# alexkroman/tiny-audio

Measured on AMD Instinct MI355X. Metric: training audio-sec/sec on 10s@16kHz clips, higher is better.
Workload: dtype bf16

## Files before the change

### include/ta355.h

```cpp
#ifndef TA355_H
#define TA355_H

#ifdef __cplusplus
extern "C" {
#endif

#ifndef __HIP_PLATFORM_AMD__
typedef struct ihipStream_t* hipStream_t;
#endif

#define TA_OK 0
#define TA_ERR_ARG 1
#define TA_ERR_LAUNCH 2

int ta_version(void);



long ta_logmel_scratch_floats(int B, int Ls, int n_mels);
int ta_logmel_mel_ranges(const float* melfb, int n_mels, int* mel_ranges, hipStream_t st);
int ta_logmel_f32(const float* wav, const long* lens, int B, int Ls, const float* dft, const float* window,
                  const float* melfb, int n_mels, float* feats, int* mask, float* scratch, const int* mel_ranges, hipStream_t st);

typedef struct {
// ... 83 lines not shown

int ta_moe_pack_images(const float* const* w1, const float* const* b1, const float* const* w2, const float* const* b2, int n, int H, int In,
                       int D, void* W1a, void* W1ta, void* W2a, void* W2ta, float* B1a, float* B2a, hipStream_t st);
long ta_moe_tape_bytes(const ta_moe_weights* w, int B, int S);
long ta_moe_bwd_workspace_bytes(const ta_moe_weights* w, int B, int S);
int ta_moe_projector_forward(const ta_moe_weights* w, const void* x_bf16, int B, int S, const float* noise, int training,
                             float* y, float* aux, void* tape, hipStream_t st);
int ta_moe_projector_backward(const ta_moe_weights* w, const void* x_bf16, int B, int S, const float* dy, float d_aux,
                              const float* noise, int training, const void* tape, float* d_norm_w, float* d_router_w,
                              float* const* dW1, float* const* db1, float* const* dW2, float* const* db2, void* ws,
                              long ws_bytes, hipStream_t st);
int ta_moe_projector_backward_dev(const ta_moe_weights* w, const void* x_bf16, int B, int S, const float* dy,
                                  const float* d_aux_dev, const float* noise, int training, const void* tape,
                                  float* d_norm_w, float* d_router_w, float* const* dW1, float* const* db1,
                                  float* const* dW2, float* const* db2, void* ws, long ws_bytes, hipStream_t st);

int ta_moe_router_aux_grads(const ta_moe_weights* w, const void* x_bf16, int B, int S, const float* d_aux_dev, const float* noise,
                            int training, const void* tape, float* d_norm_w_aux, float* d_router_w_aux, void* ws, long ws_bytes,
                            hipStream_t st);

typedef struct {
  const float* ln_in_w;
  const void *wqkv, *wqkv_t;
  const float *qn_w, *kn_w;
  const void *wo, *wo_t;
  const float* ln_post_w;
  const void *wgu, *wgu_t;
  const void *wd, *wd_t;
  const float *la_qkv, *lb_qkv, *la_o, *lb_o, *la_gu, *lb_gu, *la_d, *lb_d;
} ta_lm_layer;

typedef struct {
  float *dla_qkv, *dlb_qkv, *dla_o, *dlb_o, *dla_gu, *dlb_gu, *dla_d, *dlb_d;
} ta_lm_lora_grads;

typedef struct {
  int vocab, vocab_pad, hidden, ffn, n_layers, heads, kv_heads, head_dim, max_pos;
  float eps;
  const float* embed_f32;
  const void* embed_bf16;
  const void* embed_t_bf16;
  const float* norm_w;
  const float *rope_cos, *rope_sin;
  const ta_lm_layer* layers;
  int lora_rank;
  float lora_scale;
  int train_base;
  int lora_groups;
  int res_f32;
  int dx_f32;
  unsigned long long nope_layers;
} ta_lm_weights;

typedef struct {
  float *dwqkv;
  float *dwo;
  float *dwgu;
  float *dwd;
  float *dln_in, *dln_post;
  float *dqn, *dkn;
} ta_lm_layer_wgrads;
typedef struct {
  const ta_lm_layer_wgrads* layers;
  float* dnorm;
  float* dembed;
} ta_lm_wgrads;

long ta_lm_tape_bytes(const ta_lm_weights* w, int B, int L, int n_label_rows);
long ta_lm_workspace_bytes(const ta_lm_weights* w, int B, int L, int n_label_rows);
int ta_lm_forward_loss(const ta_lm_weights* w, const long* ids, const int* src_row, const float* audio,
                       const int* kmask, const int* pos, int B, int L, const int* label_rows,
                       const long* label_targets, int n_label_rows, float loss_scale, float* loss,
                       float* nll_rows, void* logits_out, void* tape, void* ws, long ws_bytes, hipStream_t st);
int ta_gelu_fwd(const void* h_bf16, void* a_bf16, long n, hipStream_t st);
int ta_gelu_bwd(const void* da_bf16, const void* h_bf16, void* dh_bf16, long n, hipStream_t st);
int ta_colsum(const void* x, int is_f32, int R, int C, float* out, hipStream_t st);
int ta_relu_fwd(const void* h_bf16, void* a_bf16, long n, hipStream_t st);
int ta_relu_bwd(const void* da_bf16, const void* h_bf16, void* dh_bf16, long n, hipStream_t st);
int ta_mix_fwd(const float* logits, const float* o, float* rw, float* out, int M, int D, int E, hipStream_t st);
int ta_mix_bwd(const float* dout, const float* o, const float* rw, void* do_bf16, float* dlogits, int M, int D, int E,
               hipStream_t st);
int ta_layernorm_res_fwd(const float* z, const float* keep, const float* res, long res_rows, const float* gamma,
                         const float* beta, float eps, float* xhat, float* rstd, float* y_f32, void* y_bf16, int M, int H,
                         hipStream_t st);
int ta_layernorm_bwd(const float* dy, const float* xhat, const float* rstd, const float* gamma, const float* keep, float* du,
                     void* dz_bf16, float* dgamma, float* dbeta, int M, int H, hipStream_t st);
int ta_attn_small_fwd(const void* Q, const void* K, const void* V, int EB, int heads, int hd, int Lq, int Lk, float scale,
                      const float* keep, float* P, void* O, hipStream_t st);
int ta_attn_small_bwd(const void* dO, const void* Q, const void* K, const void* V, const float* P, const float* keep,
                      float scale, void* dQ, void* dK, void* dV, int EB, int heads, int hd, int Lq, int Lk, hipStream_t st);

long ta_lm_prefill_workspace_bytes(const ta_lm_weights* w, int B, int L);
long ta_lm_lora_image_bytes(const ta_lm_weights* w);
int ta_lm_prefill(const ta_lm_weights* w, const long* ids, const int* src_row, const float* audio, const int* kmask,
                  const int* pos, int B, int L, void* kcache, void* vcache, int Lmax, const int* last_rows, float* logits,
                  void* lora_img, void* ws, long ws_bytes, hipStream_t st);
long ta_lm_decode_workspace_bytes(const ta_lm_weights* w, int B);
int ta_lm_decode_step(const ta_lm_weights* w, const long* ids, const int* pos, const int* kmask, const int* slot_dev, int B,
                      void* kcache, void* vcache, int Lmax, float* logits, const void* lora_img, void* ws, long ws_bytes,
                      hipStream_t st);
int ta_argmax_f32(const float* x, long ld, int n, int rows, long* out, hipStream_t st);
int ta_logits_process(float* logits, long ld, int V, const long* prompt_ids, int L, const long* out_seq, int max_new,
                      const int* step_dev, int B, float repetition_penalty, int no_repeat_ngram_size, hipStream_t st);
int ta_logits_warp(float* logits, long ld, int V, int B, float temperature, int top_k, float top_p, hipStream_t st);
int ta_sample_f32(const float* logits, long ld, int V, int B, unsigned long long seed, const int* step_dev, long* out, hipStream_t st);
int ta_logits_suppress_until(float* logits, long ld, int V, const long* ids, int n_ids, int min_new, const int* step_dev, int B,
                             hipStream_t st);
#define TA_SEQ_BIAS_MAX_SEQS 4096
#define TA_SEQ_BIAS_MAX_LEN 32
int ta_logits_sequence_bias(float* logits, long ld, int V, const long* prompt_ids, int L, const long* out_seq, int max_new,
                            const int* step_dev, int B, const long* seq_tokens, const int* seq_offsets, const float* seq_bias,
                            const int* group_starts, int n_seq, int n_groups, int n_tokens, hipStream_t st);
int ta_logits_step_rules(float* logits, long ld, int V, int B, const int* step_dev, int max_new, const long* forced_eos_ids,
                         int n_forced, const long* eos_ids, int n_eos, int decay_start, const float* decay_mult,
                         const long* suppress_ids, int n_suppress, const long* begin_suppress_ids, int n_begin, hipStream_t st);
int ta_logits_warp_ext(float* logits, long ld, int V, int B, float min_p, float typical_p, float epsilon_cutoff, float eta_cutoff,
                       hipStream_t st);
int ta_greedy_advance(const long* amax, const long* eos_ids, int n_eos, long pad_id, int* finished, long* next_ids,
                      long* out_seq, int max_new, int* step_dev, int* slot_dev, int* pos, int* kmask, int Lmax, int B,
                      int* n_unfinished, hipStream_t st);
int ta_token_scores_f32(const float* logits, long ld, int V, int B, const long* chosen, const int* finished, const int* step_dev,
                        int max_new, int top_k, float* logprob, float* entropy, long* top_ids, float* top_logprobs, hipStream_t st);

#define TA_EXTEND_MAX_T 256
#define TA_EXTEND_MAX_R 1024
int ta_attention_extend(const void* Q, const void* Kn, const void* Vn, const void* Kc, const void* Vc, const int* pmask,
                        const int* clip_of, const int* len, void* O, float* LSE, int B, int R, int Hq, int Hkv, int T, int Lp,
                        int Lmax, float scale, hipStream_t st);
#define TA_SCORE_MAX_ROWS 65536
#define TA_SCORE_CE_ROWS 256
long ta_lm_score_workspace_bytes(const ta_lm_weights* w, int B, int R, int T);
int ta_lm_score(const ta_lm_weights* w, const long* ids, const int* len, const int* len_host, const int* clip_of, const int* pos0,
                int B, int R, int T, const void* kcache, const void* vcache, int Lp, const int* pmask, const float* logits,
                const void* lora_img, float* token_logprobs, float* score, void* ws, long ws_bytes, hipStream_t st);

int ta_beam_logprobs_f32(float* logits, long ld, int V, int R, hipStream_t st);
long ta_beam_topk_workspace_bytes(int B, int K, int V, int M);
int ta_beam_topk_f32(const float* rows, long ld, int V, const float* score, int B, int K, int M, float* cand_score, int* cand_flat,
                     void* ws, long ws_bytes, hipStream_t st);
int ta_beam_advance(const float* cand_score, const int* cand_flat, int B, int K, int M, int V, const long* eos_ids, int n_eos,
                    long pad_id, int max_new, const float* len_div, int early_stopping, int heur_max_len, long* run_seq,
                    float* run_score, int* parent, long* next_ids, long* pool_seq, float* pool_score, int* pool_len,
                    int* pool_fin, int* heur, int* clip_done, int* step_dev, int* slot_dev, int* pos, int* kmask, int Lmax,
                    int* n_unfinished, float* tr_cand_score, int* tr_cand_flat, long* tr_run_seq, float* tr_run_score,
                    int* tr_parent, hipStream_t st);
int ta_kv_beam_expand(const void* ksrc, const void* vsrc, void* kdst, void* vdst, int layers, int B, int K, int kv_heads, int L,
                      int Lsrc, int Lmax, int head_dim, hipStream_t st);
int ta_kv_beam_reorder(void* kcache, void* vcache, int layers, int B, int K, int kv_heads, int L, int Lmax, int head_dim, int max_new,
                       const int* parent, const int* slot_dev, hipStream_t st);

int ta_lm_backward(const ta_lm_weights* w, const int* src_row, const int* kmask, const int* pos, int B, int L,
                   const int* label_rows, int n_label_rows, float* d_audio, long n_audio_rows, float* d_embeds,
                   const ta_lm_lora_grads* lora_grads, const ta_lm_wgrads* wgrads, const long* ids, const void* tape, void* ws,
                   long ws_bytes, hipStream_t st);

typedef struct ta_lora_dropout {
  float p;
  unsigned long long seed;
  unsigned long long offset;
} ta_lora_dropout;
int ta_lm_forward_loss_ex(const ta_lm_weights* w, const long* ids, const int* src_row, const float* audio,
                          const int* kmask, const int* pos, int B, int L, const int* label_rows,
                          const long* label_targets, int n_label_rows, float loss_scale, float* loss,
                          float* nll_rows, void* logits_out, void* tape, void* ws, long ws_bytes,
                          const ta_lora_dropout* drop, hipStream_t st);
int ta_lm_backward_ex(const ta_lm_weights* w, const int* src_row, const int* kmask, const int* pos, int B, int L,
                      const int* label_rows, int n_label_rows, float* d_audio, long n_audio_rows, float* d_embeds,
                      const ta_lm_lora_grads* lora_grads, const ta_lm_wgrads* wgrads, const long* ids, const void* tape, void* ws,
                      long ws_bytes, const ta_lora_dropout* drop, hipStream_t st);
int ta_segment_table(const int* segment_ids, int* seg, int* pos, int R, int L, hipStream_t st);
int ta_audio_index_seg(const long* ids, const int* segment_ids, const long* counts, int* src_row, int R, int L, int C, int N,
                       long audio_id, hipStream_t st);
int ta_lm_forward_loss_seg(const ta_lm_weights* w, const long* ids, const int* src_row, const float* audio,
                           const int* kmask, const int* pos, const int* seg, int B, int L, const int* label_rows,
                           const long* label_targets, int n_label_rows, float loss_scale, float* loss,
                           float* nll_rows, void* logits_out, void* tape, void* ws, long ws_bytes,
                           const ta_lora_dropout* drop, hipStream_t st);
int ta_lm_backward_seg(const ta_lm_weights* w, const int* src_row, const int* kmask, const int* pos, const int* seg, int B, int L,
                       const int* label_rows, int n_label_rows, float* d_audio, long n_audio_rows, float* d_embeds,
                       const ta_lm_lora_grads* lora_grads, const ta_lm_wgrads* wgrads, const long* ids, const void* tape, void* ws,
                       long ws_bytes, const ta_lora_dropout* drop, hipStream_t st);
struct ta_ce_options;
int ta_lm_forward_loss_opt(const ta_lm_weights* w, const long* ids, const int* src_row, const float* audio,
                           const int* kmask, const int* pos, const int* seg, int B, int L, const int* label_rows,
                           const long* label_targets, int n_label_rows, float loss_scale, float* loss,
                           float* nll_rows, void* logits_out, void* tape, void* ws, long ws_bytes,
                           const ta_lora_dropout* drop, const struct ta_ce_options* ce, hipStream_t st);
int ta_attention_fwd_seg(const void* Q, const void* K, const void* VT, void* O, float* LSE, const int* kmask, const int* seg,
                         int B, int Hq, int Hkv, int L, int Lp, float scale, hipStream_t st);
int ta_attention_fwd_qkv_seg(const void* qkv0, const float* qn_w, const float* kn_w, const float* cosT, const float* sinT,
                             const int* pos, void* Q, void* K, void* V, float* rq, float* rk, void* O, float* LSE,
                             const int* kmask, const int* seg, int B, int Hq, int Hkv, int L, float scale, float eps,
                             hipStream_t st);
int ta_attention_bwd_seg(const void* Q, const void* K, const void* V, const void* dO, long dO_stride, const float* LSE,
                         const float* Delta, const int* kmask, const int* seg, void* dQ, void* dK, void* dV, int B, int Hq,
                         int Hkv, int L, int Lp, float scale, hipStream_t st);
int ta_attention_bwd_qkv_seg(const void* Q, const void* K, const void* V, const void* dO, long dO_stride, const float* LSE,
                             const float* Delta, const int* kmask, const int* seg, const void* qkv0, const float* rq,
                             const float* rk, const float* qn_w, const float* kn_w, const float* cosT, const float* sinT,
                             const int* pos, void* dqkv, int B, int Hq, int Hkv, int L, int Lp, float scale, hipStream_t st);
int ta_lora_dropout_keep(const ta_lora_dropout* drop, int layer, int linear, int M, int in, unsigned char* out, hipStream_t st);


int ta_attention_enc_fwd(const void* qkv, void* out, int B, int heads, int S, hipStream_t st);
int ta_attention_enc_fwd_varlen(const void* qkv, void* out, const int* cu_rows, int B, int heads, int max_rows, hipStream_t st);

int ta_gemm_bf16_nt(const void* A, const void* W, void* C, int M, int N, int K, long lda, int a_rpb, long a_bs,
                    long ldc, int c_rpb, long c_bs, long c_off, const float* bias, const float* residual, int act,
                    int out_bf16, int splits, float* splitk_ws, hipStream_t st);
int ta_gemm_bf16_nt_ex(const void* A, const void* W, void* C, int M, int N, int K, long lda, int a_rpb, long a_bs,
                       long ldc, int c_rpb, long c_bs, long c_off, const float* bias, const float* residual, int act,
                       int out_bf16, int splits, float* splitk_ws, const int* a_idx, const int* seg,
                       const int* krange, hipStream_t st);
typedef struct {
  const void* a2; const void* w2; int k2; long lda2;
  const void* residual_bf16;
  const float* rope_tab; int rope_rows;
  int w_blocked;
  int rope_cols;
} ta_gemm_opts;
int ta_gemm_bf16_nt_opt(const void* A, const void* W, void* C, int M, int N, int K, long lda, int a_rpb, long a_bs,
                        long ldc, int c_rpb, long c_bs, long c_off, const float* bias, const float* residual, int act,
                        int out_bf16, int splits, float* splitk_ws, const int* a_idx, const int* seg,
                        const int* krange, const ta_gemm_opts* opts, hipStream_t st);
long ta_gemm_splitk_ws_bytes(int M, int N, int splits);
int ta_gemm_bf16_nt_grouped(const void* A, const void* W, void* C, int M, int N, int K, const float* bias, int act, int out_bf16,
                            const int* a_idx, const int* seg, const int* krange, int n_groups, long w_stride, long c_stride,
                            hipStream_t st);
long ta_gemm_bf16_tn_ws_bytes(int M, int Ny, int Nx);
int ta_gemm_bf16_tn(const void* Y, const void* X, float* out, int M, int Ny, int Nx, int accumulate, void* ws, long ws_bytes,
                    hipStream_t st);
int ta_profile_gemm(int enable);
int ta_profile_gemm_collect(double* total_ms, double* total_flops, long* launches);
long ta_profile_gemm_log(long* out, long max_rows);
int ta_gemm_reload_knobs(void);

int ta_layernorm_f32(const float* x, const float* w, const float* b, void* y_bf16, float* y_f32,
                     const float* rowscale, int M, int H, float eps, hipStream_t st);
int ta_layernorm_bf16(const void* x_bf16, const float* w, const float* b, void* y_bf16, float* y_f32, const float* rowscale,
                      int M, int H, float eps, hipStream_t st);
int ta_rmsnorm_fwd(const float* x, const float* w, void* y_bf16, float* y_f32, float* rstd, int M, int H,
                   float eps, int act_gelu, hipStream_t st);
int ta_rmsnorm_bwd(const float* dy, const float* x, const float* rstd, const float* w, const float* dres,
                   float* dx_f32, void* dx_bf16, float* dw_accum, int M, int H, int act_gelu, hipStream_t st);
int ta_rmsnorm_fwd_bf16(const void* x_bf16, const float* w, void* y_bf16, float* y_f32, float* rstd, int M, int H, float eps,
                        hipStream_t st);
int ta_rmsnorm_bwd_bf16(const void* dy, int dy_is_bf16, const void* x_bf16, const float* rstd, const float* w,
                        const float* dres, float* dx_f32, void* dx_bf16, int M, int H, hipStream_t st);
int ta_rmsnorm_bwd_bf16s(const void* dy, int dy_is_bf16, const void* x_bf16, const float* rstd, const float* w,
                         const void* dres_bf16, float* dx_f32, void* dx_bf16, int M, int H, hipStream_t st);
int ta_rmsnorm_bwd_dyb(const void* dy_bf16, const float* x, const float* rstd, const float* w, const float* dres, float* dx_f32,
                       void* dx_bf16, int M, int H, hipStream_t st);

int ta_rmsnorm_dw(const void* dy, int dy_is_bf16, const void* x, int x_is_bf16, const float* rstd, float* dw_accum, int M,
                  int H, hipStream_t st);

int ta_attention_fwd(const void* Q, const void* K, const void* VT, void* O, float* LSE, const int* kmask, int B,
                     int Hq, int Hkv, int L, int Lp, int head_dim, int causal, float scale, hipStream_t st);
typedef struct { long q_bs, q_hs, q_rs, k_bs, k_hs, k_rs, v_bs, v_hs, v_rs; } ta_attn_layout;
int ta_attention_fwd_ex(const void* Q, const void* K, const void* VT, void* O, float* LSE, const int* kmask, int B,
                        int Hq, int Hkv, int L, int Lp, int head_dim, int causal, float scale, const ta_attn_layout* lay,
                        hipStream_t st);
int ta_attention_fwd_qkv(const void* qkv0, const float* qn_w, const float* kn_w, const float* cosT, const float* sinT,
                         const int* pos, void* Q, void* K, void* V, float* rq, float* rk, void* O, float* LSE,
                         const int* kmask, int B, int Hq, int Hkv, int L, float scale, float eps, hipStream_t st);
int ta_attention_bwd(const void* Q, const void* QT, const void* K, const void* KT, const void* V, const void* dO,
                     long dO_stride, const void* dOT, const float* LSE, const float* Delta, const int* kmask,
                     void* dQ, void* dK, void* dV, int B, int Hq, int Hkv, int L, int Lp, int head_dim, int causal,
                     float scale, hipStream_t st);
int ta_attention_bwd_qkv(const void* Q, const void* K, const void* V, const void* dO, long dO_stride, const float* LSE,
                         const float* Delta, const int* kmask, const void* qkv0, const float* rq, const float* rk,
                         const float* qn_w, const float* kn_w, const float* cosT, const float* sinT, const int* pos,
                         void* dqkv, int B, int Hq, int Hkv, int L, int Lp, int head_dim, int causal, float scale,
                         hipStream_t st);
int ta_enc_qkv_post(const void* qkv, const float* cosT, const float* sinT, void* Q, void* K, void* VT, int B, int H,
                    int S, int Sp, hipStream_t st);
int ta_lm_qkv_post_fwd(const void* qkv0, const float* qn_w, const float* kn_w, const float* cosT, const float* sinT,
                       const int* pos, void* Q, void* K, void* V, void* QT, void* KT, void* VT, float* rq, float* rk,
                       int B, int Hq, int Hkv, int L, int Lp, float eps, hipStream_t st);
int ta_lm_qkv_post_bwd(const void* dQ, const void* dK, const void* dV, const void* qkv0, const float* rq,
                       const float* rk, const float* qn_w, const float* kn_w, const float* cosT, const float* sinT,
                       const int* pos, void* dqkv, float* dqn_accum, float* dkn_accum, int B, int Hq, int Hkv, int L, hipStream_t st);
int ta_attn_bwd_prep(const void* dO, const void* O, float* Delta, void* dOT, int B, int Hq, int L, int Lp,
                     hipStream_t st);

int ta_swiglu_fwd(const void* gu, void* act, long M, int F, hipStream_t st);
int ta_swiglu_bwd(const void* dact, const void* gu, void* dgu, long M, int F, hipStream_t st);
int ta_cast_f32_bf16(const float* x, void* y, long n, hipStream_t st);
int ta_transpose_to_bf16(const void* in, int in_is_f32, long ld_in, long in_bs, int in_rpb, void* out, long ld_out,
                         int R, int C, hipStream_t st);
int ta_feats_to_time_major(const float* feats, void* out, int B, int C, int T, hipStream_t st);
int ta_zero_pad_rows(void* buf, int B, int T, int C, hipStream_t st);
int ta_pos_add(void* x, int x_f32, const float* pos, int B, int S, int H, hipStream_t st);

int ta_audio_index(const long* ids, const long* counts, int* src_row, int B, int L, int N, long audio_id,
                   hipStream_t st);
int ta_embed_scatter(const long* ids, const int* src_row, const float* emb, const float* audio, float* x0,
                     void* x0_bf16, int n_rows, int D, long vocab, hipStream_t st);
int ta_audio_grad_gather(const int* src_row, const float* dx0, float* d_audio, int n_rows, int D, hipStream_t st);
int ta_embed_grad_scatter(const long* ids, const int* src_row, const float* dx0, float* dembed, int n_rows, int D, long vocab,
                          hipStream_t st);
int ta_gather_rows_bf16(const void* in, const int* idx, void* out, int n, int D, hipStream_t st);
int ta_scatter_rows_f32(const float* in, const int* idx, float* out, int n, int D, hipStream_t st);
int ta_bernoulli_keep(float* keep, long n, float keep_prob, unsigned long long seed, hipStream_t st);
int ta_debug_occupy(int workgroups, double micros, void* buf, long bytes, hipStream_t st);

int ta_cross_entropy(const void* logits, int logits_bf16, long ldl, const int* rows, const long* targets, int n, int V,
                     float scale, float* nll, float* loss_accum, void* dlogits_bf16, long ldd, hipStream_t st);
int ta_label_rows(const long* labels, int B, int L, int* rows, long* targets, int* n_out, hipStream_t st);
typedef struct ta_ce_options {
  float eps;
  float zc;
  float* obj;
} ta_ce_options;
int ta_cross_entropy_opt(const void* logits, int logits_bf16, long ldl, const int* rows, const long* targets, int n, int V,
                         float scale, float* nll, float* loss_accum, void* dlogits_bf16, long ldd, const ta_ce_options* opt,
                         hipStream_t st);

#define TA_SQNORM_SCRATCH_FLOATS 1024
int ta_grad_sqnorm(const float* g, long n, float* accum, float* scratch, hipStream_t st);
int ta_adamw_step(float* p, const float* g, float* m, float* v, long n, float lr, float beta1, float beta2, float eps,
                  float weight_decay, int step, const float* sqnorm, float max_norm, float grad_scale,
                  const float* denom, hipStream_t st);
int ta_adamw_step_multi(float* p, const float* g, float* m, float* v, long n, const long* seg_end, const float* seg_lr,
                        const float* seg_wd, int nseg, float lr_mult, float beta1, float beta2, float eps, int step,
                        const float* sqnorm, float max_norm, float grad_scale, const float* denom, hipStream_t st);

#define TA_WAVE_CONV_HOP 2048
#define TA_WAVE_CONV_DIRECT 32
int ta_wave_fft_twiddles(float* tw, hipStream_t st);
int ta_wave_ir_spectra(const float* ir, const long* ir_off, const int* part_off, int n_ir, int max_parts, const float* tw,
                       float* spectra, hipStream_t st);
long ta_wave_conv_ws_bytes(int B, int Ls, int max_taps);
int ta_wave_conv_f32(const float* wav, const long* lens, int B, int Ls, const int* ir_idx, const float* ir, const long* ir_off,
                     const int* part_off, int n_ir, int max_taps, const float* tw, const float* spectra, float rir_peak,
                     float* out, void* ws, long ws_bytes, hipStream_t st);
long ta_wave_mix_scratch_floats(int B, int Ls);
int ta_wave_mix_f32(float* wav, const long* lens, int B, int Ls, const int* noise_idx, const long* noise_start,
                    const float* noise_amp, const float* noise, const long* noise_off, int n_noise, const float* gauss_amp,
                    unsigned long long seed, unsigned long long offset, float* scratch, hipStream_t st);
int ta_wave_clip_f32(float* wav, const long* lens, int B, int Ls, const int* pct, hipStream_t st);
#define TA_WAVE_MAX_EVENTS 64
long ta_wave_events_scratch_floats(int B, int Ls, int ev_stride, long max_event_len);
int ta_wave_events_f32(float* wav, const long* lens, int B, int Ls, const int* ev_count, int ev_stride, const int* ev_pool,
                       const long* ev_off, const long* ev_len, const long* ev_t0, const int* ev_fade_in, const int* ev_fade_out,
                       const float* ev_amp, const float* pool, const long* pool_off, int n_pool, long max_event_len,
                       float fade_floor_db, float* scratch, hipStream_t st);
#define TA_WAVE_IIR_MAX_SECTIONS 8
#define TA_WAVE_IIR_CHUNK 256
long ta_wave_sos_ws_bytes(int B, int Ls, int chunk);
int ta_wave_sos_f32(float* wav, const long* lens, int B, int Ls, const int* n_sec, const double* sos, int chunk, void* ws,
                    long ws_bytes, hipStream_t st);

#define TA_ALIGN_MAX_TOKENS 2048
#define TA_ALIGN_MAX_FRAMES 32768
#define TA_ALIGN_MAX_CLASSES 65536
#define TA_ALIGN_MAX_CLIPS 4096
#define TA_ALIGN_THREADS 256
#define TA_ALIGN_FRAME_BLOCK 64
#define TA_ALIGN_STAGE_FLOATS 8192
long ta_ctc_align_workspace_bytes(int N, int max_T, int max_J);
int ta_ctc_align_f32(const float* emission, long ld, int C, const int* cu_frames, const int* tokens, const int* cu_tokens, int N,
                     int max_T, int max_J, int blank_id, int* frames, float* score, int* status, void* ws, long ws_bytes,
                     float* trellis_out, const long* trellis_off, hipStream_t st);

#define TA_ALIGN_LONG_MAX_TOKENS 262144
#define TA_ALIGN_LONG_MAX_FRAMES 1048576
#define TA_ALIGN_LONG_MAX_CLASSES 65536
#define TA_ALIGN_LONG_MAX_CLIPS 64
#define TA_ALIGN_LONG_MAX_COL_BLOCK 2048
#define TA_ALIGN_LONG_COL_BLOCK 256
#define TA_ALIGN_LONG_FRAME_BLOCK 64
long ta_ctc_align_long_workspace_bytes(int N, int max_T, int max_J, int col_block, int frame_block);
int ta_ctc_align_long_f32(const float* emission, long ld, int C, const int* cu_frames, const int* tokens, const int* cu_tokens, int N,
                          int max_T, int max_J, int blank_id, int col_block, int frame_block, int* frames, float* score, int* status,
                          void* ws, long ws_bytes, float* trellis_out, const long* trellis_off, hipStream_t st);

#define TA_TEXT_ALIGN_EDIT 0
#define TA_TEXT_ALIGN_LCS 1
#define TA_TEXT_ALIGN_MAX_LEN 262144
#define TA_TEXT_ALIGN_MAX_PAIRS 65536
#define TA_TEXT_ALIGN_MAX_COL_BLOCK 512
#define TA_TEXT_ALIGN_SHORT_MAX_M 512
#define TA_TEXT_ALIGN_COL_BLOCK 256
#define TA_TEXT_ALIGN_ROW_BLOCK 256
long ta_text_align_workspace_bytes(const int* cu_ref_host, const int* cu_hyp_host, int N, int max_n, int max_m, int want_path,
                                   int col_block, int row_block);
int ta_text_align_i32(const int* ref, const int* cu_ref, const int* hyp, const int* cu_hyp, int N, int max_n, int max_m, int mode,
                      int want_path, int col_block, int row_block, int* dist, int* counts, int* map, int* status, void* ws,
                      long ws_bytes, hipStream_t st);

#define TA_W2V_HEAD_PAD 64
typedef struct {
  int hidden, ffn, n_layers, heads, conv_dim, n_classes;
  float ln_eps;
  const float* conv0_w;
  const float *gn_w, *gn_b;
  const void* conv_w[6];
  const float *fp_ln_w, *fp_ln_b;
  const void* fp_w;
  const float* fp_b;
  const void* pos_w;
  const float* pos_b;
  const float *enc_ln_w, *enc_ln_b;
  const ta_enc_layer* layers;
  const void* head_w;
  const float* head_b;
  int res_f32;
} ta_wav2vec2_weights;

long ta_wav2vec2_workspace_bytes(const ta_wav2vec2_weights* w, int B, int Ls, long rows);
int ta_wav2vec2_forward(const ta_wav2vec2_weights* w, const float* wav, const int* lens_host, const int* lens_dev,
                        const int* cu_frames_dev, int B, int Ls, float* emissions, void* ws, long ws_bytes, hipStream_t st);

long ta_w2v_conv0_ws_bytes(int B, int Ls, int C);
int ta_w2v_conv0_gn_gelu(const float* wav, const int* lens_dev, int B, int Ls, const float* w, const float* gn_w,
                         const float* gn_b, int C, float eps, void* out_bf16, long out_rpb, void* ws, long ws_bytes,
                         hipStream_t st);
int ta_w2v_pos_conv(const void* x, int x_f32, const void* wp, const float* bias, void* y, const int* cu_rows, int B,
                    int max_rows, int H, hipStream_t st);
int ta_w2v_head_logsoftmax(const float* logits, long ld, const float* bias, int n_classes, float* out, int rows,
                           hipStream_t st);

#define TA_ECAPA_N_MELS 80
#define TA_ECAPA_FEAT_STRIDE 128
#define TA_ECAPA_SCALE 8
#define TA_ECAPA_MIN_T 5
#define TA_ECAPA_MAX_T 512
#define TA_ECAPA_MAX_DILATION 4
#define TA_ECAPA_MAX_CHANNELS 1024
#define TA_ECAPA_MAX_SE 256
#define TA_ECAPA_MAX_ATTN 256
#define TA_ECAPA_MAX_EMB 1024
typedef struct {
  const void* w1;
  const float *b1, *bn1_s, *bn1_t;
  const void* res_w;
  const float *res_b, *res_s, *res_t;
  const void* w2;
  const float *b2, *bn2_s, *bn2_t;
  const float *se_w1t, *se_b1;
  const float *se_w2t, *se_b2;
  int dilation;
} ta_ecapa_block;
typedef struct {
  int channels, se_channels, attn_channels, emb_dim;
  const float* fb_window;
  const float* fb_twiddle;
  const float* fb_mel;
  const int* fb_mel_range;
  const void* w0;
  const float *b0, *bn0_s, *bn0_t;
  ta_ecapa_block blocks[3];
  const void* mfa_w;
  const float *mfa_b, *mfa_s, *mfa_t;
  const void* att_wh;
  const void* att_wms;
  const float *att_b, *att_s, *att_t;
  const void* att_conv_w;
  const float* att_conv_b;
  const float *aspbn_s, *aspbn_t;
  const void* fc_w;
  const float* fc_b;
} ta_ecapa_weights;

long ta_ecapa_workspace_bytes(const ta_ecapa_weights* w, int n_windows, int T);
int ta_ecapa_forward(const ta_ecapa_weights* w, const float* audio, long n_audio, const int* starts_host, const int* lens_host,
                     const int* starts_dev, const int* lens_dev, int N, int window_samples, int chunk_windows, float* emb,
                     void* ws, long ws_bytes, hipStream_t st);

int ta_ecapa_fbank(const float* audio, long n_audio, const int* starts_dev, const int* lens_dev, int N, int window_samples,
                   const float* fb_window, const float* fb_twiddle, const float* fb_mel, const int* fb_mel_range,
                   float* feat, void* slab_bf16, hipStream_t st);
int ta_ecapa_res2net(const void* z1, long ldz, long z_rpw, const float* bn1_s, const float* bn1_t, const void* res_w,
                     const float* res_b, const float* res_s, const float* res_t, void* y, long ldy, long y_rpw, int N, int T,
                     int w, int dilation, hipStream_t st);
int ta_ecapa_relu_bn(const void* z, const float* scale, const float* shift, void* out, float* stats_f32, void* stats_bf16,
                     int N, int T, int Cw, hipStream_t st);
long ta_ecapa_se_ws_floats(int N, int Cw);
int ta_ecapa_se_residual(const void* z2, const float* bn2_s, const float* bn2_t, const float* se_w1t, const float* se_b1,
                         const float* se_w2t, const float* se_b2, const void* residual, long ldres, void* out, long ldout,
                         int N, int T, int Cw, int se, float* ws, hipStream_t st);
int ta_ecapa_attn_act(const float* g, const float* per_window, const float* scale, const float* shift, void* out, int N, int T,
                      int A, hipStream_t st);
int ta_ecapa_asp_pool(const float* logits, const void* h, const float* aspbn_s, const float* aspbn_t, void* out, float* attn_w,
                      float* pooled_f32, int N, int T, int Cw, hipStream_t st);

#define TA_SPK_MIN_N 6
#define TA_SPK_MAX_N 32768
#define TA_SPK_MAX_D 256
#define TA_SPK_MAX_P 32
#define TA_SPK_MAX_COLS 1024
long ta_spk_affinity_ws_floats(int N, int D);
int ta_spk_affinity_f32(const float* E, int N, int D, int keep, float* W, long ldw, float* deg, int* kept_count, float* ws, int phases,
                        hipStream_t st);
long ta_spk_lapmul_ws_floats(int N, int p);
int ta_spk_laplacian_matmul_f32(const float* W, long ldw, const float* deg, const float* X, long ldx, float* Y, long ldy, int N, int p,
                                float* ws, hipStream_t st);
long ta_spk_gram_ws_floats(int N, int a, int b);
int ta_spk_panel_gram_f32(const float* A, long lda, int a, const float* B, long ldb, int b, int N, float* C, long ldc, float* ws,
                          hipStream_t st);
int ta_spk_panel_update_f32(float* B, long ldb, int b, const float* A, long lda, int a, const float* C, long ldc, int N, hipStream_t st);
int ta_spk_panel_combine_f32(const float* V, long ldv, int c, const float* Z, long ldz, int m, float* Y, long ldy, int N, hipStream_t st);

#define TA_CUT_HOP 160
#define TA_CUT_POWER_WINDOW 400
#define TA_CUT_MAX_POSITIONS 1048576
#define TA_CUT_MAX_LEN 3000
#define TA_CUT_MAX_SMOOTH 64
#define TA_CUT_MAX_RECORDINGS 64
#define TA_CUT_MAX_BLOCKS 131072
#define TA_CUT_COST_K(h) (2 * (h) + 25 > 65 ? 2 * (h) + 25 : 65)
#define TA_WAVE_WINDOWS_MAX 65535
long ta_wave_cut_cost_workspace_bytes(int R, long max_n);
int ta_wave_cut_cost_f32(const float* wav, const long* offsets, int R, long max_n, int h, float cut_penalty, float* cost, long ld,
                         void* ws, long ws_bytes, hipStream_t st);
int ta_cut_plan_f32(const float* cost, long ld, const long* offsets, int R, long max_n, int min_len, int max_len, int* back, int* cuts,
                    long ldc, int* n_seg, float* dp_T, hipStream_t st);
int ta_wave_windows_f32(const float* wav, long total, const long* start, const int* len, int W, int Ls, float* out, long* lens,
                        hipStream_t st);

#ifdef __cplusplus
}
#endif
#endif
```

### tiny_audio_amd/csrc/api.hip

```cpp
#include <cstdlib>
#include "common.h"
#include "internal.h"
#include "../../include/ta355.h"

extern "C" int ta_version(void) { return 4; }

#include <algorithm>
#include "host_util.h"


namespace {
struct EncDesc {
  int H, F, L, nh, NM, max_pos, k1;
  float eps;
  const void *conv1_w, *conv2_w;
  const float *conv1_b, *conv2_b, *norm_w, *norm_b;
  const float *rope_cos, *rope_sin, *rope_il, *pos_emb;
  const ta_enc_layer* layers;
  int res_f32;
  bool whisper;
};
EncDesc enc_desc(const ta_encoder_weights* w) {
  return EncDesc{w->hidden, w->ffn, w->n_layers, w->heads, w->n_mels, w->max_pos, 3 * w->n_mels, w->ln_eps, w->conv1_w, w->conv2_w,
                 w->conv1_b, w->conv2_b, w->norm_w, w->norm_b, w->rope_cos, w->rope_sin, w->rope_il, nullptr, w->layers, w->res_f32, false};
}
EncDesc enc_desc(const ta_whisper_encoder_weights* w) {
  return EncDesc{w->hidden, w->ffn, w->n_layers, w->heads, w->n_mels, w->max_pos, pad64(3 * w->n_mels), w->ln_eps, w->conv1_w, w->conv2_w,
                 w->conv1_b, w->conv2_b, w->norm_w, w->norm_b, nullptr, nullptr, nullptr, w->pos_emb, w->layers, w->res_f32, true};
}
struct EncWs {
  bf16_t *x0, *x1, *xn, *qkv, *q, *k, *vt, *ao, *hf;
  float* xr;
  size_t bytes;
};
EncWs enc_carve(const EncDesc& d, int B, int T, void* base) {
  const int H = d.H, S = (T - 1) / 2 + 1, Sp = pad64(S);
  const long M = (long)B * S;
  Carver c(base);
  EncWs e;
  e.x0 = c.take<bf16_t>((size_t)B * (T + 2) * d.NM + (size_t)(d.k1 - 3 * d.NM));
  e.x1 = c.take<bf16_t>((size_t)B * (T + 2) * H);
  e.xr = (float*)c.take<float>((size_t)M * H);
  e.xn = c.take<bf16_t>((size_t)M * H);
  e.qkv = c.take<bf16_t>((size_t)M * 3 * H + 128);
  e.q = c.take<bf16_t>((size_t)M * H);
  e.k = c.take<bf16_t>((size_t)M * H);
  e.vt = c.take<bf16_t>((size_t)B * H * Sp);
  e.ao = c.take<bf16_t>((size_t)M * H);
  e.hf = c.take<bf16_t>((size_t)M * d.F);
  e.bytes = c.total();
  return e;
}

int enc_forward(const EncDesc& w, const float* feats, int B, int T, const float* frame_keep, void* out_bf16, float* out_f32,
                void* ws, long ws_bytes, hipStream_t st) {
  if (B <= 0 || T <= 0) return TA_OK;
  const int H = w.H, F = w.F, NM = w.NM, nh = w.nh, K1 = w.k1;
  if (H % 128 || F % 128 || K1 % 64 || NM % 8 || H / nh != 64 || (!out_bf16 && !out_f32)) return TA_ERR_ARG;
  const int S = (T - 1) / 2 + 1, Sp = pad64(S);
  if (S > w.max_pos) return TA_ERR_ARG;
  if (w.whisper && (T != 2 * w.max_pos || !w.pos_emb || H != nh * 64)) return TA_ERR_ARG;
  const int M = B * S;
  EncWs e = enc_carve(w, B, T, ws);
  if ((long)e.bytes > ws_bytes) return TA_ERR_ARG;
  RC(ta_feats_to_time_major(feats, e.x0, B, NM, T, st));
  if (K1 > 3 * NM && hipMemsetAsync(e.x0 + (size_t)B * (T + 2) * NM, 0, (size_t)(K1 - 3 * NM) * sizeof(bf16_t), st) != hipSuccess)
    return TA_ERR_LAUNCH;
  RC(ta_zero_pad_rows(e.x1, B, T, H, st));
  RC(ta_gemm_bf16_nt(e.x0, w.conv1_w, e.x1, B * T, H, K1, NM, T, (long)(T + 2) * NM, H, T, (long)(T + 2) * H, H,
                     w.conv1_b, nullptr, 1, 1, 1, nullptr, st));
  const bool res_f32 = w.res_f32 != 0;
  const int rb = res_f32 ? 0 : 1;
  auto ln = [&](const float* gw, const float* gb, void* yb, float* yf, const float* rowscale) -> int {
    return rb ? ta_layernorm_bf16(e.xr, gw, gb, yb, yf, rowscale, M, H, w.eps, st)
              : ta_layernorm_f32(e.xr, gw, gb, yb, yf, rowscale, M, H, w.eps, st);
  };
  auto res_gemm = [&](const void* A, const void* Wm, int K, const float* bias) -> int {
    if (rb) { ta_gemm_opts o = opts_none(); o.residual_bf16 = e.xr; return gemm_opt(A, Wm, e.xr, M, H, K, bias, nullptr, 0, 1, o, st); }
    return gemm(A, Wm, e.xr, M, H, K, bias, e.xr, 0, 0, st);
  };
  RC(ta_gemm_bf16_nt(e.x1, w.conv2_w, e.xr, M, H, 3 * H, 2L * H, S, (long)(T + 2) * H, H, 0, 0, 0, w.conv2_b, nullptr,
                     1, rb, 1, nullptr, st));
  if (w.whisper) RC(ta_pos_add(e.xr, res_f32 ? 1 : 0, w.pos_emb, B, S, H, st));
  const float scale = 0.125f;
  const char* fz = getenv("TA355_ENC_QKV_FUSED");
  const bool fa = w.whisper || (!(fz && *fz == '0') && w.rope_il && (H / nh) == 64);
  for (int l = 0; l < w.L; ++l) {
    const ta_enc_layer& L = w.layers[l];
    if (w.whisper && !(L.wqkv_fa && L.bqkv_fa)) return TA_ERR_ARG;
    RC(ln(L.ln1_w, L.ln1_b, e.xn, nullptr, nullptr));
    if (fa && L.wqkv_fa && L.bqkv_fa) {
      if (w.whisper) {
        RC(gemm(e.xn, L.wqkv_fa, e.qkv, M, 3 * H, H, L.bqkv_fa, nullptr, 0, 1, st));
      } else {
        ta_gemm_opts o = opts_none(); o.rope_tab = w.rope_il; o.rope_rows = S; o.rope_cols = 2 * H;
        RC(gemm_opt(e.xn, L.wqkv_fa, e.qkv, M, 3 * H, H, L.bqkv_fa, nullptr, 2, 1, o, st));
      }
      RC(ta_attention_enc_fwd(e.qkv, e.ao, B, nh, S, st));
      RC(res_gemm(e.ao, L.wo, H, L.bo));
    } else {
      RC(gemm(e.xn, L.wqkv, e.qkv, M, 3 * H, H, L.bqkv, nullptr, 0, 1, st));
      RC(ta_enc_qkv_post(e.qkv, w.rope_cos, w.rope_sin, e.q, e.k, e.vt, B, nh, S, Sp, st));
      RC(ta_attention_fwd(e.q, e.k, e.vt, e.ao, nullptr, nullptr, B, nh, nh, S, Sp, 64, 0, scale, st));
      RC(res_gemm(e.ao, L.wo, H, L.bo));
    }
    RC(ln(L.ln2_w, L.ln2_b, e.xn, nullptr, nullptr));
    RC(gemm(e.xn, L.w1, e.hf, M, F, H, L.b1, nullptr, 1, 1, st));
    RC(res_gemm(e.hf, L.w2, F, L.b2));
  }
  RC(ln(w.norm_w, w.norm_b, out_bf16, out_f32, frame_keep));
  return TA_OK;
}

struct EncRaggedWs {
  bf16_t *x0, *x1, *xn, *qkv, *ao, *hf;
  void* c2;
  float *xr, *rope;
  size_t bytes;
};
EncRaggedWs enc_ragged_carve(const EncDesc& d, int B, int T, long rows, void* base) {
  const int H = d.H, S = (T - 1) / 2 + 1;
  const long M = (long)B * S;
  Carver c(base);
  EncRaggedWs e;
  e.x0 = c.take<bf16_t>((size_t)B * (T + 2) * d.NM + (size_t)(d.k1 - 3 * d.NM));
  e.x1 = c.take<bf16_t>((size_t)B * (T + 2) * H);
  e.c2 = c.take<float>((size_t)M * H);
  e.xr = c.take<float>((size_t)rows * H);
  e.rope = c.take<float>((size_t)rows * 32);
  e.xn = c.take<bf16_t>((size_t)rows * H);
  e.qkv = c.take<bf16_t>((size_t)rows * 3 * H);
  e.ao = c.take<bf16_t>((size_t)rows * H);
  e.hf = c.take<bf16_t>((size_t)rows * d.F);
  e.bytes = c.total();
  return e;
}

int enc_forward_ragged(const EncDesc& w, const float* feats, int B, int T, const int* mel_len, const int* cu, const float* frame_keep,
                       void* out_bf16, float* out_f32, void* ws, long ws_bytes, hipStream_t st) {
  if (B <= 0 || T <= 0) return TA_OK;
  const int H = w.H, F = w.F, NM = w.NM, nh = w.nh, K1 = w.k1;
  if (H % 128 || F % 128 || K1 % 64 || NM % 8 || H / nh != 64 || (!out_bf16 && !out_f32) || !mel_len || !cu || !feats) return TA_ERR_ARG;
  if (!w.rope_il) return TA_ERR_ARG;
  if (K1 != 3 * NM) return TA_ERR_ARG;
  for (int l = 0; l < w.L; ++l) if (!(w.layers[l].wqkv_fa && w.layers[l].bqkv_fa)) return TA_ERR_ARG;
  const int S = (T - 1) / 2 + 1;
  if (S > w.max_pos) return TA_ERR_ARG;
  long rows_l = 0; int max_rows = 0;
  for (int b = 0; b < B; ++b) {
    if (mel_len[b] < 1 || mel_len[b] > T) return TA_ERR_ARG;
    const int Sb = (mel_len[b] - 1) / 2 + 1;
    rows_l += Sb; max_rows = Sb > max_rows ? Sb : max_rows;
  }
  if (rows_l > 0x7fffffffL / (3L * H)) return TA_ERR_ARG;
  const int rows = (int)rows_l;
  EncRaggedWs e = enc_ragged_carve(w, B, T, rows, ws);
  if ((long)e.bytes > ws_bytes) return TA_ERR_ARG;
  RC(ta_i_feats_to_time_major_len(feats, e.x0, B, NM, T, mel_len, st));
  RC(ta_gemm_bf16_nt(e.x0, w.conv1_w, e.x1, B * T, H, K1, NM, T, (long)(T + 2) * NM, H, T, (long)(T + 2) * H, H,
                     w.conv1_b, nullptr, 1, 1, 1, nullptr, st));
  RC(ta_i_zero_tail_rows(e.x1, B, T, H, mel_len, st));
  const bool res_f32 = w.res_f32 != 0;
  const int rb = res_f32 ? 0 : 1;
  RC(ta_gemm_bf16_nt(e.x1, w.conv2_w, e.c2, B * S, H, 3 * H, 2L * H, S, (long)(T + 2) * H, H, 0, 0, 0, w.conv2_b, nullptr,
                     1, rb, 1, nullptr, st));
  RC(ta_i_compact_rows(e.c2, e.xr, cu, B, S, rows, H * (rb ? 2 : 4), st));
  RC(ta_i_rope_rows(w.rope_il, e.rope, cu, B, rows, w.max_pos, st));
  const int M = rows;
  auto ln = [&](const float* gw, const float* gb, void* yb, float* yf) -> int {
    return rb ? ta_layernorm_bf16(e.xr, gw, gb, yb, yf, nullptr, M, H, w.eps, st)
              : ta_layernorm_f32(e.xr, gw, gb, yb, yf, nullptr, M, H, w.eps, st);
  };
  auto res_gemm = [&](const void* A, const void* Wm, int K, const float* bias) -> int {
    if (rb) { ta_gemm_opts o = opts_none(); o.residual_bf16 = e.xr; return gemm_opt(A, Wm, e.xr, M, H, K, bias, nullptr, 0, 1, o, st); }
    return gemm(A, Wm, e.xr, M, H, K, bias, e.xr, 0, 0, st);
  };
  for (int l = 0; l < w.L; ++l) {
    const ta_enc_layer& L = w.layers[l];
    RC(ln(L.ln1_w, L.ln1_b, e.xn, nullptr));
    ta_gemm_opts o = opts_none(); o.rope_tab = e.rope; o.rope_rows = rows; o.rope_cols = 2 * H;
    RC(gemm_opt(e.xn, L.wqkv_fa, e.qkv, M, 3 * H, H, L.bqkv_fa, nullptr, 2, 1, o, st));
    RC(ta_attention_enc_fwd_varlen(e.qkv, e.ao, cu, B, nh, max_rows, st));
    RC(res_gemm(e.ao, L.wo, H, L.bo));
    RC(ln(L.ln2_w, L.ln2_b, e.xn, nullptr));
    RC(gemm(e.xn, L.w1, e.hf, M, F, H, L.b1, nullptr, 1, 1, st));
    RC(res_gemm(e.hf, L.w2, F, L.b2));
  }
  bf16_t* yb = out_bf16 ? e.xn : nullptr;
  float* yf = out_f32 ? (float*)e.qkv : nullptr;
  RC(ln(w.norm_w, w.norm_b, yb, yf));
  RC(ta_i_expand_rows(yb, yf, out_bf16, out_f32, cu, frame_keep, B, S, rows, H, st));
  return TA_OK;
}
}

extern "C" long ta_encoder_workspace_bytes(const ta_encoder_weights* w, int B, int T) {
  return (long)enc_carve(enc_desc(w), B, T, nullptr).bytes;
}
extern "C" int ta_encoder_forward(const ta_encoder_weights* w, const float* feats, int B, int T, const float* frame_keep,
                                  void* out_bf16, float* out_f32, void* ws, long ws_bytes, hipStream_t st) {
  return enc_forward(enc_desc(w), feats, B, T, frame_keep, out_bf16, out_f32, ws, ws_bytes, st);
}
extern "C" long ta_encoder_ragged_workspace_bytes(const ta_encoder_weights* w, int B, int T, long rows) {
  return (long)enc_ragged_carve(enc_desc(w), B, T, rows < 0 ? 0 : rows, nullptr).bytes;
}
extern "C" int ta_encoder_forward_ragged(const ta_encoder_weights* w, const float* feats, int B, int T, const int* mel_len_host,
                                         const int* cu_rows_dev, const float* frame_keep, void* out_bf16, float* out_f32, void* ws,
                                         long ws_bytes, hipStream_t st) {
  return enc_forward_ragged(enc_desc(w), feats, B, T, mel_len_host, cu_rows_dev, frame_keep, out_bf16, out_f32, ws, ws_bytes, st);
}
extern "C" long ta_whisper_encoder_workspace_bytes(const ta_whisper_encoder_weights* w, int B, int T) {
  return (long)enc_carve(enc_desc(w), B, T, nullptr).bytes;
}
extern "C" int ta_whisper_encoder_forward(const ta_whisper_encoder_weights* w, const float* feats, int B, int T, const float* frame_keep,
                                          void* out_bf16, float* out_f32, void* ws, long ws_bytes, hipStream_t st) {
  return enc_forward(enc_desc(w), feats, B, T, frame_keep, out_bf16, out_f32, ws, ws_bytes, st);
}

namespace {
struct MlpTape { float *h1, *r1, *h2, *r2; bf16_t* a1; size_t bytes; };
MlpTape mlp_tape(const ta_mlp_weights* w, int B, int S, void* base) {
  const int N = (S - w->k) / w->k + 1;
  const long Mp = (long)B * N;
  Carver c(base);
  MlpTape t;
  t.h1 = c.take<float>((size_t)Mp * w->hidden);
  t.r1 = c.take<float>((size_t)Mp);
  t.a1 = c.take<bf16_t>((size_t)Mp * w->hidden);
  t.h2 = c.take<float>((size_t)Mp * w->llm_dim);
  t.r2 = c.take<float>((size_t)Mp);
  t.bytes = c.total();
  return t;
}
struct MlpBwdWs { float *dh2, *da1, *skws, *dgws; bf16_t *dh2b, *dh2T, *a1T, *dh1b, *dh1T, *xsT; size_t bytes; };
MlpBwdWs mlp_bwd_ws(const ta_mlp_weights* w, int B, int S, void* base) {
  const int N = (S - w->k) / w->k + 1, Hd = w->hidden, D = w->llm_dim, In = w->k * w->enc_dim;
  const long Mp = (long)B * N; const int Kp = pad64((int)Mp);
  Carver c(base);
  MlpBwdWs s;
  s.dh2 = c.take<float>((size_t)Mp * D);
  s.dh2b = c.take<bf16_t>((size_t)Mp * D);
  s.dh2T = c.take<bf16_t>((size_t)D * Kp);
  s.a1T = c.take<bf16_t>((size_t)Hd * Kp);
  s.da1 = c.take<float>((size_t)Mp * Hd);
  s.dh1b = c.take<bf16_t>((size_t)Mp * Hd);
  s.dh1T = c.take<bf16_t>((size_t)Hd * Kp);
  s.xsT = c.take<bf16_t>((size_t)In * Kp);
  const int s1 = pick_splits(Hd, In, Kp), s2 = pick_splits(D, Hd, Kp);
  const size_t sk1 = (size_t)ta_gemm_splitk_ws_bytes(Hd, In, s1), sk2 = (size_t)ta_gemm_splitk_ws_bytes(D, Hd, s2);
  s.skws = c.take<float>((sk1 > sk2 ? sk1 : sk2) / 4 + 4);
  s.dgws = c.take<float>((size_t)ta_i_rmsnorm_bwd_ws_floats((int)Mp, Hd > D ? Hd : D));
  s.bytes = c.total();
  return s;
}
}

extern "C" long ta_mlp_tape_bytes(const ta_mlp_weights* w, int B, int S) { return (long)mlp_tape(w, B, S, nullptr).bytes; }
extern "C" long ta_mlp_bwd_workspace_bytes(const ta_mlp_weights* w, int B, int S) {
  return (long)mlp_bwd_ws(w, B, S, nullptr).bytes;
}

extern "C" int ta_mlp_projector_forward(const ta_mlp_weights* w, const void* x, int B, int S, float* y, void* tape,
                                        hipStream_t st) {
  const int k = w->k, E = w->enc_dim, Hd = w->hidden, D = w->llm_dim, In = k * E;
  const int N = (S - k) / k + 1;
  if (B <= 0 || N <= 0) return TA_OK;
  if (In % 64 || Hd % 64 || D % 4 || Hd % 4) return TA_ERR_ARG;
  const int Mp = B * N;
  MlpTape t = mlp_tape(w, B, S, tape);
  RC(ta_gemm_bf16_nt(x, w->w1, t.h1, Mp, Hd, In, In, N, (long)S * E, Hd, 0, 0, 0, nullptr, nullptr, 0, 0, 1, nullptr, st));
  RC(ta_rmsnorm_fwd(t.h1, w->g1, t.a1, nullptr, t.r1, Mp, Hd, w->eps, 1, st));
  RC(gemm(t.a1, w->w2, t.h2, Mp, D, Hd, nullptr, nullptr, 0, 0, st));
  RC(ta_rmsnorm_fwd(t.h2, w->g2, nullptr, y, t.r2, Mp, D, w->eps, 0, st));
  return TA_OK;
}

extern "C" int ta_mlp_projector_backward(const ta_mlp_weights* w, const void* x, int B, int S, const float* dy,
                                         const void* tape, float* dW1, float* dg1, float* dW2, float* dg2, void* ws,
                                         long ws_bytes, hipStream_t st) {
  const int k = w->k, E = w->enc_dim, Hd = w->hidden, D = w->llm_dim, In = k * E;
  const int N = (S - k) / k + 1;
  if (B <= 0 || N <= 0) return TA_OK;
  const int Mp = B * N, Kp = pad64(Mp);
  MlpTape t = mlp_tape(w, B, S, (void*)tape);
  MlpBwdWs s = mlp_bwd_ws(w, B, S, ws);
  if ((long)s.bytes > ws_bytes) return TA_ERR_ARG;
  if (hipMemsetAsync(dg1, 0, (size_t)Hd * 4, st) != hipSuccess) return TA_ERR_LAUNCH;
  if (hipMemsetAsync(dg2, 0, (size_t)D * 4, st) != hipSuccess) return TA_ERR_LAUNCH;
  RC(ta_i_rmsnorm_bwd(dy, t.h2, t.r2, w->g2, nullptr, nullptr, s.dh2b, dg2, s.dgws, Mp, D, 0, st));
  RC(ta_transpose_to_bf16(s.dh2b, 0, D, 0, 0, s.dh2T, Kp, Mp, D, st));
  RC(ta_transpose_to_bf16(t.a1, 0, Hd, 0, 0, s.a1T, Kp, Mp, Hd, st));
  const int s2 = pick_splits(D, Hd, Kp);
  RC(ta_gemm_bf16_nt(s.dh2T, s.a1T, dW2, D, Hd, Kp, Kp, 0, 0, Hd, 0, 0, 0, nullptr, nullptr, 0, 0, s2, s.skws, st));
  RC(gemm(s.dh2b, w->w2_t, s.da1, Mp, Hd, D, nullptr, nullptr, 0, 0, st));
  RC(ta_i_rmsnorm_bwd(s.da1, t.h1, t.r1, w->g1, nullptr, nullptr, s.dh1b, dg1, s.dgws, Mp, Hd, 1, st));
  RC(ta_transpose_to_bf16(s.dh1b, 0, Hd, 0, 0, s.dh1T, Kp, Mp, Hd, st));
  RC(ta_transpose_to_bf16(x, 0, In, (long)S * E, N, s.xsT, Kp, Mp, In, st));
  const int s1 = pick_splits(Hd, In, Kp);
  RC(ta_gemm_bf16_nt(s.dh1T, s.xsT, dW1, Hd, In, Kp, Kp, 0, 0, In, 0, 0, 0, nullptr, nullptr, 0, 0, s1, s.skws, st));
  return TA_OK;
}

namespace {
inline bool lm_res_bf16(const ta_lm_weights* w) { return w->res_f32 == 0; }
struct LmLayerTape {
  float *x_in, *r_in, *rq, *rk, *lse, *x1, *r_post;
  bf16_t *qkv0, *q, *k, *v, *qt, *kt, *vt, *ao, *gu;
  bf16_t *xn_s, *xn2_s, *act_s, *xa_qkv, *xa_o, *xa_gu, *xa_d;
  LoraImg i_qkv, i_o, i_gu, i_d;
};
struct LmTape {
  LmLayerTape* L;
  float *x_final, *r_f;
  bf16_t *hn, *dlogits;
  size_t bytes;
};
constexpr int MAX_LM_LAYERS = 64;
struct LmDims { int D, F, nq, nkv, hd, NQKV, Lp; long M; };
LmDims lm_dims(const ta_lm_weights* w, int B, int L) {
  LmDims d;
  d.D = w->hidden; d.F = w->ffn; d.nq = w->heads; d.nkv = w->kv_heads; d.hd = w->head_dim;
  d.NQKV = (d.nq + 2 * d.nkv) * d.hd; d.Lp = pad64(L); d.M = (long)B * L;
  return d;
}
inline const float* lm_rope_cos(const ta_lm_weights* w, int l) { return ((w->nope_layers >> l) & 1) ? nullptr : w->rope_cos; }
inline const float* lm_rope_sin(const ta_lm_weights* w, int l) { return ((w->nope_layers >> l) & 1) ? nullptr : w->rope_sin; }
inline bool lm_attn_fused(const LmDims& d, int L) { return d.hd == 128 && L <= 192 && (d.nq / d.nkv) * ((L + 31) / 32) <= 12; }
LmTape lm_tape(const ta_lm_weights* w, int B, int L, int n_lab, void* base, LmLayerTape* store) {
  const LmDims d = lm_dims(w, B, L);
  Carver c(base);
  LmTape t; t.L = store;
  for (int l = 0; l < w->n_layers; ++l) {
    LmLayerTape& p = store[l];
    p.x_in = c.take<float>((size_t)d.M * d.D);
    p.r_in = c.take<float>((size_t)d.M);
    p.qkv0 = c.take<bf16_t>((size_t)d.M * d.NQKV);
    p.rq = c.take<float>((size_t)d.M * d.nq);
    p.rk = c.take<float>((size_t)d.M * d.nkv);
    p.q = c.take<bf16_t>((size_t)d.M * d.nq * d.hd);
    p.k = c.take<bf16_t>((size_t)d.M * d.nkv * d.hd);
    p.v = c.take<bf16_t>((size_t)d.M * d.nkv * d.hd);
    p.qt = nullptr; p.kt = nullptr;
    p.vt = c.take<bf16_t>((size_t)B * d.nkv * d.hd * d.Lp);
    p.ao = c.take<bf16_t>((size_t)d.M * d.nq * d.hd);
    p.lse = c.take<float>((size_t)B * d.nq * L);
    p.x1 = c.take<float>((size_t)d.M * d.D);
    p.r_post = c.take<float>((size_t)d.M);
    p.gu = c.take<bf16_t>((size_t)d.M * 2 * d.F);
    if (w->lora_rank > 0 || w->train_base) {
      p.xn_s = c.take<bf16_t>((size_t)d.M * d.D); p.xn2_s = c.take<bf16_t>((size_t)d.M * d.D);
      p.act_s = c.take<bf16_t>((size_t)d.M * d.F);
    }
    if (w->lora_rank > 0) {
      p.xa_qkv = c.take<bf16_t>((size_t)d.M * 64); p.xa_o = c.take<bf16_t>((size_t)d.M * 64);
      p.xa_gu = c.take<bf16_t>((size_t)d.M * 64); p.xa_d = c.take<bf16_t>((size_t)d.M * 64);
      auto img = [&](LoraImg& g, int in, int N) {
        g.a = c.take<bf16_t>((size_t)64 * in); g.at = c.take<bf16_t>((size_t)64 * in);
        g.b = c.take<bf16_t>((size_t)64 * N); g.bt = c.take<bf16_t>((size_t)64 * N);
      };
      img(p.i_qkv, d.D, d.NQKV); img(p.i_o, d.nq * d.hd, d.D); img(p.i_gu, d.D, 2 * d.F); img(p.i_d, d.F, d.D);
    }
  }
  t.x_final = c.take<float>((size_t)d.M * d.D);
  t.r_f = c.take<float>((size_t)d.M);
  t.hn = c.take<bf16_t>((size_t)d.M * d.D);
  t.dlogits = c.take<bf16_t>((size_t)(n_lab > 0 ? n_lab : 1) * w->vocab_pad);
  t.bytes = c.total();
  return t;
}
struct LmWs {
  bf16_t *xn, *act, *hl, *dxb, *dact, *dgu, *dao, *dot, *dq, *dk, *dv, *dqkv, *dyB;
  float* lora_part;
  long lp_layer, lp_off[8], lp_size[8]; int lp_chunks[8];
  float *logits, *dhl, *dhn, *dxa, *dxb32, *dxn, *delta, *skws;
  bf16_t *tA, *tB;
  float* wsk;
  size_t bytes;
};
inline int wgrad_splits(int n_out, int k_in, int kp) { return pick_splits(n_out, k_in, kp); }
LmWs lm_ws(const ta_lm_weights* w, int B, int L, int n_lab, void* base) {
  const LmDims d = lm_dims(w, B, L);
  const int nl = n_lab > 0 ? n_lab : 1;
  Carver c(base);
  LmWs s;
  s.xn = c.take<bf16_t>((size_t)d.M * d.D);
  s.act = c.take<bf16_t>((size_t)d.M * d.F);
  s.hl = c.take<bf16_t>((size_t)nl * d.D);
  s.logits = c.take<float>((size_t)nl * w->vocab_pad);
  s.dhl = c.take<float>((size_t)nl * d.D);
  s.dhn = c.take<float>((size_t)d.M * d.D);
  s.dxa = c.take<float>((size_t)d.M * d.D);
  s.dxb32 = c.take<float>((size_t)d.M * d.D);
  s.dxn = c.take<float>((size_t)d.M * d.D);
  s.dxb = c.take<bf16_t>((size_t)d.M * d.D);
  s.dact = c.take<bf16_t>((size_t)d.M * d.F);
  s.dgu = c.take<bf16_t>((size_t)d.M * 2 * d.F);
  s.dao = c.take<bf16_t>((size_t)d.M * d.nq * d.hd);
  s.dot = nullptr;
  s.delta = c.take<float>((size_t)B * d.nq * L);
  s.dq = c.take<bf16_t>((size_t)d.M * d.nq * d.hd);
  s.dk = c.take<bf16_t>((size_t)d.M * d.nkv * d.hd);
  s.dv = c.take<bf16_t>((size_t)d.M * d.nkv * d.hd);
  s.dqkv = c.take<bf16_t>((size_t)d.M * d.NQKV);
  s.dyB = c.take<bf16_t>((size_t)d.M * 64);
  s.lora_part = nullptr; s.lp_layer = 0;
  if (w->lora_rank > 0) {
    const int r = w->lora_rank, bq = d.nq * d.hd;
    const int members[4] = {3, 1, 2, 1}, Ng[4] = {d.NQKV, d.D, 2 * d.F, d.D}, ing[4] = {d.D, bq, d.D, d.F};
    long off = 0;
    for (int g = 0; g < 4; ++g) {
      const int chunks = ta_cdiv((int)d.M, ta_i_lora_tn2_rows((int)d.M, Ng[g], ing[g]));
      s.lp_size[2 * g] = (long)members[g] * r * ing[g]; s.lp_size[2 * g + 1] = (long)Ng[g] * r;
      for (int h = 0; h < 2; ++h) { s.lp_chunks[2 * g + h] = chunks; s.lp_off[2 * g + h] = off; off += s.lp_size[2 * g + h] * chunks; }
    }
    s.lp_layer = off;
    s.lora_part = c.take<float>((size_t)off * w->n_layers);
  }
  const int sp = pick_splits(nl, d.D, w->vocab_pad);
  s.skws = c.take<float>((size_t)ta_gemm_splitk_ws_bytes(nl, d.D, sp) / 4 + 4);
  s.tA = s.tB = nullptr; s.wsk = nullptr;
  if (w->train_base) {
    const int Kp = pad64((int)d.M), Kl = pad64(nl), bq = d.nq * d.hd;
    const size_t a_rows = (size_t)std::max(std::max(2 * d.F, d.NQKV), d.D), b_rows = (size_t)std::max(std::max(d.F, bq), d.D);
    s.tA = c.take<bf16_t>(std::max(a_rows * Kp, (size_t)w->vocab_pad * Kl));
    s.tB = c.take<bf16_t>(std::max(b_rows * Kp, (size_t)d.D * Kl));
    const int shp[4][2] = {{d.NQKV, d.D}, {d.D, bq}, {2 * d.F, d.D}, {d.D, d.F}};
    size_t mx = 0;
    for (auto& q : shp) {
      mx = std::max(mx, (size_t)ta_gemm_splitk_ws_bytes(q[0], q[1], wgrad_splits(q[0], q[1], Kp)));
      mx = std::max(mx, (size_t)ta_gemm_bf16_tn_ws_bytes((int)d.M, q[0], q[1]));
    }
    s.wsk = c.take<float>(mx / 4 + 4);
  }
  s.bytes = c.total();
  return s;
}
}

extern "C" long ta_lm_tape_bytes(const ta_lm_weights* w, int B, int L, int n_label_rows) {
  LmLayerTape store[MAX_LM_LAYERS];
  if (w->n_layers > MAX_LM_LAYERS) return -1;
  return (long)lm_tape(w, B, L, n_label_rows, nullptr, store).bytes;
}
extern "C" long ta_lm_workspace_bytes(const ta_lm_weights* w, int B, int L, int n_label_rows) {
  return (long)lm_ws(w, B, L, n_label_rows, nullptr).bytes;
}

struct LmExtend { const bf16_t *kc, *vc; const int *pmask, *clip_of, *len; int clips, Lp; };
static int lm_layers_forward(const ta_lm_weights* w, const LmDims& d, int B, int L, const int* kmask, const int* pos,
                             LmLayerTape* store, bool alias, float* x_final, LmWs& s, const ta_i_lora_layer_imgs* ext,
                             bf16_t* kcache, bf16_t* vcache, int Lmax, hipStream_t st, const LoraDropDev* drop = nullptr,
                             const int* seg = nullptr, const LmExtend* xt = nullptr) {
  const int M = (int)d.M;
  const float scale = 1.0f / sqrtf((float)d.hd);
  const bool lora = w->lora_rank > 0;
  const int r = w->lora_rank;
  if (lora && (r < 1 || 3 * r > 64)) return TA_ERR_ARG;
  const int lgm = lora ? (w->lora_groups ? w->lora_groups : 15) : 0;
  ta_gemm_opts kx = opts_none();
  auto lora_fwd = [&](const bf16_t* x, int in, const LoraImg& g, bf16_t* xa, int members, int lj0) -> int {
    if (drop) RC(ta_i_lora_skinny_nt_drop(x, in, g.a, xa, M, LoraDrop{*drop, (unsigned)lj0, r, members}, st));
    else RC(ta_i_lora_skinny_nt(x, in, g.a, xa, M, members * r, st));
    kx = opts_kext(xa, g.b);
    return TA_OK;
  };
  auto take_ext = [&]() { const ta_gemm_opts o = kx; kx = opts_none(); return o; };
  if (lora && !xt) {
    const int NB = 1 << 30, bq = d.nq * d.hd, bk = bq + d.nkv * d.hd, NL = w->n_layers;
    auto imgs_of = [&](int l) {
      LmLayerTape q = store[(alias || ext) ? 0 : l];
      if (ext) { q.i_qkv = ext[l].g[0]; q.i_o = ext[l].g[1]; q.i_gu = ext[l].g[2]; q.i_d = ext[l].g[3]; }
      return q;
    };
    const LmLayerTape q0 = imgs_of(0), q1 = imgs_of(NL > 1 ? 1 : 0);
    const ta_lm_layer &L0 = w->layers[0], &L1 = w->layers[NL > 1 ? 1 : 0];
    bool strided = NL > 1 && (ext || !alias);
    const long is_ = strided ? (long)(q1.i_qkv.a - q0.i_qkv.a) : 0;
    struct Kind { const float* m0; const float* m1; bf16_t* o0; bf16_t* o1; bf16_t* t0; bf16_t* t1; };
    const Kind kinds[8] = {{L0.la_qkv, L1.la_qkv, q0.i_qkv.a, q1.i_qkv.a, q0.i_qkv.at, q1.i_qkv.at}, {L0.lb_qkv, L1.lb_qkv, q0.i_qkv.b, q1.i_qkv.b, q0.i_qkv.bt, q1.i_qkv.bt},
                           {L0.la_o, L1.la_o, q0.i_o.a, q1.i_o.a, q0.i_o.at, q1.i_o.at}, {L0.lb_o, L1.lb_o, q0.i_o.b, q1.i_o.b, q0.i_o.bt, q1.i_o.bt},
                           {L0.la_gu, L1.la_gu, q0.i_gu.a, q1.i_gu.a, q0.i_gu.at, q1.i_gu.at}, {L0.lb_gu, L1.lb_gu, q0.i_gu.b, q1.i_gu.b, q0.i_gu.bt, q1.i_gu.bt},
                           {L0.la_d, L1.la_d, q0.i_d.a, q1.i_d.a, q0.i_d.at, q1.i_d.at}, {L0.lb_d, L1.lb_d, q0.i_d.b, q1.i_d.b, q0.i_d.bt, q1.i_d.bt}};
    long ms[8];
    for (int k = 0; k < 8 && strided; ++k) {
      ms[k] = (long)(kinds[k].m1 - kinds[k].m0);
      if ((long)(kinds[k].o1 - kinds[k].o0) != is_ || (long)(kinds[k].t1 - kinds[k].t0) != is_) strided = false;
    }
    for (int l = 2; l < NL && strided; ++l) {
      const ta_lm_layer& Ll = w->layers[l];
      const LmLayerTape ql = imgs_of(l);
      const float* mm[8] = {Ll.la_qkv, Ll.lb_qkv, Ll.la_o, Ll.lb_o, Ll.la_gu, Ll.lb_gu, Ll.la_d, Ll.lb_d};
      const bf16_t* oo[8] = {ql.i_qkv.a, ql.i_qkv.b, ql.i_o.a, ql.i_o.b, ql.i_gu.a, ql.i_gu.b, ql.i_d.a, ql.i_d.b};
      for (int k = 0; k < 8; ++k)
        if (mm[k] != kinds[k].m0 + l * ms[k] || oo[k] != kinds[k].o0 + l * is_) strided = false;
    }
    const int reps = strided ? 1 : NL, per = strided ? NL : 1;
    for (int l = 0; l < reps; ++l) {
      const ta_lm_layer& Ll = w->layers[l];
      const LmLayerTape ql = imgs_of(l);
      if (lgm & 1) RC(ta_i_lora_pack_a(Ll.la_qkv, w->lora_scale, ql.i_qkv.a, ql.i_qkv.at, 3 * r, d.D, per, strided ? ms[0] : 0, is_, st));
      if (lgm & 1) RC(ta_i_lora_pack_b(Ll.lb_qkv, ql.i_qkv.b, ql.i_qkv.bt, d.NQKV, r, bq, bk, per, strided ? ms[1] : 0, is_, st));
      if (lgm & 2) RC(ta_i_lora_pack_a(Ll.la_o, w->lora_scale, ql.i_o.a, ql.i_o.at, r, bq, per, strided ? ms[2] : 0, is_, st));
      if (lgm & 2) RC(ta_i_lora_pack_b(Ll.lb_o, ql.i_o.b, ql.i_o.bt, d.D, r, NB, NB, per, strided ? ms[3] : 0, is_, st));
      if (lgm & 4) RC(ta_i_lora_pack_a(Ll.la_gu, w->lora_scale, ql.i_gu.a, ql.i_gu.at, 2 * r, d.D, per, strided ? ms[4] : 0, is_, st));
      if (lgm & 4) RC(ta_i_lora_pack_b(Ll.lb_gu, ql.i_gu.b, ql.i_gu.bt, 2 * d.F, r, d.F, NB, per, strided ? ms[5] : 0, is_, st));
      if (lgm & 8) RC(ta_i_lora_pack_a(Ll.la_d, w->lora_scale, ql.i_d.a, ql.i_d.at, r, d.F, per, strided ? ms[6] : 0, is_, st));
      if (lgm & 8) RC(ta_i_lora_pack_b(Ll.lb_d, ql.i_d.b, ql.i_d.bt, d.D, r, NB, NB, per, strided ? ms[7] : 0, is_, st));
    }
  }
  for (int l = 0; l < w->n_layers; ++l) {
    const ta_lm_layer& Lw = w->layers[l];
    LmLayerTape p = store[alias ? 0 : l];
    if (ext) { p.i_qkv = ext[l].g[0]; p.i_o = ext[l].g[1]; p.i_gu = ext[l].g[2]; p.i_d = ext[l].g[3]; }
    float* x_next = (l + 1 < w->n_layers) ? store[alias ? 0 : l + 1].x_in : x_final;
    const bool keep = lora || (w->train_base && !alias);
    bf16_t* xn = keep ? p.xn_s : s.xn;
    const bool rb = lm_res_bf16(w);
    auto norm = [&](const float* x, const float* gw, bf16_t* y, float* r) -> int {
      return rb ? ta_rmsnorm_fwd_bf16(x, gw, y, nullptr, r, M, d.D, w->eps, st) : ta_rmsnorm_fwd(x, gw, y, nullptr, r, M, d.D, w->eps, 0, st);
    };
    auto res_gemm = [&](const void* A, const void* Wm, float* out, int K, const float* res) -> int {
      ta_gemm_opts o = take_ext();
      if (rb) { o.residual_bf16 = res; return gemm_opt(A, Wm, out, M, d.D, K, nullptr, nullptr, 0, 1, o, st); }
      return gemm_opt(A, Wm, out, M, d.D, K, nullptr, res, 0, 0, o, st);
    };
    RC(norm(p.x_in, Lw.ln_in_w, xn, p.r_in));
    if (lgm & 1) RC(lora_fwd(xn, d.D, p.i_qkv, p.xa_qkv, 3, 8 * l + 0));
    RC(gemm_opt(xn, Lw.wqkv, p.qkv0, M, d.NQKV, d.D, nullptr, nullptr, 0, 1, take_ext(), st));
    const bool fused_fwd = !xt && lm_attn_fused(d, L);
    if (xt)
      RC(ta_lm_qkv_post_fwd(p.qkv0, Lw.qn_w, Lw.kn_w, lm_rope_cos(w, l), lm_rope_sin(w, l), pos, p.q, p.k, p.v, nullptr, nullptr, nullptr,
                            p.rq, p.rk, B, d.nq, d.nkv, L, d.Lp, w->eps, st));
    else if (fused_fwd && seg)
      RC(ta_attention_fwd_qkv_seg(p.qkv0, Lw.qn_w, Lw.kn_w, lm_rope_cos(w, l), lm_rope_sin(w, l), pos, p.q, p.k, (kcache || w->train_base) ? p.v : nullptr, p.rq, p.rk, p.ao, p.lse, kmask,
                                  seg, B, d.nq, d.nkv, L, scale, w->eps, st));
    else if (fused_fwd)
      RC(ta_attention_fwd_qkv(p.qkv0, Lw.qn_w, Lw.kn_w, lm_rope_cos(w, l), lm_rope_sin(w, l), pos, p.q, p.k, (kcache || w->train_base) ? p.v : nullptr, p.rq, p.rk, p.ao, p.lse, kmask,
                              B, d.nq, d.nkv, L, scale, w->eps, st));
    else
      RC(ta_lm_qkv_post_fwd(p.qkv0, Lw.qn_w, Lw.kn_w, lm_rope_cos(w, l), lm_rope_sin(w, l), pos, p.q, p.k, p.v, p.qt, p.kt, p.vt, p.rq,
                            p.rk, B, d.nq, d.nkv, L, d.Lp, w->eps, st));
    if (kcache) {
      const size_t row = (size_t)L * d.hd * 2, pitch = (size_t)Lmax * d.hd * 2, rows = (size_t)B * d.nkv;
      if (hipMemcpy2DAsync(kcache + (size_t)l * rows * Lmax * d.hd, pitch, p.k, row, row, rows, hipMemcpyDeviceToDevice, st) != hipSuccess ||
          hipMemcpy2DAsync(vcache + (size_t)l * rows * Lmax * d.hd, pitch, p.v, row, row, rows, hipMemcpyDeviceToDevice, st) != hipSuccess)
        return TA_ERR_LAUNCH;
    }
    if (xt) {
      const size_t layer = (size_t)xt->clips * d.nkv * xt->Lp * d.hd;
      RC(ta_attention_extend(p.q, p.k, p.v, xt->kc + l * layer, xt->vc + l * layer, xt->pmask, xt->clip_of, xt->len, p.ao, nullptr,
                             xt->clips, B, d.nq, d.nkv, L, xt->Lp, xt->Lp, scale, st));
    } else if (!fused_fwd && seg) RC(ta_attention_fwd_seg(p.q, p.k, p.vt, p.ao, p.lse, kmask, seg, B, d.nq, d.nkv, L, d.Lp, scale, st));
    else if (!fused_fwd) RC(ta_attention_fwd(p.q, p.k, p.vt, p.ao, p.lse, kmask, B, d.nq, d.nkv, L, d.Lp, d.hd, 1, scale, st));
    if (lgm & 2) RC(lora_fwd(p.ao, d.nq * d.hd, p.i_o, p.xa_o, 1, 8 * l + 3));
    RC(res_gemm(p.ao, Lw.wo, p.x1, d.nq * d.hd, p.x_in));
    bf16_t* xn2 = keep ? p.xn2_s : s.xn;
    bf16_t* act = keep ? p.act_s : s.act;
    RC(norm(p.x1, Lw.ln_post_w, xn2, p.r_post));
    if (lgm & 4) RC(lora_fwd(xn2, d.D, p.i_gu, p.xa_gu, 2, 8 * l + 4));
    RC(gemm_opt(xn2, Lw.wgu, p.gu, M, 2 * d.F, d.D, nullptr, nullptr, 0, 1, take_ext(), st));
    RC(ta_swiglu_fwd(p.gu, act, M, d.F, st));
    if (lgm & 8) RC(lora_fwd(act, d.F, p.i_d, p.xa_d, 1, 8 * l + 6));
    RC(res_gemm(act, Lw.wd, x_next, d.F, p.x1));
  }
  return TA_OK;
}

static int lm_lora_drop(const ta_lm_weights* w, const ta_lora_dropout* drop, LoraDropDev* dd, const LoraDropDev** out) {
  *out = nullptr;
  if (!drop) return TA_OK;
  if (!(drop->p >= 0.f) || !(drop->p < 1.f) || w->n_layers >= 512 || w->ffn >= (1 << 23) || w->hidden >= (1 << 23)) return TA_ERR_ARG;
  if (!ta_i_lora_drop_dev(drop, dd)) return TA_OK;
  if (w->lora_rank <= 0 || w->train_base) return TA_ERR_ARG;
  *out = dd;
  return TA_OK;
}
static int lm_forward_loss_impl(const ta_lm_weights* w, const long* ids, const int* src_row, const float* audio,
                                const int* kmask, const int* pos, const int* seg, int B, int L, const int* label_rows,
                                const long* label_targets, int n_lab, float loss_scale, float* loss, float* nll_rows,
                                void* logits_out, void* tape, void* ws, long ws_bytes, const ta_lora_dropout* drop,
                                const ta_ce_options* ce, hipStream_t st) {
  if (ce && (!(ce->eps >= 0.f) || !(ce->eps < 1.f) || !(ce->zc >= 0.f) || ((ce->eps > 0.f || ce->zc > 0.f) && !ce->obj)))
    return TA_ERR_ARG;
  LoraDropDev dd;
  const LoraDropDev* dp = nullptr;
  RC(lm_lora_drop(w, drop, &dd, &dp));
  if (B <= 0 || L <= 0) return TA_OK;
  if (w->n_layers > MAX_LM_LAYERS || w->head_dim != 128 || w->hidden % 128 || w->ffn % 64 || w->vocab_pad % 128 ||
      w->vocab > w->vocab_pad || L > w->max_pos)
    return TA_ERR_ARG;
  const LmDims d = lm_dims(w, B, L);
  const int M = (int)d.M;
  LmLayerTape store[MAX_LM_LAYERS];
  LmTape t = lm_tape(w, B, L, n_lab, tape, store);
  LmWs s = lm_ws(w, B, L, n_lab, ws);
  if ((long)s.bytes > ws_bytes) return TA_ERR_ARG;
  float* x = store[0].x_in;
  if (lm_res_bf16(w)) RC(ta_embed_scatter(ids, src_row, w->embed_f32, audio, nullptr, x, M, d.D, w->vocab, st));
  else RC(ta_embed_scatter(ids, src_row, w->embed_f32, audio, x, nullptr, M, d.D, w->vocab, st));
  RC(lm_layers_forward(w, d, B, L, kmask, pos, store, false, t.x_final, s, nullptr, nullptr, nullptr, 0, st, dp, seg));
  if (lm_res_bf16(w)) RC(ta_rmsnorm_fwd_bf16(t.x_final, w->norm_w, t.hn, nullptr, t.r_f, M, d.D, w->eps, st));
  else RC(ta_rmsnorm_fwd(t.x_final, w->norm_w, t.hn, nullptr, t.r_f, M, d.D, w->eps, 0, st));
  if (logits_out)
    RC(gemm(t.hn, w->embed_bf16, logits_out, M, w->vocab_pad, d.D, nullptr, nullptr, 0, 1, st));
  if (n_lab > 0) {
    RC(ta_gather_rows_bf16(t.hn, label_rows, s.hl, n_lab, d.D, st));
    RC(gemm(s.hl, w->embed_bf16, s.logits, n_lab, w->vocab_pad, d.D, nullptr, nullptr, 0, 1, st));
    RC(ta_cross_entropy_opt(s.logits, 1, w->vocab_pad, nullptr, label_targets, n_lab, w->vocab, loss_scale, nll_rows, loss,
                            t.dlogits, w->vocab_pad, ce, st));
  }
  return TA_OK;
}

extern "C" int ta_lm_forward_loss(const ta_lm_weights* w, const long* ids, const int* src_row, const float* audio,
                                  const int* kmask, const int* pos, int B, int L, const int* label_rows,
                                  const long* label_targets, int n_lab, float loss_scale, float* loss, float* nll_rows,
                                  void* logits_out, void* tape, void* ws, long ws_bytes, hipStream_t st) {
  return lm_forward_loss_impl(w, ids, src_row, audio, kmask, pos, nullptr, B, L, label_rows, label_targets, n_lab, loss_scale, loss,
                              nll_rows, logits_out, tape, ws, ws_bytes, nullptr, nullptr, st);
}
extern "C" int ta_lm_forward_loss_ex(const ta_lm_weights* w, const long* ids, const int* src_row, const float* audio,
                                     const int* kmask, const int* pos, int B, int L, const int* label_rows,
                                     const long* label_targets, int n_lab, float loss_scale, float* loss, float* nll_rows,
                                     void* logits_out, void* tape, void* ws, long ws_bytes, const ta_lora_dropout* drop,
                                     hipStream_t st) {
  return lm_forward_loss_impl(w, ids, src_row, audio, kmask, pos, nullptr, B, L, label_rows, label_targets, n_lab, loss_scale, loss,
                              nll_rows, logits_out, tape, ws, ws_bytes, drop, nullptr, st);
}
extern "C" int ta_lm_forward_loss_seg(const ta_lm_weights* w, const long* ids, const int* src_row, const float* audio,
                                      const int* kmask, const int* pos, const int* seg, int B, int L, const int* label_rows,
                                      const long* label_targets, int n_lab, float loss_scale, float* loss, float* nll_rows,
                                      void* logits_out, void* tape, void* ws, long ws_bytes, const ta_lora_dropout* drop,
                                      hipStream_t st) {
  return lm_forward_loss_impl(w, ids, src_row, audio, kmask, pos, seg, B, L, label_rows, label_targets, n_lab, loss_scale, loss,
                              nll_rows, logits_out, tape, ws, ws_bytes, drop, nullptr, st);
}
extern "C" int ta_lm_forward_loss_opt(const ta_lm_weights* w, const long* ids, const int* src_row, const float* audio,
                                      const int* kmask, const int* pos, const int* seg, int B, int L, const int* label_rows,
                                      const long* label_targets, int n_lab, float loss_scale, float* loss, float* nll_rows,
                                      void* logits_out, void* tape, void* ws, long ws_bytes, const ta_lora_dropout* drop,
                                      const ta_ce_options* ce, hipStream_t st) {
  return lm_forward_loss_impl(w, ids, src_row, audio, kmask, pos, seg, B, L, label_rows, label_targets, n_lab, loss_scale, loss,
                              nll_rows, logits_out, tape, ws, ws_bytes, drop, ce, st);
}

namespace {
struct PrefillWs { ta_lm_weights w1; LmLayerTape layer[1]; LmTape t; LmWs s; size_t tape_bytes, bytes; };
PrefillWs prefill_ws(const ta_lm_weights* w, int B, int L, void* base) {
  PrefillWs p;
  p.w1 = *w; p.w1.n_layers = 1;
  p.t = lm_tape(&p.w1, B, L, 1, base, p.layer);
  p.tape_bytes = p.t.bytes;
  p.s = lm_ws(w, B, L, B, base ? (char*)base + p.tape_bytes : nullptr);
  p.bytes = p.tape_bytes + p.s.bytes;
  return p;
}
}
extern "C" long ta_lm_prefill_workspace_bytes(const ta_lm_weights* w, int B, int L) {
  return (long)prefill_ws(w, B, L, nullptr).bytes;
}
extern "C" long ta_lm_lora_image_bytes(const ta_lm_weights* w) {
  return w->lora_rank > 0 ? (long)lora_imgs_carve(w, nullptr, nullptr) : 0;
}
extern "C" int ta_lm_prefill(const ta_lm_weights* w, const long* ids, const int* src_row, const float* audio,
                             const int* kmask, const int* pos, int B, int L, void* kcache, void* vcache, int Lmax,
                             const int* last_rows, float* logits, void* lora_img, void* ws, long ws_bytes,
                             hipStream_t st) {
  if (B <= 0 || L <= 0) return TA_OK;
  if (w->n_layers > MAX_LM_LAYERS || w->head_dim != 128 || w->hidden % 128 || w->ffn % 64 || w->vocab_pad % 128 ||
      w->vocab > w->vocab_pad || L > w->max_pos || Lmax < L || !kcache || !vcache || !last_rows || !logits)
    return TA_ERR_ARG;
  if (w->lora_rank > 0 && !lora_img) return TA_ERR_ARG;
  const LmDims d = lm_dims(w, B, L);
  const int M = (int)d.M;
  PrefillWs p = prefill_ws(w, B, L, ws);
  if ((long)p.bytes > ws_bytes) return TA_ERR_ARG;
  ta_i_lora_layer_imgs imgs[MAX_LM_LAYERS];
  if (w->lora_rank > 0) lora_imgs_carve(w, lora_img, imgs);
  if (lm_res_bf16(w)) RC(ta_embed_scatter(ids, src_row, w->embed_f32, audio, nullptr, p.layer[0].x_in, M, d.D, w->vocab, st));
  else RC(ta_embed_scatter(ids, src_row, w->embed_f32, audio, p.layer[0].x_in, nullptr, M, d.D, w->vocab, st));
  RC(lm_layers_forward(w, d, B, L, kmask, pos, p.layer, true, p.t.x_final, p.s, w->lora_rank > 0 ? imgs : nullptr,
                       (bf16_t*)kcache, (bf16_t*)vcache, Lmax, st));
  if (lm_res_bf16(w)) RC(ta_rmsnorm_fwd_bf16(p.t.x_final, w->norm_w, p.t.hn, nullptr, p.t.r_f, M, d.D, w->eps, st));
  else RC(ta_rmsnorm_fwd(p.t.x_final, w->norm_w, p.t.hn, nullptr, p.t.r_f, M, d.D, w->eps, 0, st));
  RC(ta_gather_rows_bf16(p.t.hn, last_rows, p.s.hl, B, d.D, st));
  RC(gemm(p.s.hl, w->embed_bf16, logits, B, w->vocab_pad, d.D, nullptr, nullptr, 0, 0, st));
  return TA_OK;
}

namespace {
struct ScoreWs {
  PrefillWs p;
  long *ids_clean, *label_targets;
  int *pos, *off, *label_rows;
  float *nll, *lse;
  int chunk;
  size_t bytes;
};
ScoreWs score_ws(const ta_lm_weights* w, int B, int R, int T, void* base) {
  ScoreWs q;
  const long rows = (long)R * T, labs = std::max((long)R * (T - 1), 1L);
  q.chunk = (int)std::min((long)TA_SCORE_CE_ROWS, labs);
  q.p.w1 = *w; q.p.w1.n_layers = 1;
  q.p.t = lm_tape(&q.p.w1, R, T, 1, base, q.p.layer);
  q.p.tape_bytes = q.p.t.bytes;
  q.p.s = lm_ws(w, R, T, q.chunk, base ? (char*)base + q.p.tape_bytes : nullptr);
  q.p.bytes = q.p.tape_bytes + q.p.s.bytes;
  Carver c(base ? (char*)base + q.p.bytes : nullptr);
  q.ids_clean = c.take<long>((size_t)rows);
  q.pos = c.take<int>((size_t)rows);
  q.off = c.take<int>((size_t)R + 1);
  q.label_rows = c.take<int>((size_t)labs);
  q.label_targets = c.take<long>((size_t)labs);
  q.nll = c.take<float>((size_t)labs);
  q.lse = c.take<float>((size_t)B);
  q.bytes = q.p.bytes + c.total();
  return q;
}
bool score_shape_ok(const ta_lm_weights* w, int B, int R, int T) {
  return w && B >= 1 && R >= 1 && R <= TA_EXTEND_MAX_R && T >= 1 && T <= TA_EXTEND_MAX_T && (long)R * T <= TA_SCORE_MAX_ROWS &&
         w->n_layers <= MAX_LM_LAYERS && w->n_layers >= 1;
}
}
extern "C" long ta_lm_score_workspace_bytes(const ta_lm_weights* w, int B, int R, int T) {
  if (!score_shape_ok(w, B, R, T)) return -1;
  return (long)score_ws(w, B, R, T, nullptr).bytes;
}
extern "C" int ta_lm_score(const ta_lm_weights* w, const long* ids, const int* len, const int* len_host, const int* clip_of,
                           const int* pos0, int B, int R, int T, const void* kcache, const void* vcache, int Lp, const int* pmask,
                           const float* logits, const void* lora_img, float* token_logprobs, float* score, void* ws, long ws_bytes,
                           hipStream_t st) {
  if (!score_shape_ok(w, B, R, T) || !ids || !len || !len_host || !clip_of || !pos0 || !kcache || !vcache || !pmask || !logits ||
      !token_logprobs || !score || !ws)
    return TA_ERR_ARG;
  const int grp = w->kv_heads > 0 && w->heads % w->kv_heads == 0 ? w->heads / w->kv_heads : 0;
  if (w->head_dim != 128 || w->hidden % 128 || w->ffn % 64 || w->vocab_pad % 128 || w->vocab > w->vocab_pad || w->vocab < 1 ||
      (grp != 1 && grp != 2 && grp != 4) || Lp < 1 || (long)Lp + T > w->max_pos)
    return TA_ERR_ARG;
  if (w->lora_rank > 0 && !lora_img) return TA_ERR_ARG;
  long n_lab = 0;
  for (int r = 0; r < R; ++r) {
    if (len_host[r] < 1 || len_host[r] > T) return TA_ERR_ARG;
    n_lab += len_host[r] - 1;
  }
  ScoreWs q = score_ws(w, B, R, T, ws);
  if ((long)q.bytes > ws_bytes) return TA_ERR_ARG;
  const LmDims d = lm_dims(w, R, T);
  const int M = (int)d.M;
  ta_i_lora_layer_imgs imgs[MAX_LM_LAYERS];
  if (w->lora_rank > 0) lora_imgs_carve(w, (void*)lora_img, imgs);
  RC(ta_i_score_prep(ids, len, clip_of, pos0, B, R, T, Lp, w->vocab, q.ids_clean, q.pos, q.off, q.label_rows, q.label_targets, st));
  RC(ta_i_score_lse(logits, w->vocab_pad, w->vocab, B, q.lse, st));
  if (n_lab > 0) {
    float* x0 = q.p.layer[0].x_in;
    if (lm_res_bf16(w)) RC(ta_embed_scatter(q.ids_clean, nullptr, w->embed_f32, nullptr, nullptr, x0, M, d.D, w->vocab, st));
    else RC(ta_embed_scatter(q.ids_clean, nullptr, w->embed_f32, nullptr, x0, nullptr, M, d.D, w->vocab, st));
    const LmExtend xt{(const bf16_t*)kcache, (const bf16_t*)vcache, pmask, clip_of, len, B, Lp};
    RC(lm_layers_forward(w, d, R, T, nullptr, q.pos, q.p.layer, true, q.p.t.x_final, q.p.s, w->lora_rank > 0 ? imgs : nullptr, nullptr,
                         nullptr, 0, st, nullptr, nullptr, &xt));
    if (lm_res_bf16(w)) RC(ta_rmsnorm_fwd_bf16(q.p.t.x_final, w->norm_w, q.p.t.hn, nullptr, q.p.t.r_f, M, d.D, w->eps, st));
    else RC(ta_rmsnorm_fwd(q.p.t.x_final, w->norm_w, q.p.t.hn, nullptr, q.p.t.r_f, M, d.D, w->eps, 0, st));
    for (long c0 = 0; c0 < n_lab; c0 += q.chunk) {
      const int n = (int)std::min((long)q.chunk, n_lab - c0);
      RC(ta_gather_rows_bf16(q.p.t.hn, q.label_rows + c0, q.p.s.hl, n, d.D, st));
      RC(gemm(q.p.s.hl, w->embed_bf16, q.p.s.logits, n, w->vocab_pad, d.D, nullptr, nullptr, 0, 0, st));
      RC(ta_cross_entropy(q.p.s.logits, 0, w->vocab_pad, nullptr, q.label_targets + c0, n, w->vocab, 1.0f, q.nll + c0, nullptr, nullptr, 0, st));
    }
  }
  RC(ta_i_score_finish(logits, w->vocab_pad, q.lse, q.ids_clean, len, clip_of, q.off, q.nll, B, R, T, token_logprobs, score, st));
  return TA_OK;
}

static int lm_backward_impl(const ta_lm_weights* w, const int* src_row, const int* kmask, const int* pos, const int* seg, int B, int L,
                            const int* label_rows, int n_lab, float* d_audio, long n_audio_rows, float* d_embeds,
                            const ta_lm_lora_grads* lora_grads, const ta_lm_wgrads* wg, const long* ids, const void* tape,
                            void* ws, long ws_bytes, const ta_lora_dropout* drop, hipStream_t st) {
  LoraDropDev dd;
  const LoraDropDev* dp = nullptr;
  RC(lm_lora_drop(w, drop, &dd, &dp));
  if (B <= 0 || L <= 0) return TA_OK;
  if (w->n_layers > MAX_LM_LAYERS) return TA_ERR_ARG;
  const bool lora = w->lora_rank > 0;
  if (lora && !lora_grads) return TA_ERR_ARG;
  if (wg && (!w->train_base || lora || !wg->layers || (wg->dembed && !ids))) return TA_ERR_ARG;
  const LmDims d = lm_dims(w, B, L);
  const int M = (int)d.M;
  LmLayerTape store[MAX_LM_LAYERS];
  LmTape t = lm_tape(w, B, L, n_lab, (void*)tape, store);
  LmWs s = lm_ws(w, B, L, n_lab, ws);
  if ((long)s.bytes > ws_bytes) return TA_ERR_ARG;
  const float scale = 1.0f / sqrtf((float)d.hd);
  if (d_audio && hipMemsetAsync(d_audio, 0, (size_t)n_audio_rows * d.D * 4, st) != hipSuccess) return TA_ERR_LAUNCH;
  const int r = w->lora_rank;
  const int lgm = lora ? (w->lora_groups ? w->lora_groups : 15) : 0;
  const int bq = d.nq * d.hd, bk = bq + d.nkv * d.hd;
  auto zero_lora = [&](const ta_lm_lora_grads& g) -> bool {
    auto z = [&](float* q, size_t n) { return hipMemsetAsync(q, 0, n * 4, st) == hipSuccess; };
    return z(g.dla_qkv, (size_t)3 * r * d.D) && z(g.dlb_qkv, (size_t)d.NQKV * r) && z(g.dla_o, (size_t)r * bq) &&
           z(g.dlb_o, (size_t)d.D * r) && z(g.dla_gu, (size_t)2 * r * d.D) && z(g.dlb_gu, (size_t)2 * d.F * r) &&
           z(g.dla_d, (size_t)r * d.F) && z(g.dlb_d, (size_t)d.D * r);
  };
  bool lora_parts = false;
  if (lora) {
    const int NL = w->n_layers;
    const size_t sz[8] = {(size_t)3 * r * d.D, (size_t)d.NQKV * r, (size_t)r * bq, (size_t)d.D * r, (size_t)2 * r * d.D,
                          (size_t)2 * d.F * r, (size_t)r * d.F, (size_t)d.D * r};
    auto fld = [&](const ta_lm_lora_grads& g, int k) -> float* {
      float* const f[8] = {g.dla_qkv, g.dlb_qkv, g.dla_o, g.dlb_o, g.dla_gu, g.dlb_gu, g.dla_d, g.dlb_d};
      return f[k];
    };
    bool stacked = true;
    for (int k = 0; k < 8 && stacked; ++k)
      for (int l = 1; l < NL; ++l)
        if (fld(lora_grads[l], k) != fld(lora_grads[0], k) + (size_t)l * sz[k]) { stacked = false; break; }
    lora_parts = stacked && s.lora_part && (r % 4 == 0);
    for (int k = 0; k < 8 && lora_parts; ++k) if (sz[k] != (size_t)s.lp_size[k]) lora_parts = false;
    if (stacked) {
      if (!lora_parts || lgm != 15)
        for (int k = 0; k < 8; ++k)
          if (hipMemsetAsync(fld(lora_grads[0], k), 0, sz[k] * NL * 4, st) != hipSuccess) return TA_ERR_LAUNCH;
    } else {
      for (int l = 0; l < NL; ++l) if (!zero_lora(lora_grads[l])) return TA_ERR_LAUNCH;
    }
  }
  if (n_lab <= 0) {
    if (d_embeds && hipMemsetAsync(d_embeds, 0, (size_t)M * d.D * 4, st) != hipSuccess) return TA_ERR_LAUNCH;
    return TA_OK;
  }
  ta_gemm_opts kx = opts_none();
  LoraDrop pend{};
  const bf16_t* pend_at = nullptr;
  auto lora_bwd = [&](const bf16_t* dy, int N, const bf16_t* x, int in, const bf16_t* xa, const LoraImg& g, float* dla,
                      float* dlb, int members, int b0, int b1, int layer, int grp) -> int {
    static const int lj_base[4] = {0, 3, 4, 6};
    RC(ta_i_lora_skinny_nt(dy, N, g.bt, s.dyB, M, members * r, st));
    float* pb = lora_parts ? s.lora_part + (long)layer * s.lp_layer + s.lp_off[2 * grp + 1] : nullptr;
    float* pa = lora_parts ? s.lora_part + (long)layer * s.lp_layer + s.lp_off[2 * grp] : nullptr;
    if (dp) {
      pend = LoraDrop{*dp, (unsigned)(8 * layer + lj_base[grp]), r, members};
      RC(ta_i_lora_skinny_tn2(dy, N, xa, members * r, dlb, r, 1, 1.0f, r, b0, b1, x, in, s.dyB, members * r, dla, 1, in,
                              w->lora_scale * dp->inv_keep, 0, 0, 0, M, pb, s.lp_size[2 * grp + 1], pa, s.lp_size[2 * grp], st, &pend));
      pend_at = g.at;
      return TA_OK;
    }
    RC(ta_i_lora_skinny_tn2(dy, N, xa, members * r, dlb, r, 1, 1.0f, r, b0, b1, x, in, s.dyB, members * r, dla, 1, in, w->lora_scale,
                            0, 0, 0, M, pb, s.lp_size[2 * grp + 1], pa, s.lp_size[2 * grp], st));
    kx = opts_kext(s.dyB, g.at);
    return TA_OK;
  };
  auto take_ext = [&]() { const ta_gemm_opts o = kx; kx = opts_none(); return o; };
  auto dx_drop_term = [&](void* out, int in) -> int {
    if (!pend_at) return TA_OK;
    const bf16_t* at = pend_at;
    pend_at = nullptr;
    return ta_i_lora_dx_drop(s.dyB, at, out, M, in, pend, st);
  };
  const int sp = pick_splits(n_lab, d.D, w->vocab_pad);
  RC(ta_gemm_bf16_nt(t.dlogits, w->embed_t_bf16, s.dhl, n_lab, d.D, w->vocab_pad, w->vocab_pad, 0, 0, d.D, 0, 0, 0, nullptr,
                     nullptr, 0, 0, sp, s.skws, st));
  if (hipMemsetAsync(s.dhn, 0, (size_t)M * d.D * 4, st) != hipSuccess) return TA_ERR_LAUNCH;
  RC(ta_scatter_rows_f32(s.dhl, label_rows, s.dhn, n_lab, d.D, st));
  const int Kp = pad64(M);
  auto wgrad = [&](const bf16_t* dy, int n_out, const bf16_t* x, int k_in, float* dW) -> int {
    if (!dW) return TA_OK;
    if (n_out <= 4096 && k_in <= 2048)
      return ta_gemm_bf16_tn(dy, x, dW, M, n_out, k_in, 1, s.wsk, ta_gemm_bf16_tn_ws_bytes(M, n_out, k_in), st);
    RC(ta_transpose_to_bf16(dy, 0, n_out, 0, 0, s.tA, Kp, M, n_out, st));
    RC(ta_transpose_to_bf16(x, 0, k_in, 0, 0, s.tB, Kp, M, k_in, st));
    return ta_gemm_bf16_nt(s.tA, s.tB, dW, n_out, k_in, Kp, Kp, 0, 0, k_in, 0, 0, 0, nullptr, dW, 0, 0,
                           wgrad_splits(n_out, k_in, Kp), s.wsk, st);
  };
  if (wg) {
    if (wg->dembed) {
      const int Kl = pad64(n_lab);
      RC(ta_gather_rows_bf16(t.hn, label_rows, s.hl, n_lab, d.D, st));
      RC(ta_transpose_to_bf16(t.dlogits, 0, w->vocab_pad, 0, 0, s.tA, Kl, n_lab, w->vocab_pad, st));
      RC(ta_transpose_to_bf16(s.hl, 0, d.D, 0, 0, s.tB, Kl, n_lab, d.D, st));
      RC(ta_gemm_bf16_nt(s.tA, s.tB, wg->dembed, w->vocab, d.D, Kl, Kl, 0, 0, d.D, 0, 0, 0, nullptr, wg->dembed, 0, 0, 1,
                         nullptr, st));
    }
    if (wg->dnorm) RC(ta_rmsnorm_dw(s.dhn, 0, t.x_final, lm_res_bf16(w), t.r_f, wg->dnorm, M, d.D, st));
  }
  float* dx = s.dxa;
  float* dx_alt = s.dxb32;
  const int gb = 1;
  const bool dx_bf16 = lm_res_bf16(w) && w->dx_f32 == 0;
  auto norm_bwd = [&](const float* dy, int dyb, const float* x, const float* r, const float* gw, const float* dres, float* dxf,
                      bool last = false) -> int {
    if (dx_bf16) return ta_rmsnorm_bwd_bf16s(dy, dyb, x, r, gw, dres ? s.dxb : nullptr, last ? dxf : nullptr, s.dxb, M, d.D, st);
    if (lm_res_bf16(w)) return ta_rmsnorm_bwd_bf16(dy, dyb, x, r, gw, dres, dxf, s.dxb, M, d.D, st);
    return dyb ? ta_rmsnorm_bwd_dyb(dy, x, r, gw, dres, dxf, s.dxb, M, d.D, st)
               : ta_rmsnorm_bwd(dy, x, r, gw, dres, dxf, s.dxb, nullptr, M, d.D, 0, st);
  };
  RC(norm_bwd(s.dhn, 0, t.x_final, t.r_f, w->norm_w, nullptr, dx, w->n_layers == 0));
  for (int l = w->n_layers - 1; l >= 0; --l) {
    const ta_lm_layer& Lw = w->layers[l];
    const LmLayerTape& p = store[l];
    if (lgm & 8) RC(lora_bwd(s.dxb, d.D, p.act_s, d.F, p.xa_d, p.i_d, lora_grads[l].dla_d, lora_grads[l].dlb_d, 1, 1 << 30, 1 << 30, l, 3));
    const ta_lm_layer_wgrads* g = wg ? &wg->layers[l] : nullptr;
    if (g) RC(wgrad(s.dxb, d.D, p.act_s, d.F, g->dwd));
    RC(gemm_opt(s.dxb, Lw.wd_t, s.dact, M, d.F, d.D, nullptr, nullptr, 0, 1, take_ext(), st));
    RC(dx_drop_term(s.dact, d.F));
    RC(ta_swiglu_bwd(s.dact, p.gu, s.dgu, M, d.F, st));
    if (lgm & 4) RC(lora_bwd(s.dgu, 2 * d.F, p.xn2_s, d.D, p.xa_gu, p.i_gu, lora_grads[l].dla_gu, lora_grads[l].dlb_gu, 2, d.F, 1 << 30, l, 2));
    if (g) RC(wgrad(s.dgu, 2 * d.F, p.xn2_s, d.D, g->dwgu));
    RC(gemm_opt(s.dgu, Lw.wgu_t, s.dxn, M, d.D, 2 * d.F, nullptr, nullptr, 0, gb, take_ext(), st));
    RC(dx_drop_term(s.dxn, d.D));
    if (g && g->dln_post) RC(ta_rmsnorm_dw(s.dxn, gb, p.x1, lm_res_bf16(w), p.r_post, g->dln_post, M, d.D, st));
    RC(norm_bwd(s.dxn, gb, p.x1, p.r_post, Lw.ln_post_w, dx, dx_alt));
    if (lgm & 2) RC(lora_bwd(s.dxb, d.D, p.ao, bq, p.xa_o, p.i_o, lora_grads[l].dla_o, lora_grads[l].dlb_o, 1, 1 << 30, 1 << 30, l, 1));
    if (g) RC(wgrad(s.dxb, d.D, p.ao, bq, g->dwo));
    RC(gemm_opt(s.dxb, Lw.wo_t, s.dao, M, d.nq * d.hd, d.D, nullptr, nullptr, 0, 1, take_ext(), st));
    RC(dx_drop_term(s.dao, d.nq * d.hd));
    RC(ta_attn_bwd_prep(s.dao, p.ao, s.delta, s.dot, B, d.nq, L, d.Lp, st));
    const bf16_t* v_hm = (w->train_base || !lm_attn_fused(d, L)) ? p.v : nullptr;
    if (seg && !(g && (g->dqn || g->dkn))) {
      RC(ta_attention_bwd_qkv_seg(p.q, p.k, v_hm, s.dao, (long)d.nq * d.hd, p.lse, s.delta, kmask, seg, p.qkv0, p.rq, p.rk, Lw.qn_w, Lw.kn_w,
                                  lm_rope_cos(w, l), lm_rope_sin(w, l), pos, s.dqkv, B, d.nq, d.nkv, L, d.Lp, scale, st));
    } else if (seg) {
      RC(ta_attention_bwd_seg(p.q, p.k, p.v, s.dao, (long)d.nq * d.hd, p.lse, s.delta, kmask, seg, s.dq, s.dk, s.dv, B, d.nq, d.nkv, L,
                              d.Lp, scale, st));
      RC(ta_lm_qkv_post_bwd(s.dq, s.dk, s.dv, p.qkv0, p.rq, p.rk, Lw.qn_w, Lw.kn_w, lm_rope_cos(w, l), lm_rope_sin(w, l), pos, s.dqkv,
                            g ? g->dqn : nullptr, g ? g->dkn : nullptr, B, d.nq, d.nkv, L, st));
    } else if (!(g && (g->dqn || g->dkn))) {
      RC(ta_attention_bwd_qkv(p.q, p.k, (w->train_base || !lm_attn_fused(d, L)) ? p.v : nullptr, s.dao, (long)d.nq * d.hd, p.lse, s.delta, kmask, p.qkv0, p.rq, p.rk, Lw.qn_w, Lw.kn_w,
                              lm_rope_cos(w, l), lm_rope_sin(w, l), pos, s.dqkv, B, d.nq, d.nkv, L, d.Lp, d.hd, 1, scale, st));
    } else {
      RC(ta_attention_bwd(p.q, p.qt, p.k, p.kt, p.v, s.dao, (long)d.nq * d.hd, s.dot, p.lse, s.delta, kmask, s.dq, s.dk, s.dv,
                          B, d.nq, d.nkv, L, d.Lp, d.hd, 1, scale, st));
      RC(ta_lm_qkv_post_bwd(s.dq, s.dk, s.dv, p.qkv0, p.rq, p.rk, Lw.qn_w, Lw.kn_w, lm_rope_cos(w, l), lm_rope_sin(w, l), pos, s.dqkv,
                            g ? g->dqn : nullptr, g ? g->dkn : nullptr, B, d.nq, d.nkv, L, st));
    }
    if (g) RC(wgrad(s.dqkv, d.NQKV, p.xn_s, d.D, g->dwqkv));
    if (lgm & 1) RC(lora_bwd(s.dqkv, d.NQKV, p.xn_s, d.D, p.xa_qkv, p.i_qkv, lora_grads[l].dla_qkv, lora_grads[l].dlb_qkv, 3, bq, bk, l, 0));
    RC(gemm_opt(s.dqkv, Lw.wqkv_t, s.dxn, M, d.D, d.NQKV, nullptr, nullptr, 0, gb, take_ext(), st));
    RC(dx_drop_term(s.dxn, d.D));
    if (g && g->dln_in) RC(ta_rmsnorm_dw(s.dxn, gb, p.x_in, lm_res_bf16(w), p.r_in, g->dln_in, M, d.D, st));
    RC(norm_bwd(s.dxn, gb, p.x_in, p.r_in, Lw.ln_in_w, dx_alt, dx, l == 0));
  }
  if (d_embeds && hipMemcpyAsync(d_embeds, dx, (size_t)M * d.D * 4, hipMemcpyDeviceToDevice, st) != hipSuccess)
    return TA_ERR_LAUNCH;
  if (d_audio && src_row) RC(ta_audio_grad_gather(src_row, dx, d_audio, M, d.D, st));
  if (wg && wg->dembed) RC(ta_embed_grad_scatter(ids, src_row, dx, wg->dembed, M, d.D, w->vocab, st));
  if (lora_parts) {
    LoraReduceDesc rd;
    float* const f0[8] = {lora_grads[0].dla_qkv, lora_grads[0].dlb_qkv, lora_grads[0].dla_o, lora_grads[0].dlb_o,
                          lora_grads[0].dla_gu, lora_grads[0].dlb_gu, lora_grads[0].dla_d, lora_grads[0].dlb_d};
    for (int k = 0; k < 8; ++k) {
      const bool on = (lgm >> (k >> 1)) & 1;
      rd.out[k] = f0[k]; rd.out_ls[k] = s.lp_size[k]; rd.size[k] = on ? s.lp_size[k] : 0; rd.part_off[k] = s.lp_off[k];
      rd.chunks[k] = s.lp_chunks[k];
    }
    rd.part = s.lora_part; rd.part_ls = s.lp_layer;
    RC(ta_i_lora_reduce_parts(rd, w->n_layers, st));
  }
  return TA_OK;
}

extern "C" int ta_lm_backward(const ta_lm_weights* w, const int* src_row, const int* kmask, const int* pos, int B, int L,
                              const int* label_rows, int n_lab, float* d_audio, long n_audio_rows, float* d_embeds,
                              const ta_lm_lora_grads* lora_grads, const ta_lm_wgrads* wg, const long* ids, const void* tape,
                              void* ws, long ws_bytes, hipStream_t st) {
  return lm_backward_impl(w, src_row, kmask, pos, nullptr, B, L, label_rows, n_lab, d_audio, n_audio_rows, d_embeds, lora_grads, wg, ids,
                          tape, ws, ws_bytes, nullptr, st);
}
extern "C" int ta_lm_backward_ex(const ta_lm_weights* w, const int* src_row, const int* kmask, const int* pos, int B, int L,
                                 const int* label_rows, int n_lab, float* d_audio, long n_audio_rows, float* d_embeds,
                                 const ta_lm_lora_grads* lora_grads, const ta_lm_wgrads* wg, const long* ids, const void* tape,
                                 void* ws, long ws_bytes, const ta_lora_dropout* drop, hipStream_t st) {
  return lm_backward_impl(w, src_row, kmask, pos, nullptr, B, L, label_rows, n_lab, d_audio, n_audio_rows, d_embeds, lora_grads, wg, ids,
                          tape, ws, ws_bytes, drop, st);
}
extern "C" int ta_lm_backward_seg(const ta_lm_weights* w, const int* src_row, const int* kmask, const int* pos, const int* seg, int B,
                                  int L, const int* label_rows, int n_lab, float* d_audio, long n_audio_rows, float* d_embeds,
                                  const ta_lm_lora_grads* lora_grads, const ta_lm_wgrads* wg, const long* ids, const void* tape,
                                  void* ws, long ws_bytes, const ta_lora_dropout* drop, hipStream_t st) {
  return lm_backward_impl(w, src_row, kmask, pos, seg, B, L, label_rows, n_lab, d_audio, n_audio_rows, d_embeds, lora_grads, wg, ids,
                          tape, ws, ws_bytes, drop, st);
}
```

### tiny_audio_amd/csrc/elementwise.hip

```cpp
#include "common.h"
#include "internal.h"

static inline int ew_blocks(long n, int per_block = 256) {
  long b = (n + per_block - 1) / per_block;
  return (int)(b > 4096 ? 4096 : (b < 1 ? 1 : b));
}

__global__ void swiglu_fwd_kernel(const bf16_t* __restrict__ gu, bf16_t* __restrict__ act, long M, int F) {
  const long n4 = M * (F / 4);
  for (long i = (long)blockIdx.x * blockDim.x + threadIdx.x; i < n4; i += (long)gridDim.x * blockDim.x) {
    const long m = i / (F / 4); const int c = (int)(i % (F / 4)) * 4;
    const uint2 gv = *(const uint2*)(gu + m * 2 * F + c);
    const uint2 uv = *(const uint2*)(gu + m * 2 * F + F + c);
    const float g[4] = {bf2f(gv.x & 0xffff), bf2f(gv.x >> 16), bf2f(gv.y & 0xffff), bf2f(gv.y >> 16)};
    const float u[4] = {bf2f(uv.x & 0xffff), bf2f(uv.x >> 16), bf2f(uv.y & 0xffff), bf2f(uv.y >> 16)};
    float a[4];
#pragma unroll
    for (int j = 0; j < 4; ++j) a[j] = g[j] / (1.f + __expf(-g[j])) * u[j];
    uint2 o; o.x = pack2bf(a[0], a[1]); o.y = pack2bf(a[2], a[3]);
    *(uint2*)(act + m * F + c) = o;
  }
}
__global__ void swiglu_bwd_kernel(const bf16_t* __restrict__ dact, const bf16_t* __restrict__ gu,
                                  bf16_t* __restrict__ dgu, long M, int F) {
// ... 35 lines not shown
  const int tx = threadIdx.x & 63, ty = threadIdx.x >> 6;
  for (int i = ty; i < 64; i += 4) {
    const int r = r0 + i, c = c0 + tx;
    bf16_t v = 0;
    if (r < R && c < C) {
      const long off = (long)(r / in_rpb) * in_bs + (long)(r % in_rpb) * ld_in + c;
      if constexpr (sizeof(T) == 4) v = f2bf(((const float*)in)[off]); else v = ((const bf16_t*)in)[off];
    }
    tile[i][tx] = v;
  }
  __syncthreads();
  for (int i = ty; i < 64; i += 4) {
    const int c = c0 + i, r = r0 + tx;
    if (c < C && r < ld_out) out[(long)c * ld_out + r] = tile[tx][i];
  }
}

template <typename T>
__global__ __launch_bounds__(256) void transpose_to_bf16_vec_kernel(const T* __restrict__ in, long ld_in, long in_bs, int in_rpb,
                                                                    bf16_t* __restrict__ out, long ld_out, int R, int C) {
  constexpr int P = 72;
  __shared__ __attribute__((aligned(16))) bf16_t tile[64 * P];
  const int r0 = blockIdx.y * 64, c0 = blockIdx.x * 64, tid = threadIdx.x;
#pragma unroll
  for (int it = 0; it < 2; ++it) {
    const int ch = tid + it * 256, r = ch >> 3, cc = ch & 7;
    const int gr = r0 + r, gc = c0 + cc * 8;
    uint4 v = make_uint4(0, 0, 0, 0);
    if (gr < R && gc < C) {
      const long off = (long)(gr / in_rpb) * in_bs + (long)(gr % in_rpb) * ld_in + gc;
      if constexpr (sizeof(T) == 4) {
        const float4 a = *(const float4*)((const float*)in + off), b = *(const float4*)((const float*)in + off + 4);
        v = make_uint4(pack2bf(a.x, a.y), pack2bf(a.z, a.w), pack2bf(b.x, b.y), pack2bf(b.z, b.w));
      } else {
        v = *(const uint4*)((const bf16_t*)in + off);
      }
    }
    *(uint4*)(tile + r * P + cc * 8) = v;
  }
  __syncthreads();
#pragma unroll
  for (int it = 0; it < 2; ++it) {
    const int ch = tid + it * 256, c = ch >> 3, rc = ch & 7;
    const int gc = c0 + c, gr = r0 + rc * 8;
    if (gc < C && gr < ld_out) {
      union { uint4 v; bf16_t e[8]; } u;
#pragma unroll
      for (int j = 0; j < 8; ++j) u.e[j] = tile[(rc * 8 + j) * P + c];
      *(uint4*)(out + (long)gc * ld_out + gr) = u.v;
    }
  }
}

__global__ __launch_bounds__(256) void feats_to_tm_kernel(const float* __restrict__ f, bf16_t* __restrict__ out, int C, int T) {
  __shared__ float tile[64][65];
  const int b = blockIdx.z, t0 = blockIdx.x * 64, c0 = blockIdx.y * 64;
  const int tx = threadIdx.x & 63, ty = threadIdx.x >> 6;
  for (int i = ty; i < 64; i += 4) {
    const int c = c0 + i, t = t0 + tx;
    tile[i][tx] = (c < C && t < T) ? f[((long)b * C + c) * T + t] : 0.f;
  }
  __syncthreads();
  for (int i = ty; i < 64; i += 4) {
    const int t = t0 + i, c = c0 + tx;
    if (t < T && c < C) out[((long)b * (T + 2) + t + 1) * C + c] = f2bf(tile[tx][i]);
  }
  if (blockIdx.x == 0 && ty == 0 && c0 + tx < C) {
    out[((long)b * (T + 2)) * C + c0 + tx] = 0;
    out[((long)b * (T + 2) + T + 1) * C + c0 + tx] = 0;
  }
}
__global__ void zero_pad_rows_kernel(bf16_t* __restrict__ buf, int T, int C) {
  const int b = blockIdx.x;
  for (int c = threadIdx.x; c < C; c += blockDim.x) {
    buf[((long)b * (T + 2)) * C + c] = 0;
    buf[((long)b * (T + 2) + T + 1) * C + c] = 0;
  }
}

__global__ __launch_bounds__(256) void feats_to_tm_len_kernel(const float* __restrict__ f, bf16_t* __restrict__ out, int C, int T, int b0,
                                                              RaggedLens lens) {
  __shared__ float tile[64][65];
  const int b = b0 + blockIdx.z, t0 = blockIdx.x * 64, c0 = blockIdx.y * 64;
  const int Tb = lens.len[blockIdx.z];
  const int tx = threadIdx.x & 63, ty = threadIdx.x >> 6;
  for (int i = ty; i < 64; i += 4) {
    const int c = c0 + i, t = t0 + tx;
    float v = 0.f;
    if (c < C && t < Tb) v = f[((long)b * C + c) * T + t];
    tile[i][tx] = v;
  }
  __syncthreads();
  for (int i = ty; i < 64; i += 4) {
    const int t = t0 + i, c = c0 + tx;
    if (t < T && c < C) out[((long)b * (T + 2) + t + 1) * C + c] = f2bf(tile[tx][i]);
  }
  if (blockIdx.x == 0 && ty == 0 && c0 + tx < C) {
    out[((long)b * (T + 2)) * C + c0 + tx] = 0;
    out[((long)b * (T + 2) + T + 1) * C + c0 + tx] = 0;
  }
}
__global__ __launch_bounds__(256) void zero_tail_rows_kernel(bf16_t* __restrict__ buf, int T, int C, int b0, RaggedLens lens) {
  const int b = b0 + blockIdx.y, Tb = lens.len[blockIdx.y];
  const int cpr = C / 8;
  const long ntail = (long)(T + 1 - Tb) * cpr;
  uint4* base = (uint4*)(buf + (long)b * (T + 2) * C);
  const uint4 z = make_uint4(0, 0, 0, 0);
  for (long i = (long)blockIdx.x * 256 + threadIdx.x; i < ntail; i += (long)gridDim.x * 256) base[(long)(Tb + 1) * cpr + i] = z;
  if (blockIdx.x == 0) for (int i = threadIdx.x; i < cpr; i += 256) base[i] = z;
}
__device__ __forceinline__ int clip_of_row(const int* __restrict__ cu, int B, int m) {
  int lo = 0, hi = B;
  while (hi - lo > 1) { const int mid = (lo + hi) >> 1; if (cu[mid] <= m) lo = mid; else hi = mid; }
  return lo;
}
__global__ __launch_bounds__(256) void compact_rows_kernel(const char* __restrict__ src, char* __restrict__ dst,
                                                           const int* __restrict__ cu, int B, int S, int rows, int row_bytes) {
  const int m = blockIdx.x * 4 + (threadIdx.x >> 6);
  if (m >= rows) return;
  const int b = clip_of_row(cu, B, m), s = m - cu[b];
  if (s < 0 || s >= S) return;
  const uint4* in = (const uint4*)(src + ((long)b * S + s) * row_bytes);
  uint4* out = (uint4*)(dst + (long)m * row_bytes);
  for (int c = threadIdx.x & 63; c < row_bytes / 16; c += 64) out[c] = in[c];
}
__global__ __launch_bounds__(256) void rope_rows_kernel(const float* __restrict__ rope_il, float* __restrict__ tab,
                                                        const int* __restrict__ cu, int B, int rows, int max_pos) {
  const int m = blockIdx.x * 32 + (threadIdx.x >> 3);
  if (m >= rows) return;
  int pos = m - cu[clip_of_row(cu, B, m)];
  pos = pos < 0 ? 0 : (pos < max_pos ? pos : max_pos - 1);
  ((float4*)(tab + (long)m * 32))[threadIdx.x & 7] = ((const float4*)(rope_il + (long)pos * 32))[threadIdx.x & 7];
}
__global__ __launch_bounds__(256) void expand_rows_kernel(const bf16_t* __restrict__ yb, const float* __restrict__ yf,
                                                          bf16_t* __restrict__ ob, float* __restrict__ of, const int* __restrict__ cu,
                                                          const float* __restrict__ keep, int B, int S, int rows, int H) {
  const long p = (long)blockIdx.x * 4 + (threadIdx.x >> 6);
  if (p >= (long)B * S) return;
  const int b = (int)(p / S), s = (int)(p % S);
  const int c0 = cu[b], Sb = cu[b + 1] - c0;
  const long m = (long)c0 + s;
  const bool real = s < Sb && c0 >= 0 && m < rows && (!keep || keep[p] != 0.f);
  const int lane = threadIdx.x & 63;
  if (ob) for (int c = lane; c < H / 8; c += 64)
    ((uint4*)(ob + p * H))[c] = real ? ((const uint4*)(yb + m * H))[c] : make_uint4(0, 0, 0, 0);
  if (of) for (int c = lane; c < H / 4; c += 64)
    ((float4*)(of + p * H))[c] = real ? ((const float4*)(yf + m * H))[c] : make_float4(0.f, 0.f, 0.f, 0.f);
}

template <bool F32>
__global__ __launch_bounds__(256) void pos_add_kernel(void* __restrict__ xv, const float* __restrict__ pos, long n_chunks, long per_clip) {
  for (long i = (long)blockIdx.x * blockDim.x + threadIdx.x; i < n_chunks; i += (long)gridDim.x * blockDim.x) {
    const long j = i % per_clip;
    if constexpr (F32) {
      float4 v = ((const float4*)xv)[i];
      const float4 p = ((const float4*)pos)[j];
      v.x += p.x; v.y += p.y; v.z += p.z; v.w += p.w;
      ((float4*)xv)[i] = v;
    } else {
      const uint4 v = ((const uint4*)xv)[i];
      const float4 p0 = ((const float4*)pos)[2 * j], p1 = ((const float4*)pos)[2 * j + 1];
      uint4 o;
      o.x = pack2bf(bf2f(v.x & 0xffff) + p0.x, bf2f(v.x >> 16) + p0.y);
      o.y = pack2bf(bf2f(v.y & 0xffff) + p0.z, bf2f(v.y >> 16) + p0.w);
      o.z = pack2bf(bf2f(v.z & 0xffff) + p1.x, bf2f(v.z >> 16) + p1.y);
      o.w = pack2bf(bf2f(v.w & 0xffff) + p1.z, bf2f(v.w >> 16) + p1.w);
      ((uint4*)xv)[i] = o;
    }
  }
}
extern "C" int ta_pos_add(void* x, int x_f32, const float* pos, int B, int S, int H, hipStream_t st) {
  if (B <= 0 || S <= 0) return TA_OK;
  if (!x || !pos || H <= 0 || (H % 8)) return TA_ERR_ARG;
  const long per_clip = (long)S * H / (x_f32 ? 4 : 8), n = per_clip * B;
  if (x_f32) TA_LAUNCH((pos_add_kernel<true>), dim3(ew_blocks(n)), dim3(256), 0, st, x, pos, n, per_clip);
  else TA_LAUNCH((pos_add_kernel<false>), dim3(ew_blocks(n)), dim3(256), 0, st, x, pos, n, per_clip);
  TA_CHECK_LAUNCH(); return TA_OK;
}

__global__ __launch_bounds__(1024) void audio_index_kernel(const long* __restrict__ ids, const long* __restrict__ counts,
                                                           int* __restrict__ src_row, int B, int L, int N, long audio_id) {
  __shared__ int scan[1024];
  __shared__ int carry;
  __shared__ long cum[1025];
  const int tid = threadIdx.x;
  if (tid == 0) {
    carry = 0; cum[0] = 0;
    for (int i = 0; i < B && i < 1024; ++i) cum[i + 1] = cum[i] + counts[i];
  }
  __syncthreads();
  const int total = B * L;
  for (int base = 0; base < total; base += 1024) {
    const int p = base + tid;
    const int flag = (p < total && ids[p] == audio_id) ? 1 : 0;
    scan[tid] = flag;
    __syncthreads();
    for (int o = 1; o < 1024; o <<= 1) {
      const int v = tid >= o ? scan[tid - o] : 0;
      __syncthreads();
      scan[tid] += v;
      __syncthreads();
    }
    if (p < total) {
      int out = -1;
      if (flag) {
        const long rank = carry + scan[tid] - 1;
        int lo = 0, hi = B;
        while (hi - lo > 1) { const int mid = (lo + hi) >> 1; if (cum[mid] <= rank) lo = mid; else hi = mid; }
        const long n = rank - cum[lo];
        out = (rank < cum[B] && n < N) ? (int)(lo * N + n) : -2;
      }
      src_row[p] = out;
    }
    __syncthreads();
    if (tid == 1023) carry += scan[1023];
    __syncthreads();
  }
}
__global__ __launch_bounds__(256) void segment_table_kernel(const int* __restrict__ sid, int* __restrict__ seg_start,
                                                            int* __restrict__ seg_end, int* __restrict__ pos, int R, int L) {
  const long p = (long)blockIdx.x * 256 + threadIdx.x;
  if (p >= (long)R * L) return;
  const int l = (int)(p % L);
  const int* row = sid + (p - l);
  const int s = row[l];
  int a = l, e = l + 1;
  if (s == 0) { a = l + 1; e = l; }
  else {
    while (a > 0 && row[a - 1] == s) --a;
    while (e < L && row[e] == s) ++e;
  }
  seg_start[p] = a;
  seg_end[p] = e;
  if (pos) pos[p] = s == 0 ? 0 : l - a;
}
__global__ __launch_bounds__(256) void audio_index_seg_kernel(const long* __restrict__ ids, const int* __restrict__ sid,
                                                              const long* __restrict__ counts, int* __restrict__ src_row, int R, int L,
                                                              int C_, int N, long audio_id) {
  __shared__ int clip0;
  const int r = blockIdx.x;
  if (threadIdx.x == 0) {
    int c = 0;
    for (int i = 0; i < r; ++i) { int m = 0; for (int l = 0; l < L; ++l) m = max(m, sid[(long)i * L + l]); c += m; }
    clip0 = c;
  }
  __syncthreads();
  const int* srow = sid + (long)r * L;
  const long* irow = ids + (long)r * L;
  for (int l = threadIdx.x; l < L; l += 256) {
    int out = -1;
    const int s = srow[l];
    if (s > 0 && irow[l] == audio_id) {
      int j = 0;
      for (int k = l - 1; k >= 0 && srow[k] == s; --k) j += irow[k] == audio_id;
      const int c = clip0 + s - 1;
      out = (c < C_ && j < N && j < counts[c]) ? c * N + j : -2;
    }
    src_row[(long)r * L + l] = out;
  }
}
__global__ __launch_bounds__(256) void embed_scatter_kernel(const long* __restrict__ ids, const int* __restrict__ src_row,
                                                            const float* __restrict__ emb, const float* __restrict__ audio,
                                                            float* __restrict__ x0, bf16_t* __restrict__ x0b, int n_rows, int D,
                                                            long vocab) {
  const int row = blockIdx.x * 4 + (threadIdx.x >> 6);
  if (row >= n_rows) return;
  const int lane = threadIdx.x & 63;
  const int s = src_row ? src_row[row] : -1;
  long id = ids[row]; if (id < 0) id = 0; if (id >= vocab) id = vocab - 1;
  const float4* src = s >= 0 ? (const float4*)(audio + (long)s * D) : (const float4*)(emb + id * D);
  for (int c = lane; c < D / 4; c += 64) {
    const float4 v = (s == -2) ? make_float4(0.f, 0.f, 0.f, 0.f) : src[c];
    if (x0) ((float4*)(x0 + (long)row * D))[c] = v;
    if (x0b) { uint2 o; o.x = pack2bf(v.x, v.y); o.y = pack2bf(v.z, v.w); ((uint2*)(x0b + (long)row * D))[c] = o; }
  }
}
__global__ __launch_bounds__(256) void audio_grad_gather_kernel(const int* __restrict__ src_row, const float* __restrict__ dx0,
                                                                float* __restrict__ d_audio, int n_rows, int D) {
  const int row = blockIdx.x * 4 + (threadIdx.x >> 6);
  if (row >= n_rows) return;
  const int s = src_row[row];
  if (s < 0) return;
  const int lane = threadIdx.x & 63;
  for (int c = lane; c < D / 4; c += 64) ((float4*)(d_audio + (long)s * D))[c] = ((const float4*)(dx0 + (long)row * D))[c];
}

__global__ __launch_bounds__(256) void gather_rows_bf16_kernel(const bf16_t* __restrict__ in, const int* __restrict__ idx,
                                                               bf16_t* __restrict__ out, int n, int D) {
  const int row = blockIdx.x * 4 + (threadIdx.x >> 6);
  if (row >= n) return;
  const int lane = threadIdx.x & 63;
  const long s = idx[row];
  for (int c = lane; c < D / 8; c += 64) ((uint4*)(out + (long)row * D))[c] = ((const uint4*)(in + s * D))[c];
}
__global__ __launch_bounds__(256) void scatter_rows_f32_kernel(const float* __restrict__ in, const int* __restrict__ idx,
                                                               float* __restrict__ out, int n, int D) {
  const int row = blockIdx.x * 4 + (threadIdx.x >> 6);
  if (row >= n) return;
  const int lane = threadIdx.x & 63;
  const long s = idx[row];
  for (int c = lane; c < D / 4; c += 64) ((float4*)(out + s * D))[c] = ((const float4*)(in + (long)row * D))[c];
}

__global__ void bernoulli_keep_kernel(float* __restrict__ keep, long n, float keep_prob, unsigned long long seed) {
  for (long i = (long)blockIdx.x * blockDim.x + threadIdx.x; i < n; i += (long)gridDim.x * blockDim.x) {
    unsigned long long z = seed + 0x9E3779B97F4A7C15ull * (unsigned long long)(i + 1);
    z = (z ^ (z >> 30)) * 0xBF58476D1CE4E5B9ull;
    z = (z ^ (z >> 27)) * 0x94D049BB133111EBull;
    z = z ^ (z >> 31);
    const float u = (float)(z >> 40) * (1.0f / 16777216.0f);
    keep[i] = u < keep_prob ? 1.f : 0.f;
  }
}

extern "C" int ta_swiglu_fwd(const void* gu, void* act, long M, int F, hipStream_t st) {
  if (M <= 0) return TA_OK;
  if (F % 4) return TA_ERR_ARG;
  TA_LAUNCH(swiglu_fwd_kernel, dim3(ew_blocks(M * (F / 4))), dim3(256), 0, st, (const bf16_t*)gu, (bf16_t*)act, M, F);
  TA_CHECK_LAUNCH(); return TA_OK;
}
extern "C" int ta_swiglu_bwd(const void* dact, const void* gu, void* dgu, long M, int F, hipStream_t st) {
  if (M <= 0) return TA_OK;
  if (F % 4) return TA_ERR_ARG;
  TA_LAUNCH(swiglu_bwd_kernel, dim3(ew_blocks(M * (F / 4))), dim3(256), 0, st, (const bf16_t*)dact,
                     (const bf16_t*)gu, (bf16_t*)dgu, M, F);
  TA_CHECK_LAUNCH(); return TA_OK;
}
extern "C" int ta_cast_f32_bf16(const float* x, void* y, long n, hipStream_t st) {
  if (n <= 0) return TA_OK;
  if (n % 4) return TA_ERR_ARG;
  TA_LAUNCH(cast_f32_bf16_kernel, dim3(ew_blocks(n / 4)), dim3(256), 0, st, x, (bf16_t*)y, n / 4);
  TA_CHECK_LAUNCH(); return TA_OK;
}
extern "C" int ta_transpose_to_bf16(const void* in, int in_is_f32, long ld_in, long in_bs, int in_rpb, void* out,
                                    long ld_out, int R, int C, hipStream_t st) {
  if (R <= 0 || C <= 0) return TA_OK;
  if (ld_out < R) return TA_ERR_ARG;
  dim3 grid(ta_cdiv(C, 64), ta_cdiv(ld_out, 64));
  if (in_rpb <= 0) in_rpb = R;
  if (!((ld_in | in_bs | (long)C | ld_out) & 7) && !(((uintptr_t)in | (uintptr_t)out) & 15)) {
    if (in_is_f32)
      TA_LAUNCH((transpose_to_bf16_vec_kernel<float>), grid, dim3(256), 0, st, (const float*)in, ld_in, in_bs, in_rpb,
                (bf16_t*)out, ld_out, R, C);
    else
      TA_LAUNCH((transpose_to_bf16_vec_kernel<bf16_t>), grid, dim3(256), 0, st, (const bf16_t*)in, ld_in, in_bs, in_rpb,
                (bf16_t*)out, ld_out, R, C);
    TA_CHECK_LAUNCH(); return TA_OK;
  }
  if (in_is_f32)
    TA_LAUNCH((transpose_to_bf16_kernel<float>), grid, dim3(256), 0, st, (const float*)in, ld_in, in_bs, in_rpb,
                       (bf16_t*)out, ld_out, R, C);
  else
    TA_LAUNCH((transpose_to_bf16_kernel<bf16_t>), grid, dim3(256), 0, st, (const bf16_t*)in, ld_in, in_bs, in_rpb,
                       (bf16_t*)out, ld_out, R, C);
  TA_CHECK_LAUNCH(); return TA_OK;
}
extern "C" int ta_feats_to_time_major(const float* feats, void* out, int B, int C, int T, hipStream_t st) {
  if (B <= 0 || T <= 0) return TA_OK;
  TA_LAUNCH(feats_to_tm_kernel, dim3(ta_cdiv(T, 64), ta_cdiv(C, 64), B), dim3(256), 0, st, feats, (bf16_t*)out, C, T);
  TA_CHECK_LAUNCH(); return TA_OK;
}
extern "C" int ta_zero_pad_rows(void* buf, int B, int T, int C, hipStream_t st) {
  if (B <= 0) return TA_OK;
  TA_LAUNCH(zero_pad_rows_kernel, dim3(B), dim3(256), 0, st, (bf16_t*)buf, T, C);
  TA_CHECK_LAUNCH(); return TA_OK;
}
int ta_i_feats_to_time_major_len(const float* feats, void* out, int B, int C, int T, const int* len_host, hipStream_t st) {
  for (int b0 = 0; b0 < B; b0 += RAGGED_CHUNK) {
    const int n = B - b0 < RAGGED_CHUNK ? B - b0 : RAGGED_CHUNK;
    RaggedLens l;
    for (int i = 0; i < RAGGED_CHUNK; ++i) l.len[i] = i < n ? len_host[b0 + i] : 0;
    TA_LAUNCH(feats_to_tm_len_kernel, dim3(ta_cdiv(T, 64), ta_cdiv(C, 64), n), dim3(256), 0, st, feats, (bf16_t*)out, C, T, b0, l);
    TA_CHECK_LAUNCH();
  }
  return TA_OK;
}
int ta_i_zero_tail_rows(void* buf, int B, int T, int C, const int* len_host, hipStream_t st) {
  if (C % 8) return TA_ERR_ARG;
  for (int b0 = 0; b0 < B; b0 += RAGGED_CHUNK) {
    const int n = B - b0 < RAGGED_CHUNK ? B - b0 : RAGGED_CHUNK;
    RaggedLens l;
    for (int i = 0; i < RAGGED_CHUNK; ++i) l.len[i] = i < n ? len_host[b0 + i] : T;
    TA_LAUNCH(zero_tail_rows_kernel, dim3(8, n), dim3(256), 0, st, (bf16_t*)buf, T, C, b0, l);
    TA_CHECK_LAUNCH();
  }
  return TA_OK;
}
int ta_i_compact_rows(const void* src, void* dst, const int* cu, int B, int S, int rows, int row_bytes, hipStream_t st) {
  if (row_bytes % 16) return TA_ERR_ARG;
  TA_LAUNCH(compact_rows_kernel, dim3(ta_cdiv(rows, 4)), dim3(256), 0, st, (const char*)src, (char*)dst, cu, B, S, rows, row_bytes);
  TA_CHECK_LAUNCH(); return TA_OK;
}
int ta_i_rope_rows(const float* rope_il, float* tab, const int* cu, int B, int rows, int max_pos, hipStream_t st) {
  TA_LAUNCH(rope_rows_kernel, dim3(ta_cdiv(rows, 32)), dim3(256), 0, st, rope_il, tab, cu, B, rows, max_pos);
  TA_CHECK_LAUNCH(); return TA_OK;
}
int ta_i_expand_rows(const void* y_bf16, const float* y_f32, void* out_bf16, float* out_f32, const int* cu, const float* keep, int B,
                     int S, int rows, int H, hipStream_t st) {
  if (H % 8) return TA_ERR_ARG;
  TA_LAUNCH(expand_rows_kernel, dim3((unsigned)(((long)B * S + 3) / 4)), dim3(256), 0, st, (const bf16_t*)y_bf16, y_f32,
            (bf16_t*)out_bf16, out_f32, cu, keep, B, S, rows, H);
  TA_CHECK_LAUNCH(); return TA_OK;
}
extern "C" int ta_audio_index(const long* ids, const long* counts, int* src_row, int B, int L, int N, long audio_id,
                              hipStream_t st) {
  if (B <= 0 || L <= 0) return TA_OK;
  if (B > 1024) return TA_ERR_ARG;
  TA_LAUNCH(audio_index_kernel, dim3(1), dim3(1024), 0, st, ids, counts, src_row, B, L, N, audio_id);
  TA_CHECK_LAUNCH(); return TA_OK;
}
extern "C" int ta_segment_table(const int* segment_ids, int* seg, int* pos, int R, int L, hipStream_t st) {
  if (R <= 0 || L <= 0) return TA_OK;
  if (!segment_ids || !seg) return TA_ERR_ARG;
  const long n = (long)R * L;
  TA_LAUNCH(segment_table_kernel, dim3((unsigned)((n + 255) / 256)), dim3(256), 0, st, segment_ids, seg, seg + n, pos, R, L);
  TA_CHECK_LAUNCH(); return TA_OK;
}
extern "C" int ta_audio_index_seg(const long* ids, const int* segment_ids, const long* counts, int* src_row, int R, int L, int C,
                                  int N, long audio_id, hipStream_t st) {
  if (R <= 0 || L <= 0) return TA_OK;
  if (!ids || !segment_ids || !counts || !src_row || C < 0) return TA_ERR_ARG;
  TA_LAUNCH(audio_index_seg_kernel, dim3(R), dim3(256), 0, st, ids, segment_ids, counts, src_row, R, L, C, N, audio_id);
  TA_CHECK_LAUNCH(); return TA_OK;
}
extern "C" int ta_embed_scatter(const long* ids, const int* src_row, const float* emb, const float* audio, float* x0,
                                void* x0_bf16, int n_rows, int D, long vocab, hipStream_t st) {
  if (n_rows <= 0) return TA_OK;
  if (D % 4) return TA_ERR_ARG;
  TA_LAUNCH(embed_scatter_kernel, dim3(ta_cdiv(n_rows, 4)), dim3(256), 0, st, ids, src_row, emb, audio, x0,
                     (bf16_t*)x0_bf16, n_rows, D, vocab);
  TA_CHECK_LAUNCH(); return TA_OK;
}
extern "C" int ta_audio_grad_gather(const int* src_row, const float* dx0, float* d_audio, int n_rows, int D, hipStream_t st) {
  if (n_rows <= 0) return TA_OK;
  if (D % 4) return TA_ERR_ARG;
  TA_LAUNCH(audio_grad_gather_kernel, dim3(ta_cdiv(n_rows, 4)), dim3(256), 0, st, src_row, dx0, d_audio, n_rows, D);
  TA_CHECK_LAUNCH(); return TA_OK;
}
__global__ __launch_bounds__(256) void embed_grad_scatter_kernel(const long* __restrict__ ids, const int* __restrict__ src_row,
                                                                 const float* __restrict__ dx0, float* __restrict__ dembed,
                                                                 int n_rows, int D, long vocab) {
  const int row = blockIdx.x * 4 + (threadIdx.x >> 6), lane = threadIdx.x & 63;
  if (row >= n_rows) return;
  if (src_row && src_row[row] != -1) return;
  const long id = ids[row];
  if (id < 0 || id >= vocab) return;
  for (int c = lane * 4; c < D; c += 256) {
    const float4 g = *(const float4*)(dx0 + (long)row * D + c);
    float* dst = dembed + id * D + c;
    unsafeAtomicAdd(dst, g.x); unsafeAtomicAdd(dst + 1, g.y); unsafeAtomicAdd(dst + 2, g.z); unsafeAtomicAdd(dst + 3, g.w);
  }
}
extern "C" int ta_embed_grad_scatter(const long* ids, const int* src_row, const float* dx0, float* dembed, int n_rows, int D,
                                     long vocab, hipStream_t st) {
  if (n_rows <= 0) return TA_OK;
  if (D % 4) return TA_ERR_ARG;
  TA_LAUNCH(embed_grad_scatter_kernel, dim3(ta_cdiv(n_rows, 4)), dim3(256), 0, st, ids, src_row, dx0, dembed, n_rows, D, vocab);
  TA_CHECK_LAUNCH(); return TA_OK;
}
extern "C" int ta_gather_rows_bf16(const void* in, const int* idx, void* out, int n, int D, hipStream_t st) {
  if (n <= 0) return TA_OK;
  if (D % 8) return TA_ERR_ARG;
  TA_LAUNCH(gather_rows_bf16_kernel, dim3(ta_cdiv(n, 4)), dim3(256), 0, st, (const bf16_t*)in, idx, (bf16_t*)out, n, D);
  TA_CHECK_LAUNCH(); return TA_OK;
}
extern "C" int ta_scatter_rows_f32(const float* in, const int* idx, float* out, int n, int D, hipStream_t st) {
  if (n <= 0) return TA_OK;
  if (D % 4) return TA_ERR_ARG;
  TA_LAUNCH(scatter_rows_f32_kernel, dim3(ta_cdiv(n, 4)), dim3(256), 0, st, in, idx, out, n, D);
  TA_CHECK_LAUNCH(); return TA_OK;
}
extern "C" int ta_bernoulli_keep(float* keep, long n, float keep_prob, unsigned long long seed, hipStream_t st) {
  if (n <= 0) return TA_OK;
  TA_LAUNCH(bernoulli_keep_kernel, dim3(ew_blocks(n)), dim3(256), 0, st, keep, n, keep_prob, seed);
  TA_CHECK_LAUNCH(); return TA_OK;
}

__global__ __launch_bounds__(256) void occupy_kernel(uint4* __restrict__ buf, long n16, long ticks) {
  const unsigned long long t0 = wall_clock64();
  long i = (long)blockIdx.x * 256 + threadIdx.x;
  const long stride = (long)gridDim.x * 256;
  uint4 acc = make_uint4(0, 0, 0, 0);
  while ((long)(wall_clock64() - t0) < ticks) {
#pragma unroll 4
    for (int u = 0; u < 16; ++u) {
      if (i >= n16) i -= (i / n16) * n16;
      const uint4 v = buf[i];
      acc.x ^= v.x; acc.y ^= v.y; acc.z ^= v.z; acc.w ^= v.w;
      buf[i] = v;
      i += stride;
    }
  }
  if (acc.x == 0x12345678u && acc.y == 0x9abcdef0u) buf[0] = acc;
}
extern "C" int ta_debug_occupy(int workgroups, double micros, void* buf, long bytes, hipStream_t st) {
  if (workgroups <= 0 || micros <= 0 || !buf || bytes < 4096) return TA_ERR_ARG;
  int dev = 0, rate_khz = 0;
  (void)hipGetDevice(&dev);
  (void)hipDeviceGetAttribute(&rate_khz, hipDeviceAttributeWallClockRate, dev);
  if (rate_khz <= 0) rate_khz = 100000;
  TA_LAUNCH(occupy_kernel, dim3(workgroups), dim3(256), 0, st, (uint4*)buf, bytes / 16, (long)(micros * rate_khz / 1000.0));
  TA_CHECK_LAUNCH(); return TA_OK;
}
```

### tiny_audio_amd/csrc/generate.hip

```cpp
#include <cstdlib>
#include "host_util.h"
#include "internal.h"
#include "philox.h"

static bool read_decode_fused() { const char* e = getenv("TA355_DECODE_FUSED"); return !(e && *e == '0'); }
static bool g_decode_fused = read_decode_fused();
static const bool g_decode_prefetch = true;
static const int g_decode_pf_wgs = 0;
static bool read_scores_split() { const char* e = getenv("TA355_SCORES_SPLIT"); return !(e && *e == '0'); }
static bool g_scores_split = read_scores_split();
void ta_i_reload_decode_knobs() { g_decode_fused = read_decode_fused(); g_scores_split = read_scores_split(); }

namespace {
constexpr int HD = 128;

template <bool NORM, bool ROPE>
__global__ __launch_bounds__(64) void lm_qkv_post_decode_kernel(const bf16_t* __restrict__ qkv0, const float* __restrict__ qn_w,
                                                                const float* __restrict__ kn_w, const float* __restrict__ cosT,
                                                                const float* __restrict__ sinT, const int* __restrict__ pos,
                                                                const int* __restrict__ slot_p, bf16_t* __restrict__ q_out,
                                                                bf16_t* __restrict__ kc, bf16_t* __restrict__ vc, int Hq, int Hkv,
                                                                int Lmax, float eps) {
  const int lane = threadIdx.x, hh = blockIdx.x, b = blockIdx.y;
  const int sec = hh < Hq ? 0 : (hh < Hq + Hkv ? 1 : 2);
  const int head = sec == 0 ? hh : (sec == 1 ? hh - Hq : hh - Hq - Hkv);
  const long ld = (long)(Hq + 2 * Hkv) * HD;
  const bf16_t* src = qkv0 + (long)b * ld + (long)hh * HD;
  float y1 = bf2f(src[lane]), y2 = bf2f(src[lane + 64]);
  if ((NORM || ROPE) && sec < 2) {
    float n1 = y1, n2 = y2;
    if constexpr (NORM) {
      const float* nw = sec == 0 ? qn_w : kn_w;
      const float r = rsqrtf(wave_sum(y1 * y1 + y2 * y2) / (float)HD + eps);
      n1 = y1 * r * nw[lane]; n2 = y2 * r * nw[lane + 64];
    }
    if constexpr (ROPE) {
      const int p = pos[b];
      const float c = cosT[(long)p * 64 + lane], s = sinT[(long)p * 64 + lane];
      y1 = n1 * c - n2 * s;
      y2 = n2 * c + n1 * s;
    } else {
      y1 = n1; y2 = n2;
    }
  }
  bf16_t* dst;
  if (sec == 0) dst = q_out + ((long)b * Hq + head) * HD;
  else dst = (sec == 1 ? kc : vc) + (((long)b * Hkv + head) * Lmax + *slot_p) * HD;
  dst[lane] = f2bf(y1);
  dst[lane + 64] = f2bf(y2);
}

__global__ __launch_bounds__(256) void attn_decode_kernel(const bf16_t* __restrict__ q, const bf16_t* __restrict__ kc,
                                                          const bf16_t* __restrict__ vc, const int* __restrict__ kmask,
                                                          const int* __restrict__ slot_p, bf16_t* __restrict__ out, int Hq,
                                                          int Hkv, int Lmax, float scale) {
  extern __shared__ float sm[];
  float* sc = sm;
  float* qs = sm + Lmax;
  float* red = qs + HD;
  float* oh = red + 8;
  const int tid = threadIdx.x, lane = tid & 63, wave = tid >> 6;
  const int h = blockIdx.x, b = blockIdx.y, hk = h / (Hq / Hkv);
  const int n = *slot_p + 1;
  if (tid < HD) qs[tid] = bf2f(q[((long)b * Hq + h) * HD + tid]);
  __syncthreads();
  const bf16_t* K = kc + ((long)b * Hkv + hk) * Lmax * HD;
  const bf16_t* V = vc + ((long)b * Hkv + hk) * Lmax * HD;
  float mx = -INFINITY;
  for (int j = tid; j < n; j += 256) {
    float s = -INFINITY;
    if (kmask[(long)b * Lmax + j]) {
      const uint4* kr = (const uint4*)(K + (long)j * HD);
      float acc = 0.f;
#pragma unroll
      for (int c = 0; c < HD / 8; ++c) {
        const uint4 v = kr[c];
        const uint32_t u[4] = {v.x, v.y, v.z, v.w};
#pragma unroll
        for (int e = 0; e < 4; ++e)
          acc += bf2f((bf16_t)(u[e] & 0xffff)) * qs[c * 8 + 2 * e] + bf2f((bf16_t)(u[e] >> 16)) * qs[c * 8 + 2 * e + 1];
      }
      s = acc * scale;
    }
    sc[j] = s;
    mx = fmaxf(mx, s);
  }
  mx = wave_max(mx);
  if (lane == 0) red[wave] = mx;
  __syncthreads();
  mx = fmaxf(fmaxf(red[0], red[1]), fmaxf(red[2], red[3]));
  float sum = 0.f;
  for (int j = tid; j < n; j += 256) {
    const float p = sc[j] == -INFINITY ? 0.f : __expf(sc[j] - mx);
    sc[j] = p;
    sum += p;
  }
  sum = wave_sum(sum);
  if (lane == 0) red[4 + wave] = sum;
  __syncthreads();
  const float inv = 1.0f / (red[4] + red[5] + red[6] + red[7]);
  const int dc = tid & 15, kg = tid >> 4;
  float o[8] = {0.f, 0.f, 0.f, 0.f, 0.f, 0.f, 0.f, 0.f};
#pragma unroll 4
  for (int j = kg; j < n; j += 16) {
    const float p = sc[j];
    const uint4 v = *(const uint4*)(V + (long)j * HD + dc * 8);
    const uint32_t u[4] = {v.x, v.y, v.z, v.w};
#pragma unroll
    for (int e = 0; e < 4; ++e) {
      o[2 * e] += p * bf2f((bf16_t)(u[e] & 0xffff));
      o[2 * e + 1] += p * bf2f((bf16_t)(u[e] >> 16));
    }
  }
#pragma unroll
  for (int e = 0; e < 8; ++e) oh[kg * HD + dc * 8 + e] = o[e];
  __syncthreads();
  if (tid < HD) {
    float t = 0.f;
#pragma unroll
    for (int k = 0; k < 16; ++k) t += oh[k * HD + tid];
    out[((long)b * Hq + h) * HD + tid] = f2bf(t * inv);
  }
}

__global__ __launch_bounds__(1024) void argmax_rows_kernel(const float* __restrict__ x, long ld, int n, long* __restrict__ out) {
  __shared__ float bv[16];
  __shared__ int bi[16];
  const float* row = x + (long)blockIdx.x * ld;
  float best = -INFINITY; int idx = 0x7fffffff;
  auto take = [&](float v, int j) { if (v > best || (v == best && j < idx)) { best = v; idx = j; } };
  const bool vec = (((size_t)row) & 15) == 0;
  const int n4 = vec ? n / 4 : 0;
  for (int q = threadIdx.x; q < n4; q += 1024) {
    const float4 v = ((const float4*)row)[q];
    take(v.x, 4 * q); take(v.y, 4 * q + 1); take(v.z, 4 * q + 2); take(v.w, 4 * q + 3);
  }
  for (int j = n4 * 4 + threadIdx.x; j < n; j += 1024) take(row[j], j);
#pragma unroll
  for (int o = 32; o > 0; o >>= 1) {
    const float ov = __shfl_xor(best, o, 64); const int oi = __shfl_xor(idx, o, 64);
    if (ov > best || (ov == best && oi < idx)) { best = ov; idx = oi; }
  }
  if ((threadIdx.x & 63) == 0) { bv[threadIdx.x >> 6] = best; bi[threadIdx.x >> 6] = idx; }
  __syncthreads();
  if (threadIdx.x == 0) {
    for (int w = 1; w < 16; ++w)
      if (bv[w] > best || (bv[w] == best && bi[w] < idx)) { best = bv[w]; idx = bi[w]; }
    out[blockIdx.x] = idx == 0x7fffffff ? 0 : idx;
  }
}

#define LP_MAXSEQ 8192
__global__ __launch_bounds__(1024) void logits_process_kernel(float* __restrict__ logits, long ld, int V, const long* __restrict__ prompt,
                                                              int L, const long* __restrict__ out_seq, int max_new,
                                                              const int* __restrict__ step_p, float penalty, int ngram) {
  __shared__ float val[LP_MAXSEQ];
  const int b = blockIdx.x, t = *step_p, n = L + (t < max_new ? t : max_new);
  float* row = logits + (long)b * ld;
  const long* pr = prompt + (long)b * L;
  const long* gen = out_seq + (long)b * max_new;
  auto tok = [&](int i) -> long { return i < L ? pr[i] : gen[i - L]; };
  if (penalty != 1.0f) {
    for (int i = threadIdx.x; i < n; i += blockDim.x) {
      const long id = tok(i);
      float sc = 0.f;
      if (id >= 0 && id < V) { sc = row[id]; sc = sc < 0.f ? sc * penalty : sc / penalty; }
      val[i] = sc;
    }
    __syncthreads();
    for (int i = threadIdx.x; i < n; i += blockDim.x) {
      const long id = tok(i);
      if (id >= 0 && id < V) row[id] = val[i];
    }
    __syncthreads();
  }
  if (ngram > 0 && n + 1 >= ngram) {
    const int pre = ngram - 1;
    for (int i = threadIdx.x; i + pre < n; i += blockDim.x) {
      bool same = true;
      for (int j = 0; j < pre; ++j) same &= tok(i + j) == tok(n - pre + j);
      const long id = tok(i + pre);
      if (same && id >= 0 && id < V) row[id] = -INFINITY;
    }
  }
}

__global__ void greedy_advance_kernel(const long* __restrict__ amax, const long* __restrict__ eos, int n_eos, long pad_id,
                                      int* __restrict__ finished, long* __restrict__ next_ids, long* __restrict__ out_seq,
                                      int max_new, int* __restrict__ step_p, int* __restrict__ slot_p, int* __restrict__ pos,
                                      int* __restrict__ kmask, int Lmax, int B, int* __restrict__ n_unfinished) {
  __shared__ int alive;
  const int t = *step_p, slot = *slot_p;
  if (threadIdx.x == 0) alive = 0;
  __syncthreads();
  for (int b = threadIdx.x; b < B; b += blockDim.x) {
    long tok = finished[b] ? pad_id : amax[b];
    if (t < max_new) out_seq[(long)b * max_new + t] = tok;
    int fin = finished[b];
    for (int e = 0; e < n_eos; ++e) fin |= (tok == eos[e]);
    finished[b] = fin;
    next_ids[b] = tok;
    if (t > 0) pos[b] += 1;
    const int ns = t > 0 ? slot + 1 : slot;
    if (ns < Lmax) kmask[(long)b * Lmax + ns] = 1;
    if (!fin) atomicAdd(&alive, 1);
  }
  __syncthreads();
  if (threadIdx.x == 0) { *step_p = t + 1; *slot_p = t > 0 ? slot + 1 : slot; *n_unfinished = alive; }
}

typedef __attribute__((ext_vector_type(8))) short gbf16x8;
typedef __attribute__((ext_vector_type(4))) float gf32x4;
template <bool OUT_BF16, int CB>
__global__ __launch_bounds__(512) void linear_small_m_kernel(const bf16_t* __restrict__ X, const bf16_t* __restrict__ W,
                                                             void* __restrict__ out, const float* __restrict__ res, int M,
                                                             int N, int K, const bf16_t* __restrict__ A2,
                                                             const bf16_t* __restrict__ W2) {
  constexpr int COLS = CB * 16, UN = 4;
  __shared__ float red[8][32][COLS + 1];
  const int tid = threadIdx.x, wave = tid >> 6, lane = tid & 63, i = lane & 15, g = lane >> 4;
  const int n0 = blockIdx.x * COLS;
  gf32x4 acc[2][CB];
#pragma unroll
  for (int a = 0; a < 2; ++a)
#pragma unroll
    for (int b = 0; b < CB; ++b) acc[a][b] = (gf32x4){0.f, 0.f, 0.f, 0.f};
  const int ra = min(i, M - 1), rb = min(16 + i, M - 1);
  const bf16_t* xa = X + (long)ra * K + g * 8;
  const bf16_t* xb = X + (long)rb * K + g * 8;
  const bf16_t* wp[CB];
#pragma unroll
  for (int cb = 0; cb < CB; ++cb) wp[cb] = W + (long)min(n0 + cb * 16 + i, N - 1) * K + g * 8;
  const bool two = M > 16;
  for (int k0 = wave * 32; k0 < K; k0 += 256 * UN) {
    gbf16x8 a0[UN], a1[UN], b[UN][CB];
#pragma unroll
    for (int u = 0; u < UN; ++u) {
      const int kk = k0 + u * 256;
      if (kk < K) {
        a0[u] = *(const gbf16x8*)(xa + kk);
        a1[u] = two ? *(const gbf16x8*)(xb + kk) : a0[u];
#pragma unroll
        for (int cb = 0; cb < CB; ++cb) b[u][cb] = *(const gbf16x8*)(wp[cb] + kk);
      }
    }
#pragma unroll
    for (int u = 0; u < UN; ++u) {
      if (k0 + u * 256 < K) {
#pragma unroll
        for (int cb = 0; cb < CB; ++cb) {
          acc[0][cb] = __builtin_amdgcn_mfma_f32_16x16x32_bf16(a0[u], b[u][cb], acc[0][cb], 0, 0, 0);
          if (two) acc[1][cb] = __builtin_amdgcn_mfma_f32_16x16x32_bf16(a1[u], b[u][cb], acc[1][cb], 0, 0, 0);
        }
      }
    }
  }
  if (A2 && wave < 2) {
    const int kk = wave * 32 + g * 8;
    const gbf16x8 a0 = *(const gbf16x8*)(A2 + (long)ra * 64 + kk), a1 = *(const gbf16x8*)(A2 + (long)rb * 64 + kk);
#pragma unroll
    for (int cb = 0; cb < CB; ++cb) {
      const gbf16x8 b = *(const gbf16x8*)(W2 + (long)min(n0 + cb * 16 + i, N - 1) * 64 + kk);
      acc[0][cb] = __builtin_amdgcn_mfma_f32_16x16x32_bf16(a0, b, acc[0][cb], 0, 0, 0);
      acc[1][cb] = __builtin_amdgcn_mfma_f32_16x16x32_bf16(a1, b, acc[1][cb], 0, 0, 0);
    }
  }
#pragma unroll
  for (int rbk = 0; rbk < 2; ++rbk)
#pragma unroll
    for (int cb = 0; cb < CB; ++cb)
#pragma unroll
      for (int q = 0; q < 4; ++q) red[wave][rbk * 16 + g * 4 + q][cb * 16 + i] = acc[rbk][cb][q];
  __syncthreads();
  for (int e = tid; e < M * COLS; e += 512) {
    const int row = e / COLS, col = e % COLS, n = n0 + col;
    if (n >= N) continue;
    float v = 0.f;
#pragma unroll
    for (int w = 0; w < 8; ++w) v += red[w][row][col];
    if (res) v += res[(long)row * N + n];
    if (OUT_BF16) ((bf16_t*)out)[(long)row * N + n] = f2bf(v);
    else ((float*)out)[(long)row * N + n] = v;
  }
}

int linear_small_m(const bf16_t* X, const bf16_t* W, void* out, int M, int N, int K, const float* res, bool out_bf16,
                   const bf16_t* A2, const bf16_t* W2, hipStream_t st) {
  if (M > 32 || K % 32) return TA_ERR_ARG;
  const bool narrow = N <= 2048;
  const dim3 grid(ta_cdiv(N, narrow ? 16 : 64));
  if (out_bf16) {
    if (narrow) TA_LAUNCH((linear_small_m_kernel<true, 1>), grid, dim3(512), 0, st, X, W, out, res, M, N, K, A2, W2);
    else TA_LAUNCH((linear_small_m_kernel<true, 4>), grid, dim3(512), 0, st, X, W, out, res, M, N, K, A2, W2);
  } else {
    if (narrow) TA_LAUNCH((linear_small_m_kernel<false, 1>), grid, dim3(512), 0, st, X, W, out, res, M, N, K, A2, W2);
    else TA_LAUNCH((linear_small_m_kernel<false, 4>), grid, dim3(512), 0, st, X, W, out, res, M, N, K, A2, W2);
  }
  TA_CHECK_LAUNCH();
  return TA_OK;
}

struct DecodeWs {
  float *x, *x1, *r, *logits_unused;
  bf16_t *xn, *qkv0, *q, *ao, *gu, *act, *xa, *hn;
  size_t bytes;
};
DecodeWs decode_ws(const ta_lm_weights* w, int B, void* base) {
  const int D = w->hidden, F = w->ffn, bq = w->heads * HD, NQKV = (w->heads + 2 * w->kv_heads) * HD;
  Carver c(base);
  DecodeWs s;
  const size_t Bp = B < 32 ? 32 : B;
  s.x = c.take<float>(Bp * D); s.x1 = c.take<float>(Bp * D); s.r = c.take<float>((size_t)B);
  s.xn = c.take<bf16_t>((size_t)B * D); s.qkv0 = c.take<bf16_t>((size_t)B * NQKV); s.q = c.take<bf16_t>((size_t)B * bq);
  s.ao = c.take<bf16_t>(Bp * bq); s.gu = c.take<bf16_t>((size_t)B * 2 * F); s.act = c.take<bf16_t>(Bp * F);
// ... 785 lines not shown
```

### tiny_audio_amd/ops.py

```python
from __future__ import annotations

import ctypes as C

import torch

from . import _lib
from ._lib import check, lib

BF16 = torch.bfloat16
F32 = torch.float32


def ptr(t):
    return None if t is None else C.c_void_p(t.data_ptr())


def stream():
    if _lib.DRY_RUN:
        return None
    return C.c_void_p(torch.cuda.current_stream().cuda_stream)


def _req(t, dtype=None):
    assert (t.is_cuda or _lib.DRY_RUN) and t.is_contiguous(), "ta355 ops need contiguous CUDA(HIP) tensors"
    if dtype is not None:
        assert t.dtype == dtype, (t.dtype, dtype)
    return t


_KNOB_KEYS = ("TA355_GEMM_VARIANT", "TA355_GELU_LUT", "TA355_DECODE_FUSED", "TA355_SCORES_SPLIT")
_knob_state = None


def sync_gemm_knobs():
    global _knob_state
    import os
    cur = tuple(os.environ.get(k) for k in _KNOB_KEYS)
    if cur != _knob_state:
        if _knob_state is not None or any(v is not None for v in cur):
            lib().ta_gemm_reload_knobs()
        _knob_state = cur


def gemm_nt(A, W, M=None, N=None, K=None, *, out=None, out_dtype=BF16, bias=None, residual=None, act=0,
            a_map=None, c_map=None, splits=1, k_ext=None, residual_bf16=None, rope=None, w_blocked=False):
    _req(A, BF16); _req(W, BF16)
    sync_gemm_knobs()
    opts = None
    if residual_bf16 is not None or k_ext is not None or rope is not None or w_blocked:
        from ._lib import GemmOpts
        opts = GemmOpts()
        opts.w_blocked = int(bool(w_blocked))
        if rope is not None:
            _req(rope[0], F32)
            opts.rope_tab, opts.rope_rows = ptr(rope[0]), int(rope[1])
            opts.rope_cols = int(rope[2]) if len(rope) > 2 else 0
        if residual_bf16 is not None:
            _req(residual_bf16, BF16)
            opts.residual_bf16 = ptr(residual_bf16)
        if k_ext is not None:
            A2, W2 = k_ext
            _req(A2, BF16); _req(W2, BF16)
            opts.a2, opts.w2, opts.k2, opts.lda2 = ptr(A2), ptr(W2), W2.shape[1], A2.shape[1]
    N = N or W.shape[0]
    K = K or W.shape[1]
    M = M or A.numel() // K
    lda, a_rpb, a_bs = a_map or (K, 0, 0)
    ldc, c_rpb, c_bs, c_off = c_map or (N, 0, 0, 0)
    if out is None:
        out = torch.empty((M, N), device=A.device, dtype=out_dtype)
    ws = None
    if splits > 1:
        ws = torch.empty(lib().ta_gemm_splitk_ws_bytes(M, N, splits) // 4, device=A.device, dtype=F32)
    import ctypes as _C
    check(lib().ta_gemm_bf16_nt_opt(ptr(A), ptr(W), ptr(out), M, N, K, lda, a_rpb, a_bs, ldc, c_rpb, c_bs, c_off,
                                    ptr(bias), ptr(residual), act, 1 if out.dtype == BF16 else 0, splits, ptr(ws),
                                    None, None, None, None if opts is None else _C.addressof(opts), stream()), "ta_gemm_bf16_nt_opt")
    return out


def gemm_tn(Y, X, out=None, accumulate=False):
    _req(Y, BF16); _req(X, BF16)
    M, Ny = Y.shape
    Nx = X.shape[1]
    if out is None:
        out = torch.zeros((Ny, Nx), device=Y.device, dtype=F32)
        accumulate = False
    ws = torch.empty(max(lib().ta_gemm_bf16_tn_ws_bytes(M, Ny, Nx), 16), device=Y.device, dtype=torch.uint8)
    check(lib().ta_gemm_bf16_tn(ptr(Y), ptr(X), ptr(out), M, Ny, Nx, int(bool(accumulate)), ptr(ws), ws.numel(), stream()),
          "ta_gemm_bf16_tn")
    return out


def gemm_nt_grouped(A, W, out, M, N, K, *, seg=None, krange=None, n_groups=1, bias=None, act=0, a_idx=None, w_stride=0, c_stride=0):
    _req(A, BF16); _req(W, BF16)
    sync_gemm_knobs()
    check(lib().ta_gemm_bf16_nt_grouped(ptr(A), ptr(W), ptr(out), M, N, K, ptr(bias), act, int(out.dtype == BF16), ptr(a_idx),
                                        ptr(seg), ptr(krange), n_groups, w_stride, c_stride, stream()), "ta_gemm_bf16_nt_grouped")
    return out


def layernorm(x, w, b, eps=1e-5, rowscale=None, out_bf16=True, out_f32=False):
    if x.dtype == BF16:
        M, H = x.shape
        yb = torch.empty((M, H), device=x.device, dtype=BF16) if out_bf16 else None
        yf = torch.empty((M, H), device=x.device, dtype=F32) if out_f32 else None
        check(lib().ta_layernorm_bf16(ptr(x), ptr(w), ptr(b), ptr(yb), ptr(yf), ptr(rowscale), M, H, eps, stream()),
              "ta_layernorm_bf16")
        return yb, yf
    _req(x, F32)
    M, H = x.shape
    yb = torch.empty((M, H), device=x.device, dtype=BF16) if out_bf16 else None
    yf = torch.empty((M, H), device=x.device, dtype=F32) if out_f32 else None
    check(lib().ta_layernorm_f32(ptr(x), ptr(w), ptr(b), ptr(yb), ptr(yf), ptr(rowscale), M, H, eps, stream()),
          "ta_layernorm_f32")
    return yb, yf


def rmsnorm_fwd(x, w, eps=1e-6, act_gelu=False, out_bf16=True, out_f32=False):
    M, H = x.shape
    yb = torch.empty((M, H), device=x.device, dtype=BF16) if out_bf16 else None
    yf = torch.empty((M, H), device=x.device, dtype=F32) if out_f32 else None
    r = torch.empty(M, device=x.device, dtype=F32)
    if x.dtype == BF16:
        assert not act_gelu
        check(lib().ta_rmsnorm_fwd_bf16(ptr(x), ptr(w), ptr(yb), ptr(yf), ptr(r), M, H, eps, stream()), "ta_rmsnorm_fwd_bf16")
        return yb, yf, r
    _req(x, F32)
    check(lib().ta_rmsnorm_fwd(ptr(x), ptr(w), ptr(yb), ptr(yf), ptr(r), M, H, eps, int(act_gelu), stream()),
          "ta_rmsnorm_fwd")
    return yb, yf, r


def rmsnorm_bwd(dy, x, rstd, w, dres=None, act_gelu=False, want_dw=False, out_bf16=True):
    if x.dtype != BF16:
        _req(dy, F32)
    M, H = x.shape
    dx = torch.empty((M, H), device=x.device, dtype=F32)
    dxb = torch.empty((M, H), device=x.device, dtype=BF16) if out_bf16 else None
    if x.dtype == BF16:
        assert not act_gelu and not want_dw
        check(lib().ta_rmsnorm_bwd_bf16(ptr(dy), int(dy.dtype == BF16), ptr(x), ptr(rstd), ptr(w), ptr(dres), ptr(dx), ptr(dxb), M, H, stream()),
              "ta_rmsnorm_bwd_bf16")
        return dx, dxb, None
    _req(x, F32)
    dw = torch.zeros(H, device=x.device, dtype=F32) if want_dw else None
    check(lib().ta_rmsnorm_bwd(ptr(dy), ptr(x), ptr(rstd), ptr(w), ptr(dres), ptr(dx), ptr(dxb), ptr(dw), M, H,
                               int(act_gelu), stream()), "ta_rmsnorm_bwd")
    return dx, dxb, dw


def pad64(n):
    return (n + 63) // 64 * 64


def _out(out, shape, device, dtype=BF16):
    if out is None:
        return torch.empty(shape, device=device, dtype=dtype)
    assert tuple(out.shape) == tuple(shape) and out.dtype == dtype
    return _req(out)


def attention_fwd(Q, K, VT, L, causal, scale, kmask=None, want_lse=True, out=None):
    B, Hq, _, hd = Q.shape
    Hkv, Lp = K.shape[1], VT.shape[3]
    O = _out(out, (B * L, Hq * hd), Q.device)
    lse = torch.empty((B, Hq, L), device=Q.device, dtype=F32) if want_lse else None
    check(lib().ta_attention_fwd(ptr(Q), ptr(K), ptr(VT), ptr(O), ptr(lse), ptr(kmask), B, Hq, Hkv, L, Lp, hd,
                                 int(causal), scale, stream()), "ta_attention_fwd")
    return O, lse


def attention_fwd_strided(Q, K, VT, B, Hq, Hkv, L, hd, causal, scale, layout, kmask=None):
    import ctypes as _C
    from ._lib import AttnLayout
    lay = AttnLayout(*[int(v) for v in layout])
    O = torch.empty((B * L, Hq * hd), device=Q.device, dtype=BF16)
    check(lib().ta_attention_fwd_ex(ptr(Q), ptr(K), ptr(VT), ptr(O), None, ptr(kmask), B, Hq, Hkv, L, pad64(L), hd,
                                    int(causal), scale, _C.addressof(lay), stream()), "ta_attention_fwd_ex")
    return O


def _out3(out, Q, K, V):
    if out is None:
        return torch.empty_like(Q), torch.empty_like(K), torch.empty_like(V)
    return tuple(_out(o, t.shape, t.device) for o, t in zip(out, (Q, K, V)))


def attention_bwd(Q, QT, K, KT, V, dO, dOT, lse, delta, L, causal, scale, kmask=None, out=None):
    B, Hq, _, hd = Q.shape
    Hkv, Lp = K.shape[1], (pad64(L) if KT is None else KT.shape[3])
    dQ, dK, dV = _out3(out, Q, K, V)
    check(lib().ta_attention_bwd(ptr(Q), ptr(QT), ptr(K), ptr(KT), ptr(V), ptr(dO), dO.shape[-1], ptr(dOT), ptr(lse),
                                 ptr(delta), ptr(kmask), ptr(dQ), ptr(dK), ptr(dV), B, Hq, Hkv, L, Lp, hd, int(causal),
                                 scale, stream()), "ta_attention_bwd")
    return dQ, dK, dV


def attention_enc_fwd(qkv, B, heads, S):
    _req(qkv, BF16)
    assert qkv.shape == (B * S, 3 * heads * 64)
    out = torch.empty((B * S, heads * 64), device=qkv.device, dtype=BF16)
    check(lib().ta_attention_enc_fwd(ptr(qkv), ptr(out), B, heads, S, stream()), "ta_attention_enc_fwd")
    return out


def attention_enc_fwd_varlen(qkv, cu_rows, heads, max_rows, out=None):
    _req(qkv, BF16)
    assert qkv.dim() == 2 and qkv.shape[1] == 3 * heads * 64
    assert cu_rows.dtype == torch.int32 and cu_rows.is_contiguous() and cu_rows.device == qkv.device
    if out is None:
        out = torch.empty((qkv.shape[0], heads * 64), device=qkv.device, dtype=BF16)
    check(lib().ta_attention_enc_fwd_varlen(ptr(qkv), ptr(out), ptr(cu_rows), cu_rows.numel() - 1, heads, int(max_rows), stream()),
          "ta_attention_enc_fwd_varlen")
    return out


def attention_fwd_seg(Q, K, VT, L, scale, kmask=None, seg=None, want_lse=True, out=None):
    B, Hq, _, hd = Q.shape
    Hkv, Lp = K.shape[1], VT.shape[3]
    assert hd == 128
    O = _out(out, (B * L, Hq * hd), Q.device)
    lse = torch.empty((B, Hq, L), device=Q.device, dtype=F32) if want_lse else None
    check(lib().ta_attention_fwd_seg(ptr(Q), ptr(K), ptr(VT), ptr(O), ptr(lse), ptr(kmask), ptr(seg), B, Hq, Hkv, L, Lp, scale,
                                     stream()), "ta_attention_fwd_seg")
    return O, lse


def attention_extend(Q, Kn, Vn, Kc, Vc, pmask, clip_of, lens, scale, want_lse=True, out=None):
    R, Hq, T, hd = Q.shape
    B, Hkv, Lmax, _ = Kc.shape
    assert hd == 128 and Kn.shape == (R, Hkv, T, hd) and Vn.shape == Kn.shape and Vc.shape == Kc.shape
    assert pmask.dtype == torch.int32 and pmask.dim() == 2 and pmask.shape[0] == B
    assert clip_of.dtype == torch.int32 and clip_of.numel() == R and lens.dtype == torch.int32 and lens.numel() == R
    for t in (Q, Kn, Vn, Kc, Vc, pmask, clip_of, lens):
        _req(t)
    O = _out(out, (R * T, Hq * hd), Q.device)
    lse = torch.empty((R, Hq, T), device=Q.device, dtype=F32) if want_lse else None
    check(lib().ta_attention_extend(ptr(Q), ptr(Kn), ptr(Vn), ptr(Kc), ptr(Vc), ptr(pmask), ptr(clip_of), ptr(lens), ptr(O), ptr(lse),
                                    B, R, Hq, Hkv, T, pmask.shape[1], Lmax, scale, stream()), "ta_attention_extend")
    return O, lse


def attention_bwd_seg(Q, K, V, dO, lse, delta, L, scale, kmask=None, seg=None, out=None):
    B, Hq, _, hd = Q.shape
    Hkv, Lp = K.shape[1], pad64(L)
    dQ, dK, dV = _out3(out, Q, K, V)
    check(lib().ta_attention_bwd_seg(ptr(Q), ptr(K), ptr(V), ptr(dO), dO.shape[-1], ptr(lse), ptr(delta), ptr(kmask), ptr(seg), ptr(dQ),
                                     ptr(dK), ptr(dV), B, Hq, Hkv, L, Lp, scale, stream()), "ta_attention_bwd_seg")
    return dQ, dK, dV


def attention_fwd_qkv(qkv0, qn_w, kn_w, cosT, sinT, B, Hq, Hkv, L, scale, eps=1e-6, kmask=None, pos=None, seg=None, out=None):
    hd, dev = 128, qkv0.device
    mk = lambda h: torch.empty((B, h, L, hd), device=dev, dtype=BF16)
    Q, K, V = mk(Hq), mk(Hkv), mk(Hkv)
    rq = torch.empty((B * L, Hq), device=dev, dtype=F32); rk = torch.empty((B * L, Hkv), device=dev, dtype=F32)
    O = _out(out, (B * L, Hq * hd), dev)
    lse = torch.empty((B, Hq, L), device=dev, dtype=F32)
    if seg is None:
        check(lib().ta_attention_fwd_qkv(ptr(qkv0), ptr(qn_w), ptr(kn_w), ptr(cosT), ptr(sinT), ptr(pos), ptr(Q), ptr(K), ptr(V), ptr(rq),
                                         ptr(rk), ptr(O), ptr(lse), ptr(kmask), B, Hq, Hkv, L, scale, eps, stream()), "ta_attention_fwd_qkv")
    else:
        check(lib().ta_attention_fwd_qkv_seg(ptr(qkv0), ptr(qn_w), ptr(kn_w), ptr(cosT), ptr(sinT), ptr(pos), ptr(Q), ptr(K), ptr(V), ptr(rq),
                                             ptr(rk), ptr(O), ptr(lse), ptr(kmask), ptr(seg), B, Hq, Hkv, L, scale, eps, stream()),
              "ta_attention_fwd_qkv_seg")
    return O, lse, Q, K, V, rq, rk


def attention_bwd_qkv(Q, K, V, dO, lse, delta, qkv0, rq, rk, qn_w, kn_w, cosT, sinT, L, scale, kmask=None, pos=None, seg=None, out=None):
    B, Hq, _, hd = Q.shape
    Hkv, Lp = K.shape[1], pad64(L)
    dqkv = _out(out, qkv0.shape, qkv0.device)
    if seg is None:
        check(lib().ta_attention_bwd_qkv(ptr(Q), ptr(K), ptr(V), ptr(dO), dO.shape[-1], ptr(lse), ptr(delta), ptr(kmask), ptr(qkv0),
                                         ptr(rq), ptr(rk), ptr(qn_w), ptr(kn_w), ptr(cosT), ptr(sinT), ptr(pos), ptr(dqkv), B, Hq, Hkv,
                                         L, Lp, hd, 1, scale, stream()), "ta_attention_bwd_qkv")
    else:
        check(lib().ta_attention_bwd_qkv_seg(ptr(Q), ptr(K), ptr(V), ptr(dO), dO.shape[-1], ptr(lse), ptr(delta), ptr(kmask), ptr(seg),
                                             ptr(qkv0), ptr(rq), ptr(rk), ptr(qn_w), ptr(kn_w), ptr(cosT), ptr(sinT), ptr(pos), ptr(dqkv),
                                             B, Hq, Hkv, L, Lp, scale, stream()), "ta_attention_bwd_qkv_seg")
    return dqkv


def lm_qkv_post_fwd(qkv0, qn_w, kn_w, cosT, sinT, B, Hq, Hkv, L, eps=1e-6, pos=None):
    hd, Lp, dev = 128, pad64(L), qkv0.device
    mk = lambda h: torch.empty((B, h, L, hd), device=dev, dtype=BF16)
    mkT = lambda h: torch.empty((B, h, hd, Lp), device=dev, dtype=BF16)
    Q, K, V, QT, KT, VT = mk(Hq), mk(Hkv), mk(Hkv), mkT(Hq), mkT(Hkv), mkT(Hkv)
    rq = torch.empty((B * L, Hq), device=dev, dtype=F32); rk = torch.empty((B * L, Hkv), device=dev, dtype=F32)
    check(lib().ta_lm_qkv_post_fwd(ptr(qkv0), ptr(qn_w), ptr(kn_w), ptr(cosT), ptr(sinT), ptr(pos), ptr(Q), ptr(K),
                                   ptr(V), ptr(QT), ptr(KT), ptr(VT), ptr(rq), ptr(rk), B, Hq, Hkv, L, Lp, eps,
                                   stream()), "ta_lm_qkv_post_fwd")
    return Q, K, V, QT, KT, VT, rq, rk


def lm_qkv_post_bwd(dQ, dK, dV, qkv0, rq, rk, qn_w, kn_w, cosT, sinT, B, Hq, Hkv, L, pos=None, dqn=None, dkn=None, out=None):
    dqkv = _out(out, qkv0.shape, qkv0.device)
    check(lib().ta_lm_qkv_post_bwd(ptr(dQ), ptr(dK), ptr(dV), ptr(qkv0), ptr(rq), ptr(rk), ptr(qn_w), ptr(kn_w),
                                   ptr(cosT), ptr(sinT), ptr(pos), ptr(dqkv), ptr(dqn), ptr(dkn), B, Hq, Hkv, L, stream()),
          "ta_lm_qkv_post_bwd")
    return dqkv


def rmsnorm_dw(dy, x, rstd, dw):
    M, H = x.shape
    check(lib().ta_rmsnorm_dw(ptr(dy), int(dy.dtype == BF16), ptr(x), int(x.dtype == BF16), ptr(rstd), ptr(dw), M, H, stream()),
          "ta_rmsnorm_dw")
    return dw


def embed_grad_scatter(ids, src_row, dx0, dembed):
    n, D = dx0.shape
    check(lib().ta_embed_grad_scatter(ptr(ids), ptr(src_row), ptr(dx0), ptr(dembed), n, D, dembed.shape[0], stream()),
          "ta_embed_grad_scatter")
    return dembed


def enc_qkv_post(qkv, cosT, sinT, B, H, S):
    Sp, dev = pad64(S), qkv.device
    Q = torch.empty((B, H, S, 64), device=dev, dtype=BF16); K = torch.empty_like(Q)
    VT = torch.empty((B, H, 64, Sp), device=dev, dtype=BF16)
    check(lib().ta_enc_qkv_post(ptr(qkv), ptr(cosT), ptr(sinT), ptr(Q), ptr(K), ptr(VT), B, H, S, Sp, stream()),
          "ta_enc_qkv_post")
    return Q, K, VT


def attn_bwd_prep(dO, O, B, Hq, L):
    Lp, dev = pad64(L), dO.device
    delta = torch.empty((B, Hq, L), device=dev, dtype=F32)
    dOT = torch.empty((B, Hq, 128, Lp), device=dev, dtype=BF16)
    check(lib().ta_attn_bwd_prep(ptr(dO), ptr(O), ptr(delta), ptr(dOT), B, Hq, L, Lp, stream()), "ta_attn_bwd_prep")
    return delta, dOT
# ... 962 lines not shown
```

Baseline: 7588.

## Restrict last LM layer's post-attention compute to label rows only

In the final LM layer, everything after attention (o-proj, post-norm, gate/up GEMM, SwiGLU, down GEMM, final norm) now runs only on the label rows. The rows are gathered right after attention, and in backward the gradients are scattered back to full rows before attention backward. This is exact because only label rows feed the loss, and it applies only when there is no LoRA, no base training, and labels cover at most half the rows. The cost is extra gather/scatter kernels and memsets, plus a larger tape and workspace.

```diff
diff --git a/include/ta355.h b/include/ta355.h
--- a/include/ta355.h
+++ b/include/ta355.h
@@ -409,6 +409,8 @@
                           hipStream_t st);
 int ta_gather_rows_bf16(const void* in, const int* idx, void* out, int n, int D, hipStream_t st);
 int ta_scatter_rows_f32(const float* in, const int* idx, float* out, int n, int D, hipStream_t st);
+int ta_gather_rows_f32(const float* in, const int* idx, float* out, int n, int D, hipStream_t st);
+int ta_scatter_rows_bf16(const void* in, const int* idx, void* out, int n, int D, hipStream_t st);
 int ta_bernoulli_keep(float* keep, long n, float keep_prob, unsigned long long seed, hipStream_t st);
 int ta_debug_occupy(int workgroups, double micros, void* buf, long bytes, hipStream_t st);
 
diff --git a/tiny_audio_amd/csrc/api.hip b/tiny_audio_amd/csrc/api.hip
--- a/tiny_audio_amd/csrc/api.hip
+++ b/tiny_audio_amd/csrc/api.hip
@@ -301,7 +301,17 @@
   return TA_OK;
 }
 
+static bool read_lm_top_rows() { const char* e = getenv("TA355_LM_TOP_ROWS"); return !(e && *e == '0'); }
+static bool g_lm_top_rows = read_lm_top_rows();
+void ta_i_reload_lm_knobs() { g_lm_top_rows = read_lm_top_rows(); }
 namespace {
+inline bool lm_top_rows(const ta_lm_weights* w, int B, int L, int n_lab) {
+  return g_lm_top_rows && w->lora_rank == 0 && !w->train_base && w->n_layers > 0 && n_lab > 0 && 2L * n_lab <= (long)B * L;
+}
+inline int lm_top_tape_rows(const ta_lm_weights* w, int B, int L, int n_lab) {
+  if (!g_lm_top_rows || w->lora_rank != 0 || w->train_base || w->n_layers <= 0 || n_lab <= 0) return 0;
+  return (int)std::min((long)n_lab, (long)B * L / 2);
+}
 inline bool lm_res_bf16(const ta_lm_weights* w) { return w->res_f32 == 0; }
 struct LmLayerTape {
   float *x_in, *r_in, *rq, *rk, *lse, *x1, *r_post;
@@ -309,10 +319,12 @@
   bf16_t *xn_s, *xn2_s, *act_s, *xa_qkv, *xa_o, *xa_gu, *xa_d;
   LoraImg i_qkv, i_o, i_gu, i_d;
 };
+struct LmTopTape { float *x1, *r_post, *xf, *r_f; bf16_t *gu, *hn; };
 struct LmTape {
   LmLayerTape* L;
   float *x_final, *r_f;
   bf16_t *hn, *dlogits;
+  LmTopTape c;
   size_t bytes;
 };
 constexpr int MAX_LM_LAYERS = 64;
@@ -326,7 +338,7 @@
 inline const float* lm_rope_cos(const ta_lm_weights* w, int l) { return ((w->nope_layers >> l) & 1) ? nullptr : w->rope_cos; }
 inline const float* lm_rope_sin(const ta_lm_weights* w, int l) { return ((w->nope_layers >> l) & 1) ? nullptr : w->rope_sin; }
 inline bool lm_attn_fused(const LmDims& d, int L) { return d.hd == 128 && L <= 192 && (d.nq / d.nkv) * ((L + 31) / 32) <= 12; }
-LmTape lm_tape(const ta_lm_weights* w, int B, int L, int n_lab, void* base, LmLayerTape* store) {
+LmTape lm_tape(const ta_lm_weights* w, int B, int L, int n_lab, int top_rows, void* base, LmLayerTape* store) {
   const LmDims d = lm_dims(w, B, L);
   Carver c(base);
   LmTape t; t.L = store;
@@ -365,6 +377,14 @@
   t.r_f = c.take<float>((size_t)d.M);
   t.hn = c.take<bf16_t>((size_t)d.M * d.D);
   t.dlogits = c.take<bf16_t>((size_t)(n_lab > 0 ? n_lab : 1) * w->vocab_pad);
+  t.c = LmTopTape{nullptr, nullptr, nullptr, nullptr, nullptr, nullptr};
+  if (top_rows > 0) {
+    const size_t n = (size_t)top_rows;
+    t.c.x1 = c.take<float>(n * d.D); t.c.r_post = c.take<float>(n);
+    t.c.gu = c.take<bf16_t>(n * 2 * d.F);
+    t.c.xf = c.take<float>(n * d.D); t.c.r_f = c.take<float>(n);
+    t.c.hn = c.take<bf16_t>(n * d.D);
+  }
   t.bytes = c.total();
   return t;
 }
@@ -373,12 +393,14 @@
   float* lora_part;
   long lp_layer, lp_off[8], lp_size[8]; int lp_chunks[8];
   float *logits, *dhl, *dhn, *dxa, *dxb32, *dxn, *delta, *skws;
+  bf16_t *top_ao, *top_dxb;
+  float *top_xa, *top_xb;
   bf16_t *tA, *tB;
   float* wsk;
   size_t bytes;
 };
 inline int wgrad_splits(int n_out, int k_in, int kp) { return pick_splits(n_out, k_in, kp); }
-LmWs lm_ws(const ta_lm_weights* w, int B, int L, int n_lab, void* base) {
+LmWs lm_ws(const ta_lm_weights* w, int B, int L, int n_lab, bool top, void* base) {
   const LmDims d = lm_dims(w, B, L);
   const int nl = n_lab > 0 ? n_lab : 1;
   Carver c(base);
@@ -403,6 +425,11 @@
   s.dv = c.take<bf16_t>((size_t)d.M * d.nkv * d.hd);
   s.dqkv = c.take<bf16_t>((size_t)d.M * d.NQKV);
   s.dyB = c.take<bf16_t>((size_t)d.M * 64);
+  s.top_ao = s.top_dxb = nullptr; s.top_xa = s.top_xb = nullptr;
+  if (top) {
+    s.top_ao = c.take<bf16_t>((size_t)nl * d.nq * d.hd); s.top_dxb = c.take<bf16_t>((size_t)nl * d.D);
+    s.top_xa = c.take<float>((size_t)nl * d.D); s.top_xb = c.take<float>((size_t)nl * d.D);
+  }
   s.lora_part = nullptr; s.lp_layer = 0;
   if (w->lora_rank > 0) {
     const int r = w->lora_rank, bq = d.nq * d.hd;
@@ -440,18 +467,20 @@
 extern "C" long ta_lm_tape_bytes(const ta_lm_weights* w, int B, int L, int n_label_rows) {
   LmLayerTape store[MAX_LM_LAYERS];
   if (w->n_layers > MAX_LM_LAYERS) return -1;
-  return (long)lm_tape(w, B, L, n_label_rows, nullptr, store).bytes;
+  return (long)lm_tape(w, B, L, n_label_rows, lm_top_tape_rows(w, B, L, n_label_rows), nullptr, store).bytes;
 }
 extern "C" long ta_lm_workspace_bytes(const ta_lm_weights* w, int B, int L, int n_label_rows) {
-  return (long)lm_ws(w, B, L, n_label_rows, nullptr).bytes;
+  return (long)lm_ws(w, B, L, n_label_rows, lm_top_rows(w, B, L, n_label_rows), nullptr).bytes;
 }
 
 struct LmExtend { const bf16_t *kc, *vc; const int *pmask, *clip_of, *len; int clips, Lp; };
+struct LmTopFwd { const int* rows; int n; LmTopTape c; };
 static int lm_layers_forward(const ta_lm_weights* w, const LmDims& d, int B, int L, const int* kmask, const int* pos,
                              LmLayerTape* store, bool alias, float* x_final, LmWs& s, const ta_i_lora_layer_imgs* ext,
                              bf16_t* kcache, bf16_t* vcache, int Lmax, hipStream_t st, const LoraDropDev* drop = nullptr,
-                             const int* seg = nullptr, const LmExtend* xt = nullptr) {
+                             const int* seg = nullptr, const LmExtend* xt = nullptr, const LmTopFwd* top = nullptr) {
   const int M = (int)d.M;
+  if (top && (alias || ext || xt || w->lora_rank > 0 || w->train_base)) return TA_ERR_ARG;
   const float scale = 1.0f / sqrtf((float)d.hd);
   const bool lora = w->lora_rank > 0;
   const int r = w->lora_rank;
@@ -516,13 +545,14 @@
     const bool keep = lora || (w->train_base && !alias);
     bf16_t* xn = keep ? p.xn_s : s.xn;
     const bool rb = lm_res_bf16(w);
+    int Mr = M;
     auto norm = [&](const float* x, const float* gw, bf16_t* y, float* r) -> int {
-      return rb ? ta_rmsnorm_fwd_bf16(x, gw, y, nullptr, r, M, d.D, w->eps, st) : ta_rmsnorm_fwd(x, gw, y, nullptr, r, M, d.D, w->eps, 0, st);
+      return rb ? ta_rmsnorm_fwd_bf16(x, gw, y, nullptr, r, Mr, d.D, w->eps, st) : ta_rmsnorm_fwd(x, gw, y, nullptr, r, Mr, d.D, w->eps, 0, st);
     };
     auto res_gemm = [&](const void* A, const void* Wm, float* out, int K, const float* res) -> int {
       ta_gemm_opts o = take_ext();
-      if (rb) { o.residual_bf16 = res; return gemm_opt(A, Wm, out, M, d.D, K, nullptr, nullptr, 0, 1, o, st); }
-      return gemm_opt(A, Wm, out, M, d.D, K, nullptr, res, 0, 0, o, st);
+      if (rb) { o.residual_bf16 = res; return gemm_opt(A, Wm, out, Mr, d.D, K, nullptr, nullptr, 0, 1, o, st); }
+      return gemm_opt(A, Wm, out, Mr, d.D, K, nullptr, res, 0, 0, o, st);
     };
     RC(norm(p.x_in, Lw.ln_in_w, xn, p.r_in));
     if (lgm & 1) RC(lora_fwd(xn, d.D, p.i_qkv, p.xa_qkv, 3, 8 * l + 0));
@@ -552,14 +582,21 @@
                              xt->clips, B, d.nq, d.nkv, L, xt->Lp, xt->Lp, scale, st));
     } else if (!fused_fwd && seg) RC(ta_attention_fwd_seg(p.q, p.k, p.vt, p.ao, p.lse, kmask, seg, B, d.nq, d.nkv, L, d.Lp, scale, st));
     else if (!fused_fwd) RC(ta_attention_fwd(p.q, p.k, p.vt, p.ao, p.lse, kmask, B, d.nq, d.nkv, L, d.Lp, d.hd, 1, scale, st));
+    if (top && l == w->n_layers - 1) {
+      RC(ta_gather_rows_bf16(p.ao, top->rows, s.top_ao, top->n, d.nq * d.hd, st));
+      if (rb) RC(ta_gather_rows_bf16(p.x_in, top->rows, s.top_xa, top->n, d.D, st));
+      else RC(ta_gather_rows_f32(p.x_in, top->rows, s.top_xa, top->n, d.D, st));
+      p.ao = s.top_ao; p.x_in = s.top_xa; p.x1 = top->c.x1; p.r_post = top->c.r_post; p.gu = top->c.gu; x_next = top->c.xf;
+      Mr = top->n;
+    }
     if (lgm & 2) RC(lora_fwd(p.ao, d.nq * d.hd, p.i_o, p.xa_o, 1, 8 * l + 3));
     RC(res_gemm(p.ao, Lw.wo, p.x1, d.nq * d.hd, p.x_in));
     bf16_t* xn2 = keep ? p.xn2_s : s.xn;
     bf16_t* act = keep ? p.act_s : s.act;
     RC(norm(p.x1, Lw.ln_post_w, xn2, p.r_post));
     if (lgm & 4) RC(lora_fwd(xn2, d.D, p.i_gu, p.xa_gu, 2, 8 * l + 4));
-    RC(gemm_opt(xn2, Lw.wgu, p.gu, M, 2 * d.F, d.D, nullptr, nullptr, 0, 1, take_ext(), st));
-    RC(ta_swiglu_fwd(p.gu, act, M, d.F, st));
+    RC(gemm_opt(xn2, Lw.wgu, p.gu, Mr, 2 * d.F, d.D, nullptr, nullptr, 0, 1, take_ext(), st));
+    RC(ta_swiglu_fwd(p.gu, act, Mr, d.F, st));
     if (lgm & 8) RC(lora_fwd(act, d.F, p.i_d, p.xa_d, 1, 8 * l + 6));
     RC(res_gemm(act, Lw.wd, x_next, d.F, p.x1));
   }
@@ -592,20 +629,43 @@
   const LmDims d = lm_dims(w, B, L);
   const int M = (int)d.M;
   LmLayerTape store[MAX_LM_LAYERS];
-  LmTape t = lm_tape(w, B, L, n_lab, tape, store);
-  LmWs s = lm_ws(w, B, L, n_lab, ws);
+  const bool top = lm_top_rows(w, B, L, n_lab);
+  LmTape t = lm_tape(w, B, L, n_lab, lm_top_tape_rows(w, B, L, n_lab), tape, store);
+  LmWs s = lm_ws(w, B, L, n_lab, top, ws);
   if ((long)s.bytes > ws_bytes) return TA_ERR_ARG;
   float* x = store[0].x_in;
   if (lm_res_bf16(w)) RC(ta_embed_scatter(ids, src_row, w->embed_f32, audio, nullptr, x, M, d.D, w->vocab, st));
   else RC(ta_embed_scatter(ids, src_row, w->embed_f32, audio, x, nullptr, M, d.D, w->vocab, st));
-  RC(lm_layers_forward(w, d, B, L, kmask, pos, store, false, t.x_final, s, nullptr, nullptr, nullptr, 0, st, dp, seg));
-  if (lm_res_bf16(w)) RC(ta_rmsnorm_fwd_bf16(t.x_final, w->norm_w, t.hn, nullptr, t.r_f, M, d.D, w->eps, st));
-  else RC(ta_rmsnorm_fwd(t.x_final, w->norm_w, t.hn, nullptr, t.r_f, M, d.D, w->eps, 0, st));
+  const LmTopFwd tf{label_rows, n_lab, t.c};
+  const bool top_fwd = top && !logits_out;
+  RC(lm_layers_forward(w, d, B, L, kmask, pos, store, false, t.x_final, s, nullptr, nullptr, nullptr, 0, st, dp, seg, nullptr,
+                       top_fwd ? &tf : nullptr));
+  const float* xf = top_fwd ? t.c.xf : t.x_final;
+  bf16_t* hn = top_fwd ? t.c.hn : t.hn;
+  float* r_f = top_fwd ? t.c.r_f : t.r_f;
+  const int Mf = top_fwd ? n_lab : M;
+  if (lm_res_bf16(w)) RC(ta_rmsnorm_fwd_bf16(xf, w->norm_w, hn, nullptr, r_f, Mf, d.D, w->eps, st));
+  else RC(ta_rmsnorm_fwd(xf, w->norm_w, hn, nullptr, r_f, Mf, d.D, w->eps, 0, st));
   if (logits_out)
     RC(gemm(t.hn, w->embed_bf16, logits_out, M, w->vocab_pad, d.D, nullptr, nullptr, 0, 1, st));
+  if (top && logits_out) {
+    const LmLayerTape& p = store[w->n_layers - 1];
+    if (lm_res_bf16(w)) {
+      RC(ta_gather_rows_bf16(p.x1, label_rows, t.c.x1, n_lab, d.D, st));
+      RC(ta_gather_rows_bf16(t.x_final, label_rows, t.c.xf, n_lab, d.D, st));
+    } else {
+      RC(ta_gather_rows_f32(p.x1, label_rows, t.c.x1, n_lab, d.D, st));
+      RC(ta_gather_rows_f32(t.x_final, label_rows, t.c.xf, n_lab, d.D, st));
+    }
+    RC(ta_gather_rows_f32(p.r_post, label_rows, t.c.r_post, n_lab, 1, st));
+    RC(ta_gather_rows_f32(t.r_f, label_rows, t.c.r_f, n_lab, 1, st));
+    RC(ta_gather_rows_bf16(p.gu, label_rows, t.c.gu, n_lab, 2 * d.F, st));
+    RC(ta_gather_rows_bf16(t.hn, label_rows, t.c.hn, n_lab, d.D, st));
+  }
   if (n_lab > 0) {
-    RC(ta_gather_rows_bf16(t.hn, label_rows, s.hl, n_lab, d.D, st));
-    RC(gemm(s.hl, w->embed_bf16, s.logits, n_lab, w->vocab_pad, d.D, nullptr, nullptr, 0, 1, st));
+    const bf16_t* hl = top ? t.c.hn : s.hl;
+    if (!top) RC(ta_gather_rows_bf16(t.hn, label_rows, s.hl, n_lab, d.D, st));
+    RC(gemm(hl, w->embed_bf16, s.logits, n_lab, w->vocab_pad, d.D, nullptr, nullptr, 0, 1, st));
     RC(ta_cross_entropy_opt(s.logits, 1, w->vocab_pad, nullptr, label_targets, n_lab, w->vocab, loss_scale, nll_rows, loss,
                             t.dlogits, w->vocab_pad, ce, st));
   }
@@ -649,9 +709,9 @@
 PrefillWs prefill_ws(const ta_lm_weights* w, int B, int L, void* base) {
   PrefillWs p;
   p.w1 = *w; p.w1.n_layers = 1;
-  p.t = lm_tape(&p.w1, B, L, 1, base, p.layer);
+  p.t = lm_tape(&p.w1, B, L, 1, 0, base, p.layer);
   p.tape_bytes = p.t.bytes;
-  p.s = lm_ws(w, B, L, B, base ? (char*)base + p.tape_bytes : nullptr);
+  p.s = lm_ws(w, B, L, B, false, base ? (char*)base + p.tape_bytes : nullptr);
   p.bytes = p.tape_bytes + p.s.bytes;
   return p;
 }
@@ -702,9 +762,9 @@
   const long rows = (long)R * T, labs = std::max((long)R * (T - 1), 1L);
   q.chunk = (int)std::min((long)TA_SCORE_CE_ROWS, labs);
   q.p.w1 = *w; q.p.w1.n_layers = 1;
-  q.p.t = lm_tape(&q.p.w1, R, T, 1, base, q.p.layer);
+  q.p.t = lm_tape(&q.p.w1, R, T, 1, 0, base, q.p.layer);
   q.p.tape_bytes = q.p.t.bytes;
-  q.p.s = lm_ws(w, R, T, q.chunk, base ? (char*)base + q.p.tape_bytes : nullptr);
+  q.p.s = lm_ws(w, R, T, q.chunk, false, base ? (char*)base + q.p.tape_bytes : nullptr);
   q.p.bytes = q.p.tape_bytes + q.p.s.bytes;
   Carver c(base ? (char*)base + q.p.bytes : nullptr);
   q.ids_clean = c.take<long>((size_t)rows);
@@ -786,8 +846,9 @@
   const LmDims d = lm_dims(w, B, L);
   const int M = (int)d.M;
   LmLayerTape store[MAX_LM_LAYERS];
-  LmTape t = lm_tape(w, B, L, n_lab, (void*)tape, store);
-  LmWs s = lm_ws(w, B, L, n_lab, ws);
+  const bool top = lm_top_rows(w, B, L, n_lab);
+  LmTape t = lm_tape(w, B, L, n_lab, lm_top_tape_rows(w, B, L, n_lab), (void*)tape, store);
+  LmWs s = lm_ws(w, B, L, n_lab, top, ws);
   if ((long)s.bytes > ws_bytes) return TA_ERR_ARG;
   const float scale = 1.0f / sqrtf((float)d.hd);
   if (d_audio && hipMemsetAsync(d_audio, 0, (size_t)n_audio_rows * d.D * 4, st) != hipSuccess) return TA_ERR_LAUNCH;
@@ -858,8 +919,10 @@
   const int sp = pick_splits(n_lab, d.D, w->vocab_pad);
   RC(ta_gemm_bf16_nt(t.dlogits, w->embed_t_bf16, s.dhl, n_lab, d.D, w->vocab_pad, w->vocab_pad, 0, 0, d.D, 0, 0, 0, nullptr,
                      nullptr, 0, 0, sp, s.skws, st));
-  if (hipMemsetAsync(s.dhn, 0, (size_t)M * d.D * 4, st) != hipSuccess) return TA_ERR_LAUNCH;
-  RC(ta_scatter_rows_f32(s.dhl, label_rows, s.dhn, n_lab, d.D, st));
+  if (!top) {
+    if (hipMemsetAsync(s.dhn, 0, (size_t)M * d.D * 4, st) != hipSuccess) return TA_ERR_LAUNCH;
+    RC(ta_scatter_rows_f32(s.dhl, label_rows, s.dhn, n_lab, d.D, st));
+  }
   const int Kp = pad64(M);
   auto wgrad = [&](const bf16_t* dy, int n_out, const bf16_t* x, int k_in, float* dW) -> int {
     if (!dW) return TA_OK;
@@ -883,35 +946,54 @@
   }
   float* dx = s.dxa;
   float* dx_alt = s.dxb32;
+  bf16_t *dxb = s.dxb, *dao = s.dao;
+  int Mr = M;
+  if (top) { Mr = n_lab; dx = s.top_xa; dx_alt = s.top_xb; dxb = s.top_dxb; dao = s.top_ao; }
   const int gb = 1;
   const bool dx_bf16 = lm_res_bf16(w) && w->dx_f32 == 0;
   auto norm_bwd = [&](const float* dy, int dyb, const float* x, const float* r, const float* gw, const float* dres, float* dxf,
                       bool last = false) -> int {
-    if (dx_bf16) return ta_rmsnorm_bwd_bf16s(dy, dyb, x, r, gw, dres ? s.dxb : nullptr, last ? dxf : nullptr, s.dxb, M, d.D, st);
-    if (lm_res_bf16(w)) return ta_rmsnorm_bwd_bf16(dy, dyb, x, r, gw, dres, dxf, s.dxb, M, d.D, st);
-    return dyb ? ta_rmsnorm_bwd_dyb(dy, x, r, gw, dres, dxf, s.dxb, M, d.D, st)
-               : ta_rmsnorm_bwd(dy, x, r, gw, dres, dxf, s.dxb, nullptr, M, d.D, 0, st);
+    if (dx_bf16) return ta_rmsnorm_bwd_bf16s(dy, dyb, x, r, gw, dres ? dxb : nullptr, last ? dxf : nullptr, dxb, Mr, d.D, st);
+    if (lm_res_bf16(w)) return ta_rmsnorm_bwd_bf16(dy, dyb, x, r, gw, dres, dxf, dxb, Mr, d.D, st);
+    return dyb ? ta_rmsnorm_bwd_dyb(dy, x, r, gw, dres, dxf, dxb, Mr, d.D, st)
+               : ta_rmsnorm_bwd(dy, x, r, gw, dres, dxf, dxb, nullptr, Mr, d.D, 0, st);
   };
-  RC(norm_bwd(s.dhn, 0, t.x_final, t.r_f, w->norm_w, nullptr, dx, w->n_layers == 0));
+  if (top) RC(norm_bwd(s.dhl, 0, t.c.xf, t.c.r_f, w->norm_w, nullptr, dx));
+  else RC(norm_bwd(s.dhn, 0, t.x_final, t.r_f, w->norm_w, nullptr, dx, w->n_layers == 0));
   for (int l = w->n_layers - 1; l >= 0; --l) {
     const ta_lm_layer& Lw = w->layers[l];
-    const LmLayerTape& p = store[l];
-    if (lgm & 8) RC(lora_bwd(s.dxb, d.D, p.act_s, d.F, p.xa_d, p.i_d, lora_grads[l].dla_d, lora_grads[l].dlb_d, 1, 1 << 30, 1 << 30, l, 3));
+    LmLayerTape p = store[l];
+    const bool top_l = top && l == w->n_layers - 1;
+    if (top_l) { p.x1 = t.c.x1; p.r_post = t.c.r_post; p.gu = t.c.gu; }
+    if (lgm & 8) RC(lora_bwd(dxb, d.D, p.act_s, d.F, p.xa_d, p.i_d, lora_grads[l].dla_d, lora_grads[l].dlb_d, 1, 1 << 30, 1 << 30, l, 3));
     const ta_lm_layer_wgrads* g = wg ? &wg->layers[l] : nullptr;
-    if (g) RC(wgrad(s.dxb, d.D, p.act_s, d.F, g->dwd));
-    RC(gemm_opt(s.dxb, Lw.wd_t, s.dact, M, d.F, d.D, nullptr, nullptr, 0, 1, take_ext(), st));
+    if (g) RC(wgrad(dxb, d.D, p.act_s, d.F, g->dwd));
+    RC(gemm_opt(dxb, Lw.wd_t, s.dact, Mr, d.F, d.D, nullptr, nullptr, 0, 1, take_ext(), st));
     RC(dx_drop_term(s.dact, d.F));
-    RC(ta_swiglu_bwd(s.dact, p.gu, s.dgu, M, d.F, st));
+    RC(ta_swiglu_bwd(s.dact, p.gu, s.dgu, Mr, d.F, st));
     if (lgm & 4) RC(lora_bwd(s.dgu, 2 * d.F, p.xn2_s, d.D, p.xa_gu, p.i_gu, lora_grads[l].dla_gu, lora_grads[l].dlb_gu, 2, d.F, 1 << 30, l, 2));
     if (g) RC(wgrad(s.dgu, 2 * d.F, p.xn2_s, d.D, g->dwgu));
-    RC(gemm_opt(s.dgu, Lw.wgu_t, s.dxn, M, d.D, 2 * d.F, nullptr, nullptr, 0, gb, take_ext(), st));
+    RC(gemm_opt(s.dgu, Lw.wgu_t, s.dxn, Mr, d.D, 2 * d.F, nullptr, nullptr, 0, gb, take_ext(), st));
     RC(dx_drop_term(s.dxn, d.D));
     if (g && g->dln_post) RC(ta_rmsnorm_dw(s.dxn, gb, p.x1, lm_res_bf16(w), p.r_post, g->dln_post, M, d.D, st));
     RC(norm_bwd(s.dxn, gb, p.x1, p.r_post, Lw.ln_post_w, dx, dx_alt));
-    if (lgm & 2) RC(lora_bwd(s.dxb, d.D, p.ao, bq, p.xa_o, p.i_o, lora_grads[l].dla_o, lora_grads[l].dlb_o, 1, 1 << 30, 1 << 30, l, 1));
-    if (g) RC(wgrad(s.dxb, d.D, p.ao, bq, g->dwo));
-    RC(gemm_opt(s.dxb, Lw.wo_t, s.dao, M, d.nq * d.hd, d.D, nullptr, nullptr, 0, 1, take_ext(), st));
-    RC(dx_drop_term(s.dao, d.nq * d.hd));
+    if (lgm & 2) RC(lora_bwd(dxb, d.D, p.ao, bq, p.xa_o, p.i_o, lora_grads[l].dla_o, lora_grads[l].dlb_o, 1, 1 << 30, 1 << 30, l, 1));
+    if (g) RC(wgrad(dxb, d.D, p.ao, bq, g->dwo));
+    RC(gemm_opt(dxb, Lw.wo_t, dao, Mr, d.nq * d.hd, d.D, nullptr, nullptr, 0, 1, take_ext(), st));
+    RC(dx_drop_term(dao, d.nq * d.hd));
+    if (top_l) {
+      float* dres = s.dxb32;
+      if (hipMemsetAsync(s.dao, 0, (size_t)M * d.nq * d.hd * 2, st) != hipSuccess) return TA_ERR_LAUNCH;
+      RC(ta_scatter_rows_bf16(dao, label_rows, s.dao, n_lab, d.nq * d.hd, st));
+      if (dx_bf16) {
+        if (hipMemsetAsync(s.dxb, 0, (size_t)M * d.D * 2, st) != hipSuccess) return TA_ERR_LAUNCH;
+        RC(ta_scatter_rows_bf16(dxb, label_rows, s.dxb, n_lab, d.D, st));
+      } else {
+        if (hipMemsetAsync(dres, 0, (size_t)M * d.D * 4, st) != hipSuccess) return TA_ERR_LAUNCH;
+        RC(ta_scatter_rows_f32(dx_alt, label_rows, dres, n_lab, d.D, st));
+      }
+      Mr = M; dx = s.dxa; dx_alt = dres; dxb = s.dxb; dao = s.dao;
+    }
     RC(ta_attn_bwd_prep(s.dao, p.ao, s.delta, s.dot, B, d.nq, L, d.Lp, st));
     const bf16_t* v_hm = (w->train_base || !lm_attn_fused(d, L)) ? p.v : nullptr;
     if (seg && !(g && (g->dqn || g->dkn))) {
diff --git a/tiny_audio_amd/csrc/elementwise.hip b/tiny_audio_amd/csrc/elementwise.hip
--- a/tiny_audio_amd/csrc/elementwise.hip
+++ b/tiny_audio_amd/csrc/elementwise.hip
@@ -361,6 +361,24 @@
   for (int c = lane; c < D / 4; c += 64) ((float4*)(out + s * D))[c] = ((const float4*)(in + (long)row * D))[c];
 }
 
+__global__ __launch_bounds__(256) void gather_rows_f32_kernel(const float* __restrict__ in, const int* __restrict__ idx,
+                                                              float* __restrict__ out, int n, int D) {
+  const int row = blockIdx.x * 4 + (threadIdx.x >> 6);
+  if (row >= n) return;
+  const int lane = threadIdx.x & 63;
+  const long s = idx[row];
+  if (D & 3) { for (int c = lane; c < D; c += 64) out[(long)row * D + c] = in[s * D + c]; return; }
+  for (int c = lane; c < D / 4; c += 64) ((float4*)(out + (long)row * D))[c] = ((const float4*)(in + s * D))[c];
+}
+__global__ __launch_bounds__(256) void scatter_rows_bf16_kernel(const bf16_t* __restrict__ in, const int* __restrict__ idx,
+                                                                bf16_t* __restrict__ out, int n, int D) {
+  const int row = blockIdx.x * 4 + (threadIdx.x >> 6);
+  if (row >= n) return;
+  const int lane = threadIdx.x & 63;
+  const long s = idx[row];
+  for (int c = lane; c < D / 8; c += 64) ((uint4*)(out + s * D))[c] = ((const uint4*)(in + (long)row * D))[c];
+}
+
 __global__ void bernoulli_keep_kernel(float* __restrict__ keep, long n, float keep_prob, unsigned long long seed) {
   for (long i = (long)blockIdx.x * blockDim.x + threadIdx.x; i < n; i += (long)gridDim.x * blockDim.x) {
     unsigned long long z = seed + 0x9E3779B97F4A7C15ull * (unsigned long long)(i + 1);
@@ -529,6 +547,18 @@
   TA_LAUNCH(scatter_rows_f32_kernel, dim3(ta_cdiv(n, 4)), dim3(256), 0, st, in, idx, out, n, D);
   TA_CHECK_LAUNCH(); return TA_OK;
 }
+extern "C" int ta_gather_rows_f32(const float* in, const int* idx, float* out, int n, int D, hipStream_t st) {
+  if (n <= 0) return TA_OK;
+  if (D <= 0) return TA_ERR_ARG;
+  TA_LAUNCH(gather_rows_f32_kernel, dim3(ta_cdiv(n, 4)), dim3(256), 0, st, in, idx, out, n, D);
+  TA_CHECK_LAUNCH(); return TA_OK;
+}
+extern "C" int ta_scatter_rows_bf16(const void* in, const int* idx, void* out, int n, int D, hipStream_t st) {
+  if (n <= 0) return TA_OK;
+  if (D % 8) return TA_ERR_ARG;
+  TA_LAUNCH(scatter_rows_bf16_kernel, dim3(ta_cdiv(n, 4)), dim3(256), 0, st, (const bf16_t*)in, idx, (bf16_t*)out, n, D);
+  TA_CHECK_LAUNCH(); return TA_OK;
+}
 extern "C" int ta_bernoulli_keep(float* keep, long n, float keep_prob, unsigned long long seed, hipStream_t st) {
   if (n <= 0) return TA_OK;
   TA_LAUNCH(bernoulli_keep_kernel, dim3(ew_blocks(n)), dim3(256), 0, st, keep, n, keep_prob, seed);
diff --git a/tiny_audio_amd/csrc/generate.hip b/tiny_audio_amd/csrc/generate.hip
--- a/tiny_audio_amd/csrc/generate.hip
+++ b/tiny_audio_amd/csrc/generate.hip
@@ -9,7 +9,8 @@
 static const int g_decode_pf_wgs = 0;
 static bool read_scores_split() { const char* e = getenv("TA355_SCORES_SPLIT"); return !(e && *e == '0'); }
 static bool g_scores_split = read_scores_split();
-void ta_i_reload_decode_knobs() { g_decode_fused = read_decode_fused(); g_scores_split = read_scores_split(); }
+void ta_i_reload_lm_knobs();
+void ta_i_reload_decode_knobs() { g_decode_fused = read_decode_fused(); g_scores_split = read_scores_split(); ta_i_reload_lm_knobs(); }
 
 namespace {
 constexpr int HD = 128;
diff --git a/tiny_audio_amd/ops.py b/tiny_audio_amd/ops.py
--- a/tiny_audio_amd/ops.py
+++ b/tiny_audio_amd/ops.py
@@ -28,7 +28,7 @@
     return t
 
 
-_KNOB_KEYS = ("TA355_GEMM_VARIANT", "TA355_GELU_LUT", "TA355_DECODE_FUSED", "TA355_SCORES_SPLIT")
+_KNOB_KEYS = ("TA355_GEMM_VARIANT", "TA355_GELU_LUT", "TA355_DECODE_FUSED", "TA355_SCORES_SPLIT", "TA355_LM_TOP_ROWS")
 _knob_state = None
 
 
```

Result: no change. 7613 (median of 6 runs) (+0.3%).
